# nanoporetech/isONclust2

Hardware: AMD Instinct MI355X
Metric: reads/s clustered (sahlin mode, k=11 w=15) (higher is better)
Workload: dtype u32

## Files before the change

include/isonclust2_hip.h:

```cpp
#ifndef ISONCLUST2_HIP_H
#define ISONCLUST2_HIP_H

#include <stddef.h>
#include <stdint.h>

#ifdef __cplusplus
extern "C" {
#endif

typedef struct ioc_ctx ioc_ctx;

typedef enum {
    IOC_OK = 0,
    IOC_ERR_ARG = -1,
    IOC_ERR_HIP = -2,
    IOC_ERR_STATE = -3,
    IOC_ERR_CAPACITY = -4,
    IOC_ERR_TABLE = -5,
    IOC_ERR_NO_DEVICE = -6,
    IOC_ERR_INPUT = -7
} ioc_status;

enum { IOC_MODE_SAHLIN = 0, IOC_MODE_FAST = 1, IOC_MODE_FURIOUS = 2, IOC_MODE_NONE = 3 };

typedef struct {
    int32_t k;
    int32_t w;
    int32_t min_shared;
    int32_t mode;
    double min_fraction;
    double mapped_threshold;
    double min_prob_no_hits;
    double aligned_threshold;
} ioc_params;

int ioc_ctx_create(int device, ioc_ctx** out);
void ioc_ctx_destroy(ioc_ctx* ctx);
int ioc_ctx_trim(ioc_ctx* ctx);
int ioc_ctx_prewarm(ioc_ctx* ctx, int32_t alignment_mode);
const char* ioc_last_error(const ioc_ctx* ctx);
int ioc_set_stream(ioc_ctx* ctx, void* hip_stream);
int ioc_synchronize(ioc_ctx* ctx);

int ioc_set_params(ioc_ctx* ctx, const ioc_params* p, const int32_t gap_limit[225]);

int ioc_queries_upload(ioc_ctx* ctx, int32_t n, const int64_t* off_fwd, const int64_t* off_rev,
                       const uint32_t* min_val, const uint32_t* min_pos, int64_t total,
                       const uint32_t* hpc_len, const uint8_t* err_cell, const uint32_t* min_total);
int ioc_queries_bind_device(ioc_ctx* ctx, int32_t n, const int64_t* d_off_fwd, const int64_t* d_off_rev,
                            const uint32_t* d_min_val, const uint32_t* d_min_pos, int64_t total,
                            const uint32_t* d_hpc_len, const uint8_t* d_err_cell,
                            const uint32_t* d_min_total, const int64_t* h_off_fwd,
                            const int64_t* h_off_rev);

int ioc_left_load(ioc_ctx* ctx, int32_t n_clusters, const uint8_t* cls_err_cell, int64_t n_keys,
                  const uint32_t* keys, const int64_t* offs, const uint32_t* postings);

int ioc_index_update(ioc_ctx* ctx, int32_t cls, const uint32_t* old_min, int64_t n_old, const uint32_t* new_min,
                     int64_t n_new, uint8_t new_err_cell);
int ioc_left_export(ioc_ctx* ctx, int64_t* n_keys, int64_t* n_postings, uint32_t* keys, int64_t* offs,
                    uint32_t* postings);

int ioc_index_build(ioc_ctx* ctx);
int ioc_score(ioc_ctx* ctx);
int ioc_resolve(ioc_ctx* ctx, int32_t* n_iter);
int ioc_get_decisions(ioc_ctx* ctx, int32_t* target, int8_t* strand, uint8_t* flags);
int ioc_get_cuts(ioc_ctx* ctx, int32_t* cut);
int ioc_force_decision(ioc_ctx* ctx, int32_t query, int32_t target, int32_t strand);
int ioc_clear_forced(ioc_ctx* ctx);
int ioc_set_aln_verdicts(ioc_ctx* ctx, const int32_t* target, const int8_t* strand);
#define IOC_TIE_SLOTS 16
int ioc_get_ties(ioc_ctx* ctx, uint32_t* count, uint32_t* keys);

int ioc_scored_candidates(ioc_ctx* ctx, int32_t q, int32_t cap, uint32_t* key, uint32_t* size);
int ioc_query_candidates(ioc_ctx* ctx, int32_t query, int32_t cap, int32_t* target, int8_t* strand,
                         uint32_t* size, uint32_t* first_index, uint32_t* total_mapped);

int ioc_index_export(ioc_ctx* ctx, int64_t* n_keys, int64_t* n_postings, uint32_t* keys,
                     int64_t* offs, uint32_t* postings);

int ioc_qual_scores(ioc_ctx* ctx, int32_t n, const int64_t* offs, const uint8_t* qual, int32_t k,
                    double* score, double* err_rate);
int ioc_extract_minimizers(ioc_ctx* ctx, int32_t n, const int64_t* offs, const uint8_t* seq,
                           const uint8_t* qual, int32_t k, int32_t w, uint32_t* hpc_len,
                           double* hpc_err, int64_t* off_fwd, int64_t* off_rev, int32_t* status);
int ioc_extracted_hpc_download(ioc_ctx* ctx, char* hpc_seq, char* hpc_qual, int64_t cap);
int ioc_extracted_download(ioc_ctx* ctx, uint32_t* min_val, uint32_t* min_pos, int64_t cap);
int ioc_queries_from_extracted(ioc_ctx* ctx, const uint8_t* keep, const uint8_t* err_cell,
                               const uint32_t* min_total);

typedef struct {
    float ms_build;
    float ms_score;
    float ms_resolve;
    int32_t resolve_iters;
    int32_t n_queries;
    int64_t n_minimizers;
    int64_t n_index_postings;
    int64_t n_candidates;
    int64_t n_mapped_evals;
    int64_t postings_traversed;
    float ms_align_fwd;
    float ms_align_trace;
    int64_t n_align_pairs;
    int64_t n_align_cells;
    int64_t n_align_refused;
    int32_t score_oob;
    int32_t score_oob_probe;
    int64_t align_arena_bytes;
    int32_t align_slices;
    int32_t align_version;
    int64_t n_align_cells_computed;
} ioc_timings;
int ioc_get_timings(ioc_ctx* ctx, ioc_timings* out);
int ioc_count_reference_postings(ioc_ctx* ctx, int64_t* n_postings);

int ioc_host_gap_limits(const char* table_path, int32_t k, int32_t w, double min_prob_no_hits,
                        int32_t* gap_limit, double* p_shared);
uint8_t ioc_host_err_cell(double err_rate);
uint32_t ioc_host_min_total(uint32_t hpc_len, double mapped_threshold);

int ioc_host_align(const char* query, int32_t qlen, const char* ref, int32_t rlen, int32_t match,
                   int32_t mismatch, int32_t gap_open, int32_t gap_extend, char* comp, int32_t comp_cap,
                   int32_t* score_out);
int32_t ioc_host_gap_open(double e1_plus_e2);
double ioc_host_aln_ratio(const char* comp, int32_t comp_len, double e, uint32_t slen, uint32_t k);

typedef struct {
    int32_t query;
    int32_t ref;
    int32_t ref_revcomp;
    int32_t reserved;
    double e;
} ioc_aln_pair;
int ioc_align_set_pool(ioc_ctx* ctx, int32_t n_seqs, const char* seqs, const int64_t* offs);
int ioc_align_pairs(ioc_ctx* ctx, int32_t n_pairs, const ioc_aln_pair* pairs, int32_t k, int32_t match,
                    int32_t mismatch, int32_t gap_extend, int32_t* out_score, int64_t* out_windows,
                    double* out_ratio);
int ioc_align_set_verdict_threshold(ioc_ctx* ctx, double aligned_threshold);

int64_t ioc_queries_generation(const ioc_ctx* ctx);
int64_t ioc_gather_records_device(ioc_ctx* ctx, int32_t n_idx, const int32_t* entries, uint32_t* d_out_min,
                                  uint32_t* d_out_pos, int64_t cap, int64_t* off_fwd, int64_t* off_rev);

typedef struct {
    int32_t n;
    const int64_t* off_fwd;
    const int64_t* off_rev;
    const uint32_t* min_val;
    const uint32_t* min_pos;
    int64_t total;
    const uint32_t* raw_len;
    const uint32_t* hpc_len;
    const double* score;
    const double* raw_err;
    const double* hpc_err;
    const uint8_t* state;
    double min_qual;
    const char* raw_seq;
    const int64_t* raw_off;
    const int32_t* n_members;
    int32_t depth;
    int32_t min_cls_size;
    const uint8_t* is_cluster;
    int32_t minimizers_on_device;
} ioc_batch_view;

typedef struct {
    int32_t n_clusters;
    const double* cls_hpc_err;
    int64_t n_keys;
    const uint32_t* keys;
    const int64_t* offs;
    const uint32_t* postings;
    const char* rep_seq;
    const int64_t* rep_off;
    const double* cls_raw_err;
} ioc_left_view;

typedef struct {
    int64_t n_clusters;
    int64_t n_joined;
    int64_t n_gated;
    int64_t n_tie_replays;
    int64_t n_aln_invoked;
    int32_t resolve_iters;
    int32_t aln_rounds;
    int64_t n_aln_pairs;
    int64_t n_aln_order_dep;
    int64_t n_cons_invoked;
    int64_t n_cons_restarts;
} ioc_cluster_stats;

int ioc_cluster_batch(ioc_ctx* ctx, const ioc_params* p, const char* table_path,
                      const ioc_batch_view* right, int32_t* out_cls, int8_t* out_strand,
                      ioc_cluster_stats* stats);
int ioc_cluster_merge(ioc_ctx* ctx, const ioc_params* p, const char* table_path, const ioc_left_view* left,
                      const ioc_batch_view* right, int32_t* out_cls, int8_t* out_strand,
                      ioc_cluster_stats* stats);
typedef struct {
    const char* raw_seq;
    int32_t raw_len;
    char raw_qual;
    double raw_err;
    double raw_score;
    const char* hpc_seq;
    int32_t hpc_len;
    double hpc_err;
    const uint32_t* fwd_min;
    const uint32_t* fwd_pos;
    int32_t n_fwd;
    const uint32_t* rev_min;
    const uint32_t* rev_pos;
    int32_t n_rev;
    int32_t entry;
} ioc_rep_record;
typedef struct {
    void* user;
    int (*create)(void* user, int side, int idx, const char* seq, int len);
    int (*size)(void* user, int side, int idx);
    int (*add)(void* user, int side, int idx, const char* seq, int len, unsigned weight);
    int (*consensus)(void* user, int side, int idx, char* out, int cap);
    int (*purge)(void* user, int side, int idx, const char* seq, int len, unsigned weight);
    void (*rep_changed)(void* user, int32_t cls, const ioc_rep_record* rec);
    const struct ioc_consensus_spec_ops* spec;
} ioc_consensus_ops;
typedef struct ioc_consensus_spec_ops {
    int (*create_tagged)(void* user, int side, int idx, const char* seq, int len, int tag);
    int (*add_tagged)(void* user, int side, int idx, const char* seq, int len, unsigned weight, int tag);
    int (*consensus_deferred)(void* user, int side, int idx, int tag);
    int (*flush)(void* user, int safe_tag);
    int (*collect)(void* user, int side, int idx, int tag, char* out, int cap);
    int (*rollback)(void* user, int first_tag);
    int (*commit)(void* user);
} ioc_consensus_spec_ops;
typedef struct {
    int32_t cons_min_size;
    int32_t cons_max_size;
    int32_t cons_period;
    int32_t left_depth;
    const int32_t* left_sizes;
} ioc_consensus_args;
int ioc_cluster_consensus(ioc_ctx* ctx, const ioc_params* p, const char* table_path, const ioc_left_view* left,
                          const ioc_batch_view* right, const ioc_consensus_args* args, const ioc_consensus_ops* ops,
                          int32_t* out_cls, int8_t* out_strand, ioc_cluster_stats* stats);

#define IOC_POA_LOCAL 0
#define IOC_POA_GLOBAL 1
#define IOC_POA_SEMI_GLOBAL 2
typedef struct ioc_poa ioc_poa;
int ioc_poa_create(ioc_ctx* ctx, int32_t m, int32_t n, int32_t g, int32_t e, int32_t q, int32_t c, ioc_poa** out);
int ioc_poa_create_mode(ioc_ctx* ctx, int32_t mode, int32_t m, int32_t n, int32_t g, int32_t e, int32_t q, int32_t c, ioc_poa** out);
void ioc_poa_destroy(ioc_poa* poa);
void ioc_poa_bind(ioc_poa* poa, ioc_consensus_ops* ops);
int ioc_poa_graph_export(ioc_poa* poa, int side, int idx, int32_t* n_nodes, int32_t* n_edges, char* bases, int32_t* rank,
                         int32_t* edge_from, int32_t* edge_to, int64_t* edge_w);
int ioc_poa_last_alignment(ioc_poa* poa, int32_t cap, int32_t* nodes, int32_t* pos, int32_t* score);
int64_t ioc_poa_graph_save(ioc_poa* poa, int side, int idx, uint8_t* out, int64_t cap);
int ioc_poa_graph_load(ioc_poa* poa, int side, int idx, const uint8_t* in, int64_t len);
int ioc_poa_graph_load_many(ioc_poa* poa, int side, int32_t count, const int32_t* idx, const uint8_t* const* in, const int64_t* len);

int ioc_cluster_resident(ioc_ctx* ctx, int32_t* out_cls, int8_t* out_strand, ioc_cluster_stats* stats);
int ioc_resident_set_sequences(ioc_ctx* ctx, const char* raw_seq, const int64_t* raw_off, const double* raw_err);

#define IOC_DIST_ID_BYTES 128
int ioc_dist_unique_id(uint8_t* id );
int ioc_dist_init(ioc_ctx* ctx, const uint8_t* id, int32_t rank, int32_t world);
int ioc_dist_shutdown(ioc_ctx* ctx);
int ioc_dist_info(const ioc_ctx* ctx, int32_t* rank, int32_t* world);
int ioc_dist_allgather_device(ioc_ctx* ctx, const void* d_send, void* d_recv, int64_t bytes_per_rank);
int ioc_dist_allgatherv_device(ioc_ctx* ctx, const void* d_send, void* d_recv, const int64_t* counts, const int64_t* displs,
                               int32_t esize);
int ioc_dist_allgather_i64(ioc_ctx* ctx, int64_t mine, int64_t* all );
int ioc_dist_allgatherv_host(ioc_ctx* ctx, const void* send, int64_t bytes, void* recv, int64_t* sizes);
int ioc_dist_allreduce_max(ioc_ctx* ctx, double* x);
int ioc_dist_barrier(ioc_ctx* ctx);
typedef struct {
    float ms_exchange_lists;
    double ms_merge;
    int64_t bytes_lists;
    int64_t bytes_records;
    int32_t sharded;
    int32_t exchanges;
} ioc_dist_merge_times;
#define IOC_XCHG_MAX_U8 0
#define IOC_XCHG_MIN_U32 1
#define IOC_XCHG_SUM_I32 2
typedef int (*ioc_exchange_fn)(void* user, void* d_buf, int64_t count, int32_t kind, void* hip_stream);
int ioc_set_shard(ioc_ctx* ctx, int32_t world, int32_t rank, ioc_exchange_fn fn, void* user);
int32_t ioc_shard_exchanges(const ioc_ctx* ctx);
int64_t ioc_shard_aligned_pairs(const ioc_ctx* ctx);
int ioc_dist_exchange(ioc_ctx* ctx, void* d_buf, int64_t count, int32_t kind);
int ioc_dist_set_shard(ioc_ctx* ctx, int32_t on);

int ioc_dist_merge(ioc_ctx* ctx, const ioc_params* p, const char* table_path, const ioc_batch_view* reps, int32_t min_cls_size,
                   int64_t out_cap, int32_t* out_cls, int8_t* out_strand, int64_t* out_counts, ioc_cluster_stats* stats,
                   ioc_dist_merge_times* times);

#ifdef __cplusplus
}
#endif
#endif
```

isonclust2_amd/_lib.py:

```python
import ctypes as C
import os

HERE = os.path.dirname(os.path.abspath(__file__))
LIB_PATH = os.environ.get("IOC_LIB", os.path.join(HERE, "libisonclust2_hip.so"))
TABLE_PATH = os.path.join(HERE, "data", "pmin_shared.bin")


class IocError(RuntimeError):
    def __init__(self, code, msg):
        super().__init__(f"isonclust2_hip error {code}: {msg}")
        self.code = code


class Params(C.Structure):
    _fields_ = [("k", C.c_int32), ("w", C.c_int32), ("min_shared", C.c_int32), ("mode", C.c_int32),
                ("min_fraction", C.c_double), ("mapped_threshold", C.c_double),
                ("min_prob_no_hits", C.c_double), ("aligned_threshold", C.c_double)]


class BatchView(C.Structure):
    _fields_ = [("n", C.c_int32), ("off_fwd", C.POINTER(C.c_int64)), ("off_rev", C.POINTER(C.c_int64)),
                ("min_val", C.POINTER(C.c_uint32)), ("min_pos", C.POINTER(C.c_uint32)),
                ("total", C.c_int64), ("raw_len", C.POINTER(C.c_uint32)),
                ("hpc_len", C.POINTER(C.c_uint32)), ("score", C.POINTER(C.c_double)),
                ("raw_err", C.POINTER(C.c_double)), ("hpc_err", C.POINTER(C.c_double)),
                ("state", C.POINTER(C.c_uint8)), ("min_qual", C.c_double),
                ("raw_seq", C.c_char_p), ("raw_off", C.POINTER(C.c_int64)),
                ("n_members", C.POINTER(C.c_int32)), ("depth", C.c_int32), ("min_cls_size", C.c_int32),
                ("is_cluster", C.POINTER(C.c_uint8)), ("minimizers_on_device", C.c_int32)]


class LeftView(C.Structure):
    _fields_ = [("n_clusters", C.c_int32), ("cls_hpc_err", C.POINTER(C.c_double)), ("n_keys", C.c_int64),
                ("keys", C.POINTER(C.c_uint32)), ("offs", C.POINTER(C.c_int64)),
                ("postings", C.POINTER(C.c_uint32)), ("rep_seq", C.c_char_p),
                ("rep_off", C.POINTER(C.c_int64)), ("cls_raw_err", C.POINTER(C.c_double))]


class ClusterStats(C.Structure):
    _fields_ = [("n_clusters", C.c_int64), ("n_joined", C.c_int64), ("n_gated", C.c_int64),
                ("n_tie_replays", C.c_int64), ("n_aln_invoked", C.c_int64),
                ("resolve_iters", C.c_int32), ("aln_rounds", C.c_int32), ("n_aln_pairs", C.c_int64),
                ("n_aln_order_dep", C.c_int64), ("n_cons_invoked", C.c_int64), ("n_cons_restarts", C.c_int64)]

    def as_dict(self):
        return {n: int(getattr(self, n)) for n, _ in self._fields_}


class RepRecord(C.Structure):
    _fields_ = [("raw_seq", C.POINTER(C.c_char)), ("raw_len", C.c_int32), ("raw_qual", C.c_char), ("raw_err", C.c_double),
                ("raw_score", C.c_double), ("hpc_seq", C.POINTER(C.c_char)), ("hpc_len", C.c_int32), ("hpc_err", C.c_double),
                ("fwd_min", C.POINTER(C.c_uint32)), ("fwd_pos", C.POINTER(C.c_uint32)), ("n_fwd", C.c_int32),
                ("rev_min", C.POINTER(C.c_uint32)), ("rev_pos", C.POINTER(C.c_uint32)), ("n_rev", C.c_int32),
                ("entry", C.c_int32)]


CONS_CREATE = C.CFUNCTYPE(C.c_int, C.c_void_p, C.c_int, C.c_int, C.POINTER(C.c_char), C.c_int)
CONS_SIZE = C.CFUNCTYPE(C.c_int, C.c_void_p, C.c_int, C.c_int)
CONS_ADD = C.CFUNCTYPE(C.c_int, C.c_void_p, C.c_int, C.c_int, C.POINTER(C.c_char), C.c_int, C.c_uint)
CONS_CONSENSUS = C.CFUNCTYPE(C.c_int, C.c_void_p, C.c_int, C.c_int, C.POINTER(C.c_char), C.c_int)
CONS_PURGE = C.CFUNCTYPE(C.c_int, C.c_void_p, C.c_int, C.c_int, C.POINTER(C.c_char), C.c_int, C.c_uint)
CONS_REP_CHANGED = C.CFUNCTYPE(None, C.c_void_p, C.c_int32, C.POINTER(RepRecord))


class ConsensusOps(C.Structure):
    _fields_ = [("user", C.c_void_p), ("create", CONS_CREATE), ("size", CONS_SIZE), ("add", CONS_ADD),
                ("consensus", CONS_CONSENSUS), ("purge", CONS_PURGE), ("rep_changed", CONS_REP_CHANGED),
                ("spec", C.c_void_p)]


class ConsensusArgs(C.Structure):
    _fields_ = [("cons_min_size", C.c_int32), ("cons_max_size", C.c_int32), ("cons_period", C.c_int32),
                ("left_depth", C.c_int32), ("left_sizes", C.POINTER(C.c_int32))]


class AlnPair(C.Structure):
    _fields_ = [("query", C.c_int32), ("ref", C.c_int32), ("ref_revcomp", C.c_int32), ("reserved", C.c_int32),
                ("e", C.c_double)]


class DistMergeTimes(C.Structure):
    _fields_ = [("ms_exchange_lists", C.c_float), ("ms_merge", C.c_double), ("bytes_lists", C.c_int64), ("bytes_records", C.c_int64),
                ("sharded", C.c_int32), ("exchanges", C.c_int32)]


EXCHANGE_FN = C.CFUNCTYPE(C.c_int, C.c_void_p, C.c_void_p, C.c_int64, C.c_int32, C.c_void_p)
XCHG_MAX_U8, XCHG_MIN_U32, XCHG_SUM_I32 = 0, 1, 2


class Timings(C.Structure):
    _fields_ = [("ms_build", C.c_float), ("ms_score", C.c_float), ("ms_resolve", C.c_float),
                ("resolve_iters", C.c_int32), ("n_queries", C.c_int32), ("n_minimizers", C.c_int64),
                ("n_index_postings", C.c_int64), ("n_candidates", C.c_int64),
                ("n_mapped_evals", C.c_int64), ("postings_traversed", C.c_int64),
                ("ms_align_fwd", C.c_float), ("ms_align_trace", C.c_float), ("n_align_pairs", C.c_int64),
                ("n_align_cells", C.c_int64),
                ("n_align_refused", C.c_int64), ("score_oob", C.c_int32), ("score_oob_probe", C.c_int32),
                ("align_arena_bytes", C.c_int64), ("align_slices", C.c_int32), ("align_version", C.c_int32),
                ("n_align_cells_computed", C.c_int64)]

    def as_dict(self):
        return {n: getattr(self, n) for n, _ in self._fields_}


SYMBOLS = [
    "ioc_ctx_create", "ioc_ctx_destroy", "ioc_ctx_trim", "ioc_ctx_prewarm", "ioc_last_error", "ioc_set_stream", "ioc_synchronize",
    "ioc_set_params", "ioc_queries_upload", "ioc_queries_bind_device", "ioc_left_load",
    "ioc_index_build", "ioc_score", "ioc_resolve", "ioc_get_decisions", "ioc_get_cuts", "ioc_force_decision",
    "ioc_clear_forced", "ioc_query_candidates", "ioc_index_export", "ioc_qual_scores",
    "ioc_extract_minimizers", "ioc_extracted_download", "ioc_extracted_hpc_download", "ioc_queries_from_extracted",
    "ioc_get_timings", "ioc_count_reference_postings", "ioc_host_gap_limits", "ioc_host_err_cell", "ioc_host_min_total",
    "ioc_cluster_batch", "ioc_cluster_merge", "ioc_cluster_resident", "ioc_host_align", "ioc_host_gap_open",
    "ioc_host_aln_ratio", "ioc_align_set_pool", "ioc_align_pairs", "ioc_set_aln_verdicts", "ioc_get_ties", "ioc_resident_set_sequences",
    "ioc_index_update", "ioc_left_export", "ioc_cluster_consensus",
    "ioc_poa_create", "ioc_poa_create_mode", "ioc_poa_destroy", "ioc_poa_bind", "ioc_poa_graph_export", "ioc_poa_last_alignment",
    "ioc_poa_graph_save", "ioc_poa_graph_load", "ioc_poa_graph_load_many", "ioc_gather_records_device", "ioc_queries_generation", "ioc_scored_candidates",
    "ioc_dist_unique_id", "ioc_dist_init", "ioc_dist_shutdown", "ioc_dist_info", "ioc_dist_allgather_device",
    "ioc_dist_allgatherv_device", "ioc_dist_allgather_i64", "ioc_dist_allgatherv_host", "ioc_dist_allreduce_max",
    "ioc_dist_barrier", "ioc_dist_merge", "ioc_set_shard", "ioc_shard_exchanges", "ioc_shard_aligned_pairs", "ioc_dist_exchange", "ioc_dist_set_shard", "ioc_align_set_verdict_threshold",
]

_lib = None


def load():
    global _lib
    if _lib is not None:
        return _lib
    if not os.path.exists(LIB_PATH):
        raise IocError(-100, f"{LIB_PATH} is missing: run `python -c 'import __graft_entry__ as g; g.build()'` "
                             "(hipcc --offload-arch=gfx950); there is no CPU fallback")
    try:
        import torch
    except Exception:
        pass
    L = C.CDLL(LIB_PATH)
    vp, i32, i64 = C.c_void_p, C.c_int32, C.c_int64
    pi64, pu32, pu8 = C.POINTER(C.c_int64), C.POINTER(C.c_uint32), C.POINTER(C.c_uint8)
    pi32, pi8, pd = C.POINTER(C.c_int32), C.POINTER(C.c_int8), C.POINTER(C.c_double)
    L.ioc_ctx_create.argtypes = [i32, C.POINTER(vp)]
    L.ioc_ctx_destroy.argtypes = [vp]
    L.ioc_ctx_destroy.restype = None
    L.ioc_last_error.argtypes = [vp]
    L.ioc_last_error.restype = C.c_char_p
    L.ioc_set_stream.argtypes = [vp, vp]
    L.ioc_synchronize.argtypes = [vp]
    L.ioc_set_params.argtypes = [vp, C.POINTER(Params), pi32]
    L.ioc_queries_upload.argtypes = [vp, i32, pi64, pi64, pu32, pu32, i64, pu32, pu8, pu32]
    L.ioc_queries_bind_device.argtypes = [vp, i32, vp, vp, vp, vp, i64, vp, vp, vp, pi64, pi64]
    L.ioc_gather_records_device.argtypes = [vp, i32, pi32, vp, vp, i64, pi64, pi64]
    L.ioc_gather_records_device.restype = i64
    L.ioc_scored_candidates.argtypes = [vp, i32, i32, pu32, pu32]
    L.ioc_queries_generation.argtypes = [vp]
    L.ioc_queries_generation.restype = i64
    L.ioc_left_load.argtypes = [vp, i32, pu8, i64, pu32, pi64, pu32]
    L.ioc_index_update.argtypes = [vp, i32, pu32, i64, pu32, i64, C.c_uint8]
    L.ioc_left_export.argtypes = [vp, pi64, pi64, pu32, pi64, pu32]
    L.ioc_index_build.argtypes = [vp]
    L.ioc_score.argtypes = [vp]
    L.ioc_resolve.argtypes = [vp, pi32]
    L.ioc_get_decisions.argtypes = [vp, pi32, pi8, pu8]
    L.ioc_get_cuts.argtypes = [vp, pi32]
    L.ioc_force_decision.argtypes = [vp, i32, i32, i32]
    L.ioc_clear_forced.argtypes = [vp]
    L.ioc_query_candidates.argtypes = [vp, i32, i32, pi32, pi8, pu32, pu32, pu32]
    L.ioc_index_export.argtypes = [vp, pi64, pi64, pu32, pi64, pu32]
    L.ioc_qual_scores.argtypes = [vp, i32, pi64, pu8, i32, pd, pd]
    L.ioc_extract_minimizers.argtypes = [vp, i32, pi64, pu8, pu8, i32, i32, pu32, pd, pi64, pi64, pi32]
    L.ioc_extracted_download.argtypes = [vp, pu32, pu32, i64]
    L.ioc_extracted_hpc_download.argtypes = [vp, C.c_char_p, C.c_char_p, i64]
    L.ioc_queries_from_extracted.argtypes = [vp, pu8, pu8, pu32]
    L.ioc_get_timings.argtypes = [vp, C.POINTER(Timings)]
    L.ioc_count_reference_postings.argtypes = [vp, pi64]
    L.ioc_host_gap_limits.argtypes = [C.c_char_p, i32, i32, C.c_double, pi32, pd]
    L.ioc_host_err_cell.argtypes = [C.c_double]
    L.ioc_host_err_cell.restype = C.c_uint8
    L.ioc_host_min_total.argtypes = [C.c_uint32, C.c_double]
    L.ioc_host_min_total.restype = C.c_uint32
    L.ioc_cluster_batch.argtypes = [vp, C.POINTER(Params), C.c_char_p, C.POINTER(BatchView), pi32, pi8,
                                    C.POINTER(ClusterStats)]
    L.ioc_cluster_merge.argtypes = [vp, C.POINTER(Params), C.c_char_p, C.POINTER(LeftView), C.POINTER(BatchView),
                                    pi32, pi8, C.POINTER(ClusterStats)]
    L.ioc_cluster_consensus.argtypes = [vp, C.POINTER(Params), C.c_char_p, C.POINTER(LeftView), C.POINTER(BatchView),
                                        C.POINTER(ConsensusArgs), C.POINTER(ConsensusOps), pi32, pi8, C.POINTER(ClusterStats)]
    L.ioc_poa_create.argtypes = [vp, i32, i32, i32, i32, i32, i32, C.POINTER(vp)]
    L.ioc_poa_create_mode.argtypes = [vp, i32, i32, i32, i32, i32, i32, i32, C.POINTER(vp)]
    L.ioc_poa_destroy.argtypes = [vp]
    L.ioc_poa_destroy.restype = None
    L.ioc_poa_bind.argtypes = [vp, C.POINTER(ConsensusOps)]
    L.ioc_poa_bind.restype = None
    L.ioc_poa_graph_export.argtypes = [vp, C.c_int, C.c_int, pi32, pi32, C.c_char_p, pi32, pi32, pi32, pi64]
    L.ioc_poa_last_alignment.argtypes = [vp, i32, pi32, pi32, pi32]
    L.ioc_poa_graph_save.argtypes = [vp, C.c_int, C.c_int, pu8, i64]
    L.ioc_poa_graph_save.restype = C.c_int64
    L.ioc_poa_graph_load.argtypes = [vp, C.c_int, C.c_int, pu8, i64]
    L.ioc_poa_graph_load_many.argtypes = [vp, C.c_int, C.c_int32, C.POINTER(C.c_int32), C.POINTER(pu8), C.POINTER(i64)]
    L.ioc_host_align.argtypes = [C.c_char_p, i32, C.c_char_p, i32, i32, i32, i32, i32, C.c_char_p, i32, pi32]
    L.ioc_host_gap_open.argtypes = [C.c_double]
    L.ioc_host_aln_ratio.argtypes = [C.c_char_p, i32, C.c_double, C.c_uint32, C.c_uint32]
    L.ioc_host_aln_ratio.restype = C.c_double
    L.ioc_cluster_resident.argtypes = [vp, pi32, pi8, C.POINTER(ClusterStats)]
    L.ioc_resident_set_sequences.argtypes = [vp, C.c_char_p, pi64, pd]
    L.ioc_set_aln_verdicts.argtypes = [vp, pi32, pi8]
    L.ioc_get_ties.argtypes = [vp, C.POINTER(C.c_uint32), C.POINTER(C.c_uint32)]
    L.ioc_align_set_pool.argtypes = [vp, i32, C.c_char_p, C.POINTER(C.c_int64)]
    L.ioc_align_pairs.argtypes = [vp, i32, C.POINTER(AlnPair), i32, i32, i32, i32, pi32, C.POINTER(C.c_int64),
                                  C.POINTER(C.c_double)]
    L.ioc_dist_unique_id.argtypes = [pu8]
    L.ioc_dist_init.argtypes = [vp, pu8, i32, i32]
    L.ioc_dist_shutdown.argtypes = [vp]
    L.ioc_dist_info.argtypes = [vp, pi32, pi32]
    L.ioc_dist_allgather_device.argtypes = [vp, vp, vp, i64]
    L.ioc_dist_allgatherv_device.argtypes = [vp, vp, vp, pi64, pi64, i32]
    L.ioc_dist_allgather_i64.argtypes = [vp, i64, pi64]
    L.ioc_dist_allgatherv_host.argtypes = [vp, vp, i64, vp, pi64]
    L.ioc_dist_allreduce_max.argtypes = [vp, pd]
    L.ioc_dist_barrier.argtypes = [vp]
    L.ioc_dist_merge.argtypes = [vp, C.POINTER(Params), C.c_char_p, C.POINTER(BatchView), i32, i64, pi32, pi8, pi64,
                                 C.POINTER(ClusterStats), C.POINTER(DistMergeTimes)]
    L.ioc_set_shard.argtypes = [vp, i32, i32, EXCHANGE_FN, vp]
    L.ioc_shard_exchanges.argtypes = [vp]
    L.ioc_shard_aligned_pairs.argtypes = [vp]
    L.ioc_shard_aligned_pairs.restype = C.c_int64
    L.ioc_dist_exchange.argtypes = [vp, vp, i64, i32]
    L.ioc_dist_set_shard.argtypes = [vp, i32]
    L.ioc_align_set_verdict_threshold.argtypes = [vp, C.c_double]
    _lib = L
    return L
```

isonclust2_amd/csrc/ioc_align_gpu.hip:

```cpp
#include <hip/hip_runtime.h>

#include <algorithm>
#include <chrono>
#include <cmath>
#include <cstdint>
#include <cstring>
#include <numeric>
#include <string>
#include <type_traits>
#include <vector>

#include "ioc_internal.h"

namespace {

constexpr int ALN_C = 8;
constexpr int ALN_MAXW = 8;
constexpr int ALN_NEG = INT32_MIN / 4;
constexpr uint32_t ALN_LEN_SHIFT = 26;

struct AlnPairDev {
    uint32_t q_off, n;
    uint32_t r_off, m;
    int32_t gap_open, ilimit;
// ... 867 lines not shown
    const AlnPairDev pr = pairs[pid];
    const uint32_t n = pr.n, m = pr.m;
    const int go = pr.gap_open, il = pr.ilimit;
    const uint8_t* __restrict__ q = pool + pr.q_off;
    const uint8_t* __restrict__ r = pool + pr.r_off;
    const int2* __restrict__ rowck = ck + cko[pid].row_off;
    const int2* __restrict__ colck = ck + cko[pid].col_off;
    const uint32_t lane = threadIdx.x & 63u;
    const uint32_t k = P.k, kmask = k >= 32 ? 0xFFFFFFFFu : ((1u << k) - 1u);
    const int4 en = ends[pid];
    uint32_t i = uint32_t(en.y), j = uint32_t(en.z);
    int state = 0;
    WinStat ws;
    ws.blanks((m - j) + (n - i), kmask, k, il);

    while (i > 0 && j > 0) {
        const uint32_t r0 = ((i - 1) / TILE) * TILE, c0 = ((j - 1) / TILE) * TILE;
        const uint32_t rows = i - r0, cols = j - c0;
        const int gd = go - P.gap_extend, ge = P.gap_extend;
        int cm = P.match + 2 * ge + gd, cx = P.mismatch + 2 * ge + gd;
        asm volatile("" : "+v"(cm), "+v"(cx));
        for (uint32_t x = lane; x < rows; x += 64) {
            s_q[x] = q[r0 + x];
            int2 le{ge * int(r0 + x + 1) - gd, ALN_NEG};
            if (c0) le = colck[uint64_t(c0 / TILE - 1) * col_pitch(n) + r0 + x];
            s_left[x] = le;
        }
        const uint32_t jb = c0 + lane * TR_C;
        uint32_t rpk[1];
        {
            uint32_t w = 0;
#pragma unroll
            for (int e = 0; e < TR_C; ++e) w |= ref_byte(r, m, pr.rc, jb + e) << (8 * e);
            rpk[0] = w;
        }
        int Hp[TR_C], F[TR_C];
        int dg = ge * int(r0 + jb) - gd;
        if (r0 == 0) {
#pragma unroll
            for (int c = 0; c < TR_C; ++c) {
                Hp[c] = ge * int(jb + c + 1) - gd;
                F[c] = ALN_NEG;
            }
        } else {
            const int* roh = reinterpret_cast<const int*>(rowck + uint64_t(r0 / TILE - 1) * row_pitch(m));
            const int* rof = roh + row_pitch(m);
#pragma unroll
            for (int c = 0; c < TR_C; ++c) {
                int2 v{0, ALN_NEG};
                if (jb + c < m) v = int2{roh[jb + c], rof[jb + c]};
                Hp[c] = v.x;
                F[c] = v.y;
            }
            if (jb > 0 && jb <= m) dg = roh[jb - 1];
        }
        tr_wave_sync();
        const uint32_t nact = (cols + TR_C - 1) / TR_C;
        const uint32_t nsteps = rows + nact - 1;
        int out_h = 0, out_e = ALN_NEG;
        uint32_t out_q = 0;
        int2 nle = s_left[0];
        uint32_t nq = s_q[0];
        auto tstep = [&](const uint32_t s) __attribute__((always_inline)) {
            int hl = int(from_left_or(uint32_t(out_h), uint32_t(nle.x)));
            int el = int(from_left_or(uint32_t(out_e), uint32_t(nle.y)));
            uint32_t qc = from_left_or(out_q, nq);
            {
                const uint32_t sn = s + 1u < rows ? s + 1u : rows - 1u;
                nle = s_left[sn];
                nq = s_q[sn];
            }
            const int ri = int(s) - int(lane);
            if (ri >= 0 && uint32_t(ri) < rows && lane < nact) {
                const int hl_in = hl;
                uint32_t bits = 0;
#pragma unroll
                for (int c = 0; c < TR_C; ++c) {
                    const bool ex = el > hl;
                    const int E = max(el, hl);
                    const bool fx = F[c] > Hp[c];
                    const int Fn = max(F[c], Hp[c]);
                    const bool mt = qc == ((rpk[0] >> (8 * c)) & 0xFFu);
                    const int hd = dg + (mt ? cm : cx);
                    const int h = max(max(hd, E), Fn);
                    const uint32_t from = h == hd ? (mt ? 0u : 3u << (4 * c)) : (h == E ? 1u << (4 * c) : 2u << (4 * c));
                    bits |= from | (ex ? 4u << (4 * c) : 0u) | (fx ? 8u << (4 * c) : 0u);
                    dg = Hp[c];
                    Hp[c] = h - gd;
                    F[c] = Fn;
                    hl = h - gd;
                    el = E;
                }
                dg = hl_in;
                if (TR_C == 4)
                    dirs[ri][lane] = uint16_t(bits);
                else
                    reinterpret_cast<uint8_t*>(&dirs[0][0])[uint32_t(ri) * 64u + lane] = uint8_t(bits);
            }
            out_h = hl;
            out_e = el;
            out_q = qc;
        };
        {
            uint32_t s = 0;
#if IOC_TR_STEP_UNROLL == 4
            for (; s + 3u < nsteps; s += 4) {
                tstep(s);
                tstep(s + 1u);
                tstep(s + 2u);
                tstep(s + 3u);
            }
#endif
            for (; s + 1u < nsteps; s += 2) {
                tstep(s);
                tstep(s + 1u);
            }
            if (s < nsteps) tstep(s);
        }
        tr_wave_sync();
        while (i > r0 && j > c0) {
            const uint32_t cj = j - c0 - 1;
            const uint32_t ri = i - r0 - 1;
            const uint32_t t = TR_C == 4 ? (uint32_t(dirs[ri][cj / TR_C]) >> (4 * (cj % TR_C))) & 0xFu
                                         : (uint32_t(reinterpret_cast<const uint8_t*>(&dirs[0][0])[ri * 64u + cj / TR_C]) >> (4 * (cj % TR_C))) & 0xFu;
            if (state == 0) {
                const bool inr = i - r0 > lane && j - c0 > lane;
                uint32_t tl = 1u;
                if (inr) {
                    const uint32_t rl = ri - lane, cl = cj - lane;
                    tl = (TR_C == 4 ? (uint32_t(dirs[rl][cl / TR_C]) >> (4 * (cl % TR_C)))
                                    : (uint32_t(reinterpret_cast<const uint8_t*>(&dirs[0][0])[rl * 64u + cl / TR_C]) >> (4 * (cl % TR_C)))) & 3u;
                }
                const bool dgl = inr && (tl == 0u || tl == 3u);
                const unsigned long long dm = __ballot(dgl);
                const uint32_t run = ~dm ? uint32_t(__builtin_ctzll(~dm)) : 64u;
                if (run > 0) {
                    const unsigned long long mb = __ballot(dgl && tl == 0u) & (run == 64u ? ~0ull : ((1ull << run) - 1ull));
                    ws.push_run(mb, run, kmask, k, il, lane);
                    i -= run;
                    j -= run;
                } else {
                    state = (t & 3u) == 1u ? 1 : 2;
                }
            } else if (state == 1) {
                ws.push(0u, kmask, k, il);
                if (!(t & 4u)) state = 0;
                --j;
            } else {
                ws.push(0u, kmask, k, il);
                if (!(t & 8u)) state = 0;
                --i;
            }
        }
        tr_wave_sync();
    }
    ws.blanks(i + j, kmask, k, il);
    if (lane == 0) {
        out_score[pid] = en.x;
        out_count[pid] = ws.cnt;
    }
}

__global__ void __launch_bounds__(256)
k_seq_flags(const uint8_t* __restrict__ pool, const int64_t* __restrict__ offs, uint8_t* __restrict__ flags)
{
    __shared__ uint32_t s_any;
    if (threadIdx.x == 0) s_any = 0;
    __syncthreads();
    const int64_t a = offs[blockIdx.x], b = offs[blockIdx.x + 1];
    uint32_t any = 0;
    for (int64_t i = a + threadIdx.x; i < b; i += 256) {
        const uint8_t ch = pool[i];
        any |= (ch != 'A' && ch != 'C' && ch != 'G' && ch != 'T') ? 1u : 0u;
    }
    if (any) s_any = 1;
    __syncthreads();
    if (threadIdx.x == 0) flags[blockIdx.x] = uint8_t(s_any);
}

int reserve(ioc_ctx* c, DevBuf& b, size_t bytes)
{
    if (bytes == 0) bytes = 16;
    if (b.cap >= bytes) return IOC_OK;
    if (b.p) {
        if (hipStreamSynchronize(c->stream) != hipSuccess) return ioc_fail(c, IOC_ERR_HIP, "stream synchronize failed");
        (void)hipFree(b.p);
        b.p = nullptr;
        b.cap = 0;
    }
    const size_t want = bytes + bytes / 8 + 256;
    const hipError_t e = hipMalloc(&b.p, want);
    if (e != hipSuccess) {
        b.p = nullptr;
        return ioc_fail(c, IOC_ERR_CAPACITY, "hipMalloc(" + std::to_string(want) + " B) failed: " + hipGetErrorString(e));
    }
    b.cap = want;
    ioc_poison(b.p, want);
    return IOC_OK;
}

#define ACHK(c, call)                                                                             \
    do {                                                                                          \
        hipError_t e__ = (call);                                                                  \
        if (e__ != hipSuccess)                                                                    \
            return ioc_fail((c), IOC_ERR_HIP, std::string(#call) + ": " + hipGetErrorString(e__)); \
    } while (0)

#include "ioc_align_v2.inc"


struct EventSet {
    std::vector<hipEvent_t> v;
    ~EventSet()
    {
        for (auto& e : v)
            if (e) (void)hipEventDestroy(e);
    }
};

void add_elapsed(ioc_ctx* c, const std::vector<hipEvent_t>& evs, size_t used)
{
    for (size_t x = 0; x + 2 < used && x + 2 < evs.size(); x += 3) {
        float a = 0, b = 0;
        if (hipEventElapsedTime(&a, evs[x], evs[x + 1]) == hipSuccess) c->tm.ms_align_fwd += a;
        if (hipEventElapsedTime(&b, evs[x + 1], evs[x + 2]) == hipSuccess) c->tm.ms_align_trace += b;
    }
}

int compute_units(const ioc_ctx* c)
{
    int n_cu = 256;
    (void)hipDeviceGetAttribute(&n_cu, hipDeviceAttributeMultiprocessorCount, c->device);
    return n_cu < 1 ? 256 : n_cu;
}

int ck_budget(ioc_ctx* c, uint64_t* budget)
{
    size_t free_b = 0, total_b = 0;
    ACHK(c, hipMemGetInfo(&free_b, &total_b));
    *budget = uint64_t(free_b + c->a_ck.cap) / 2;
    if (const char* e = getenv("IOC_ALIGN_CK_BUDGET_MB")) *budget = uint64_t(atoll(e)) << 20;
    return IOC_OK;
}


constexpr int P16_GUARD = 28000;

struct CorridorModel {
    const ioc_ctx* c;
    AlnParams P;
    double frac;
    bool fixed;
    bool fit_ok;
    double pair_frac(const AlnPairDev& d) const
    {
        if (fixed || !(P.match > 0)) return frac;
        const double e = double(d.e_sum);
        if (!(e > 0.0) || !(e < 1.0)) return frac;
        const int go = std::max(2, std::min(5, d.gap_open));
        double rho = double(P.match) - e * (double(P.match - P.mismatch) / 3.0 + 2.0 / 3.0 * double(go + P.match)), margin = 0.02;
        const ioc_ctx::CorridorFit& f = c->aln_fit[go - 2];
        if (fit_ok && f.n >= 64.0 && e >= f.e_lo - 0.02 && e <= f.e_hi + 0.02) {
            const double me = f.se / f.n, mr = f.sr / f.n, vee = f.see / f.n - me * me, ver = f.ser / f.n - me * mr, vrr = f.srr / f.n - mr * mr;
            const double slope = vee > 1e-9 ? ver / vee : 0.0;
            const double sd = std::sqrt(std::max(0.0, vrr - slope * ver));
            rho = mr + slope * (e - me) - 4.5 * std::max(sd, 0.004);
            margin = 0.003;
        }
        return std::max(0.03, std::min(0.45, 1.0 - rho / double(P.match) + margin));
    }
};

CorridorModel corridor_model(const ioc_ctx* c, const AlnParams& P, bool corridor)
{
    CorridorModel m{c, P, corridor ? 0.2 : 0.0, false, false};
    if (const char* e = getenv("IOC_ALIGN_CORRIDOR")) {
        m.frac = corridor ? std::max(0.0, std::min(1.0, atof(e))) : 0.0;
        m.fixed = true;
    }
    m.fit_ok = c->aln_fit_sig[0] == P.match && c->aln_fit_sig[1] == P.mismatch && c->aln_fit_sig[2] == P.gap_extend && !getenv("IOC_ALIGN_CORRIDOR_NO_FIT");
    return m;
}

uint32_t band_target(uint32_t ncouples, uint32_t few_limit, int occ, int n_cu)
{
    const uint32_t waves = uint32_t(occ) * uint32_t(n_cu) * uint32_t(V2_WAVES);
    uint32_t want = std::max(12u, std::min(uint32_t(V2_MAX_BANDS), (waves + ncouples - 1u) / std::max(1u, ncouples)));
    if (few_limit && ncouples <= few_limit) want = std::min(want, 17u);
    return want;
}

struct V2Plan {
    uint32_t cnt = 0, np = 0, ncouples = 0;
    std::vector<V2Couple> cps;
    std::vector<V2PairCk> pck;
    std::vector<V2PairEnd> pend;
    std::vector<uint64_t> cwords;
    uint32_t lrow_total = 0, best_total = 0, max_strips = 1;
    uint64_t tiles_skipped = 0, tiles_all = 0;
    std::vector<std::pair<uint32_t, uint32_t>> slices;
    uint64_t arena_words = 0, prof_total = 0;
    std::vector<std::vector<V2Item>> items;
    std::vector<uint32_t> n_probe;
    uint32_t max_items = 0, max_flags = 0, max_pairs = 0;
};

void plan_bands(V2Couple& cp, uint32_t ncoarse, uint32_t want_bands, bool corridor)
{
    const uint32_t wb = (corridor && ncoarse >= 16u) ? std::max(want_bands, 17u) : want_bands;
    const uint32_t reg = std::max<uint32_t>(want_bands > 16u ? 1u : 2u, (ncoarse + wb - 1) / wb);
    std::vector<uint32_t> hts;
    for (uint32_t left = ncoarse; left;) {
        const uint32_t hgt = std::min(reg, left);
        hts.push_back(hgt);
        left -= hgt;
    }
    while (hts.size() > size_t(V2_MAX_BANDS)) {
        const size_t mid = hts.size() / 2;
        hts[mid - 1] += hts[mid];
        hts.erase(hts.begin() + long(mid));
    }
    cp.nbands = uint32_t(hts.size());
    cp.tpb = reg;
    uint32_t acc = 0;
    for (uint32_t b = 0; b <= uint32_t(V2_MAX_BANDS); ++b) {
        cp.bstart[b] = uint16_t(std::min<uint32_t>(acc, 0xFFFFu));
        if (b < cp.nbands) acc += hts[b];
    }
}

uint32_t plan_corridor(V2Couple& cp, const std::vector<AlnPairDev>& dp, const CorridorModel& cm, uint32_t nmax, uint32_t mmax, int32_t cert[2])
{
    const AlnParams& P = cm.P;
    constexpr uint32_t probe_rows = 1024;
    cp.corridor = 0;
    for (uint32_t b = 0; b < uint32_t(V2_MAX_BANDS); ++b) {
        cp.plo[b] = 0;
        cp.phi[b] = uint16_t(std::min<uint32_t>(65535u, cp.nstrips - 1u));
    }
    const uint32_t strip_cols = 64u * FW_C;
    double frac = 0.0;
    for (int h = 0; h < 2; ++h)
        if (cp.pid[h] != 0xFFFFFFFFu) frac = std::max(frac, cm.pair_frac(dp[cp.pid[h]]));
    if (cm.frac <= 0.0) frac = 0.0;
    const uint32_t B = uint32_t(frac * double(std::max(nmax, mmax)));
    cp.b0 = B;
    int64_t beff = INT64_MAX;
    uint32_t skipped = 0;
    uint16_t lo[V2_MAX_BANDS], hi[V2_MAX_BANDS];
    bool fits = cm.frac > 0.0 && B >= strip_cols && cp.nstrips <= 65535u && cp.nbands <= uint32_t(V2_MAX_BANDS) && P.match > 0 && P.mismatch <= P.match &&
                P.gap_extend >= 0;
    for (int h = 0; fits && h < 2; ++h)
        if (cp.pid[h] != 0xFFFFFFFFu) fits = dp[cp.pid[h]].gap_open >= 0;
    for (uint32_t b = 0; fits && b < cp.nbands; ++b) {
        const uint32_t r0 = uint32_t(cp.bstart[b]) * uint32_t(CK2), r1 = std::min(nmax, uint32_t(cp.bstart[b + 1u]) * uint32_t(CK2));
        const uint32_t c_lo = r0 > B ? r0 - B : 0u, c_hi = std::min<uint64_t>(mmax, uint64_t(r1) + B);
        if (c_hi <= c_lo) {
            fits = false;
            break;
        }
        lo[b] = uint16_t(c_lo / strip_cols);
        hi[b] = uint16_t((c_hi - 1u) / strip_cols);
        skipped += lo[b] + (cp.nstrips - 1u - hi[b]);
        if (lo[b] > 0) beff = std::min<int64_t>(beff, int64_t(r0) - int64_t(lo[b]) * strip_cols);
        if ((uint64_t(hi[b]) + 1u) * strip_cols < mmax) beff = std::min<int64_t>(beff, int64_t(hi[b] + 1u) * strip_cols - int64_t(r1));
    }
    uint32_t pb = 0, ps = 0;
    if (fits) {
        while (pb + 1u < cp.nbands && uint32_t(cp.bstart[pb + 1u]) * uint32_t(CK2) < probe_rows) ++pb;
        const uint32_t R = uint32_t(cp.bstart[pb + 1u]) * uint32_t(CK2);
        ps = (R - 1u) / strip_cols;
        fits = pb + 1u < cp.nbands && R >= probe_rows;
        for (uint32_t b = 0; fits && b <= pb; ++b) fits = lo[b] == 0 && hi[b] >= ps;
        for (int h = 0; fits && h < 2; ++h)
            if (cp.pid[h] != 0xFFFFFFFFu) fits = dp[cp.pid[h]].n >= R && dp[cp.pid[h]].m > ps * strip_cols;
    }
    cp.probe_band = uint16_t(pb);
    cp.probe_strip = uint16_t(ps);
    if (fits && skipped * 5u >= cp.nbands * cp.nstrips && beff > 0 && beff < INT64_MAX) {
        cp.corridor = 1;
        for (uint32_t b = 0; b < cp.nbands; ++b) {
            cp.plo[b] = lo[b];
            cp.phi[b] = hi[b];
        }
    }
    for (int h = 0; h < 2; ++h) {
        cert[h] = INT32_MIN;
        if (cp.pid[h] == 0xFFFFFFFFu || !cp.corridor) continue;
        const AlnPairDev& d = dp[cp.pid[h]];
        cert[h] = int32_t(std::min<int64_t>(INT32_MAX, int64_t(P.match) * std::max<int64_t>(0, int64_t(std::max(d.n, d.m)) - beff - 1)));
    }
    return cp.corridor ? skipped : 0u;
}

uint64_t couple_words(V2Couple& cp, uint32_t nmax, uint32_t mmax)
{
    auto up4 = [](uint64_t x) { return (x + 3u) & ~uint64_t(3); };
    cp.mpad = uint32_t((uint64_t(mmax) + 15u) & ~uint64_t(15));
    cp.nq = (nmax + 3u) / 4u;
    const uint64_t ncr = (nmax - 1u) / CK2, ncc = (mmax - 1u) / CK2;
    uint64_t w = 0;
    cp.rdat = w;
    w += up4(ncr * 2u * cp.mpad);
    cp.rbase = w;
    w += up4(ncr * (cp.mpad / 16u) * 2u);
    cp.cdat = w;
    w += up4(ncc * uint64_t(cp.nq) * 8u);
    cp.cbase = w;
    w += up4(ncc * uint64_t(cp.nq) * 2u);
    return w;
}

void plan_couples(V2Plan& pl, const std::vector<AlnPairDev>& dp, const uint32_t* order, const CorridorModel& cm, uint32_t want_bands)
{
    pl.cps.resize(pl.ncouples);
    pl.pck.resize(pl.np);
    pl.pend.resize(pl.np);
    pl.cwords.resize(pl.ncouples);
    for (uint32_t k2 = 0; k2 < pl.ncouples; ++k2) {
        V2Couple& cp = pl.cps[k2];
        cp.pid[0] = order[2u * k2];
        cp.pid[1] = 2u * k2 + 1u < pl.cnt ? order[2u * k2 + 1u] : 0xFFFFFFFFu;
        uint32_t nmax = 0, mmax = 0;
        for (int h = 0; h < 2; ++h)
            if (cp.pid[h] != 0xFFFFFFFFu) {
                nmax = std::max(nmax, dp[cp.pid[h]].n);
                mmax = std::max(mmax, dp[cp.pid[h]].m);
            }
        cp.nstrips = (mmax + 64u * FW_C - 1) / (64u * FW_C);
        plan_bands(cp, (nmax + CK2 - 1) / CK2, want_bands, cm.frac > 0.0);
        int32_t cert[2];
        pl.tiles_skipped += plan_corridor(cp, dp, cm, nmax, mmax, cert);
        pl.tiles_all += uint64_t(cp.nbands) * cp.nstrips;
        pl.cwords[k2] = couple_words(cp, nmax, mmax);
        cp.prof = 0;
        pl.max_strips = std::max(pl.max_strips, cp.nstrips);
        for (int h = 0; h < 2; ++h) {
            cp.lrow0[h] = pl.lrow_total;
            cp.best0[h] = pl.best_total;
            if (cp.pid[h] == 0xFFFFFFFFu) continue;
            const AlnPairDev& d = dp[cp.pid[h]];
            const uint32_t nstr = (d.m + 64u * FW_C - 1) / (64u * FW_C);
            pl.pend[cp.pid[h]] = V2PairEnd{pl.lrow_total, pl.best_total, cp.nbands, k2, cert[h]};
            pl.lrow_total += nstr * 64u;
            pl.best_total += cp.nbands;
        }
    }
}

void slice_couples(V2Plan& pl, uint64_t budget)
{
    for (uint32_t first = 0; first < pl.ncouples;) {
        uint64_t used = 0;
        uint32_t k2 = first;
        uint64_t prof_used = 0;
        while (k2 < pl.ncouples) {
            const uint64_t prof_k = uint64_t(pl.cps[k2].nstrips) * 2u * 5u * 64u;
            if (k2 != first && (used + pl.cwords[k2]) * 4ull + (prof_used + prof_k) * sizeof(uint4) > budget) break;
            V2Couple& cp = pl.cps[k2];
            cp.prof = prof_used;
            prof_used += prof_k;
            cp.rdat += used;
            cp.rbase += used;
            cp.cdat += used;
            cp.cbase += used;
            for (int h = 0; h < 2; ++h)
                if (cp.pid[h] != 0xFFFFFFFFu) pl.pck[cp.pid[h]] = V2PairCk{cp.rdat, cp.rbase, cp.cdat, cp.cbase, cp.mpad, cp.nq, uint32_t(h), k2};
            used += pl.cwords[k2];
            ++k2;
        }
        pl.arena_words = std::max(pl.arena_words, used);
        pl.prof_total = std::max(pl.prof_total, prof_used);
        pl.slices.emplace_back(first, k2 - first);
        first = k2;
    }
}

void tile_lists(V2Plan& pl)
{
    pl.items.resize(pl.slices.size());
    pl.n_probe.assign(pl.slices.size(), 0);
    for (size_t si = 0; si < pl.slices.size(); ++si) {
        const uint32_t k_lo = pl.slices[si].first, k_hi = pl.slices[si].first + pl.slices[si].second;
        uint32_t nf = 0;
        auto& it = pl.items[si];
        uint32_t maxdiag = 0;
        size_t total_items = 0;
        for (uint32_t k2 = k_lo; k2 < k_hi; ++k2) {
            V2Couple& cp = pl.cps[k2];
            cp.flag0 = nf;
            nf += cp.nbands * cp.nstrips;
            total_items += size_t(cp.nbands) * cp.nstrips;
            maxdiag = std::max(maxdiag, cp.nbands + cp.nstrips - 2u);
        }
        it.reserve(total_items + 64u * pl.slices[si].second);
        for (uint32_t dg = 0; dg <= maxdiag; ++dg) {
            bool any = false;
            for (uint32_t k2 = k_lo; k2 < k_hi; ++k2) {
                const V2Couple& cp = pl.cps[k2];
                if (!cp.corridor || dg > uint32_t(cp.probe_band) + cp.probe_strip) continue;
                any = true;
                const uint32_t b_lo = dg >= uint32_t(cp.probe_strip) + 1u ? dg - cp.probe_strip : 0u, b_hi = std::min<uint32_t>(dg, cp.probe_band);
                for (uint32_t b = b_lo; b <= b_hi; ++b) it.push_back(V2Item{k2, uint16_t(b), uint16_t(dg - b)});
            }
            if (!any && dg > 64u) break;
        }
        pl.n_probe[si] = uint32_t(it.size());
        for (uint32_t dg = 0; dg <= maxdiag; ++dg)
            for (uint32_t k2 = k_lo; k2 < k_hi; ++k2) {
                const V2Couple& cp = pl.cps[k2];
                if (dg > cp.nbands + cp.nstrips - 2u) continue;
                const uint32_t b_lo = dg >= cp.nstrips ? dg - cp.nstrips + 1u : 0u, b_hi = std::min(dg, cp.nbands - 1u);
                for (uint32_t b = b_lo; b <= b_hi; ++b) it.push_back(V2Item{k2, uint16_t(b), uint16_t(dg - b)});
            }
        pl.max_items = std::max<uint32_t>(pl.max_items, uint32_t(it.size()));
        pl.max_flags = std::max(pl.max_flags, nf);
        pl.max_pairs = std::max(pl.max_pairs, std::min(pl.cnt, 2u * k_hi) - 2u * k_lo);
    }
}

struct V2Opts {
    int n_cu, occ, guard;
    uint32_t few_limit;
    uint32_t deadline;
    unsigned long long deadline_cycles;
    uint32_t help_wgs;
    bool side_help;
};

struct V2Dev {
    V2Couple* cps;
    V2PairCk* pck;
    V2PairEnd* pend;
    V2Item* items;
    int2 *lrow, *best;
    uint32_t* ctl;
    size_t ctl_words;
    V2Scratch *scratch, *hscratch;
    uint32_t* resume;
    uint32_t* park;
    uint32_t* early;
    uint32_t* gate;
    size_t resume_words;
};

int v2_tables(ioc_ctx* c, const V2Plan& pl, uint32_t help_wgs, V2Dev& t)
{
    hipStream_t s = c->stream;
    int r;
    const uint32_t ncouples = pl.ncouples, np = pl.np;
    const size_t tab_bytes = size_t(ncouples) * sizeof(V2Couple) + size_t(np) * (sizeof(V2PairCk) + sizeof(V2PairEnd)) + size_t(pl.max_items) * sizeof(V2Item) + 256;
    if ((r = reserve(c, c->a_cko, tab_bytes)) != IOC_OK) return r;
    uint8_t* tb = static_cast<uint8_t*>(c->a_cko.p);
    t.cps = reinterpret_cast<V2Couple*>(tb);
    t.pck = reinterpret_cast<V2PairCk*>(tb + size_t(ncouples) * sizeof(V2Couple));
    t.pend = reinterpret_cast<V2PairEnd*>(reinterpret_cast<uint8_t*>(t.pck) + size_t(np) * sizeof(V2PairCk));
    t.items = reinterpret_cast<V2Item*>(reinterpret_cast<uint8_t*>(t.pend) + size_t(np) * sizeof(V2PairEnd));
    ACHK(c, hipMemcpyAsync(t.cps, pl.cps.data(), size_t(ncouples) * sizeof(V2Couple), hipMemcpyHostToDevice, s));
    ACHK(c, hipMemcpyAsync(t.pck, pl.pck.data(), size_t(np) * sizeof(V2PairCk), hipMemcpyHostToDevice, s));
    ACHK(c, hipMemcpyAsync(t.pend, pl.pend.data(), size_t(np) * sizeof(V2PairEnd), hipMemcpyHostToDevice, s));
    if ((r = reserve(c, c->a_prof, size_t(pl.prof_total) * sizeof(uint4) + 256)) != IOC_OK) return r;
    if ((r = reserve(c, c->a_ends2, size_t(np) * sizeof(int4))) != IOC_OK) return r;
    if ((r = reserve(c, c->a_lrow, (size_t(pl.lrow_total) + pl.best_total + 16) * sizeof(int2))) != IOC_OK) return r;
    t.lrow = static_cast<int2*>(c->a_lrow.p);
    t.best = t.lrow + pl.lrow_total;
    t.ctl_words = ((16 + 2 * size_t(pl.max_flags) + np + 1) & ~size_t(1)) + 2;
    if ((r = reserve(c, c->a_xflags, t.ctl_words * 4)) != IOC_OK) return r;
    t.ctl = static_cast<uint32_t*>(c->a_xflags.p);
    const size_t n_scratch = size_t(pl.max_pairs) + size_t(help_wgs) * V2_NHELP * V2_HBUF;
    t.resume_words = size_t(np) * V2_RESUME_WORDS + 2u * (size_t(pl.max_pairs) + 1u) + 4u;
    if ((r = reserve(c, c->a_bnd, n_scratch * sizeof(V2Scratch) + t.resume_words * 4)) != IOC_OK) return r;
    t.scratch = static_cast<V2Scratch*>(c->a_bnd.p);
    t.hscratch = t.scratch + pl.max_pairs;
    t.resume = reinterpret_cast<uint32_t*>(t.scratch + n_scratch);
    t.park = t.resume + size_t(np) * V2_RESUME_WORDS;
    t.early = t.park + size_t(pl.max_pairs) + 1u;
    t.gate = t.early + size_t(pl.max_pairs) + 1u;
    return IOC_OK;
}

uint32_t v2_per_cu(const V2Plan& pl, size_t si, const V2Opts& o, bool few_couples)
{
    if (few_couples) return uint32_t(o.occ);
    uint64_t tiles = 0;
    uint32_t diags = 1;
    for (uint32_t k2 = pl.slices[si].first; k2 < pl.slices[si].first + pl.slices[si].second; ++k2) {
        const V2Couple& cp = pl.cps[k2];
        for (uint32_t b = 0; b < cp.nbands; ++b) tiles += uint32_t(cp.phi[b]) - uint32_t(cp.plo[b]) + 1u;
        diags = std::max(diags, cp.nbands + cp.nstrips - 1u);
    }
    const double x = double(tiles) / double(diags) / double(uint32_t(o.n_cu) * uint32_t(V2_WAVES));
    return x < 1.0 ? 1u : x < 2.75 ? std::min(2u, uint32_t(o.occ)) : uint32_t(o.occ);
}

int v2_slice(ioc_ctx* c, const V2Plan& pl, const V2Dev& t, size_t si, const V2Opts& o, const AlnParams& P, const uint32_t* d_order,
             int32_t* d_score, uint32_t* d_count, const hipEvent_t* ev, uint32_t* xe)
{
    hipStream_t s = c->stream;
    const uint32_t k_first = pl.slices[si].first, n_couples = pl.slices[si].second;
    const uint32_t first_pair = 2u * k_first, n_pairs = std::min(pl.cnt, 2u * (k_first + n_couples)) - first_pair;
    const uint32_t n_items = uint32_t(pl.items[si].size()), n_probe = pl.n_probe[si];
    const AlnPairDev* d_pairs = static_cast<const AlnPairDev*>(c->a_pairs.p);
    const uint8_t* d_pool = static_cast<const uint8_t*>(c->a_pool.p);
    uint32_t* d_ctl = t.ctl;
    const bool few_couples = n_couples <= o.few_limit;
    const uint32_t prog_every = few_couples ? 1u : 0u;
    ACHK(c, hipMemcpyAsync(t.items, pl.items[si].data(), size_t(n_items) * sizeof(V2Item), hipMemcpyHostToDevice, s));
    ACHK(c, hipMemcpyAsync(t.cps + k_first, pl.cps.data() + k_first, size_t(n_couples) * sizeof(V2Couple), hipMemcpyHostToDevice, s));
    hipLaunchKernelGGL(k_fwd2_prof, dim3(n_couples, pl.max_strips), dim3(128), 0, s, d_pairs, t.cps + k_first, d_pool, P, static_cast<uint4*>(c->a_prof.p));
    ACHK(c, hipGetLastError());
    ACHK(c, hipMemsetAsync(d_ctl, 0, t.ctl_words * 4, s));
    ACHK(c, hipMemsetAsync(t.resume, 0, t.resume_words * 4, s));
    if (pl.tiles_skipped)
        ACHK(c, hipMemsetAsync(t.lrow, 0x80, (size_t(pl.lrow_total) + pl.best_total) * sizeof(int2), s));
    if (getenv("IOC_ALIGN_V2_FAKE_TIMEOUT")) {
        const uint32_t one = 1;
        ACHK(c, hipMemcpyAsync(d_ctl + 1, &one, 4, hipMemcpyHostToDevice, s));
    }
    ACHK(c, hipEventRecord(ev[0], s));
    auto fwd = [&](decltype(&k_fwd2) kernel, uint32_t n_wg, const V2Item* items, uint32_t n) {
        hipLaunchKernelGGL(kernel, dim3(n_wg), dim3(64 * V2_WAVES), 0, s, d_pairs, t.cps, items, n, d_ctl, d_ctl + 16, d_ctl + 1, d_pool, P,
                           static_cast<uint32_t*>(c->a_ck.p), t.lrow, t.best, d_ctl + 16 + 2 * pl.max_flags, o.guard, static_cast<const uint4*>(c->a_prof.p),
                           reinterpret_cast<unsigned long long*>(d_ctl + t.ctl_words - 2), few_couples ? d_ctl + 16 + pl.max_flags : static_cast<uint32_t*>(nullptr),
                           prog_every);
    };
    if (n_probe) {
        fwd(k_fwd2, std::max(1u, std::min(uint32_t(o.occ) * uint32_t(o.n_cu), (n_probe + V2_WAVES - 1) / V2_WAVES)), t.items, n_probe);
        ACHK(c, hipGetLastError());
        hipLaunchKernelGGL(k_fwd2_probe, dim3(n_couples), dim3(64), 0, s, d_pairs, t.cps + k_first, t.pend, static_cast<const uint32_t*>(c->a_ck.p), P);
        ACHK(c, hipGetLastError());
        ACHK(c, hipMemsetAsync(d_ctl, 0, 4, s));
    }
    const uint32_t n_main = n_items - n_probe, per_cu = v2_per_cu(pl, si, o, few_couples);
    const uint32_t n_wg = std::max(1u, std::min(per_cu * uint32_t(o.n_cu), (n_main + V2_WAVES - 1) / V2_WAVES));
    fwd((per_cu <= 2 && !getenv("IOC_ALIGN_V2_NO_W2")) ? k_fwd2_w2 : k_fwd2, n_wg, t.items + n_probe, n_main);
    ACHK(c, hipGetLastError());
    const uint32_t n_help = std::min<uint32_t>(n_pairs, o.help_wgs);
    hipLaunchKernelGGL(k_fwd2_ends, dim3(n_pairs), dim3(64), 0, s, d_pairs, t.cps, d_order + first_pair, n_pairs, t.pend, t.lrow, t.best,
                       d_ctl + 16 + 2 * pl.max_flags, static_cast<int4*>(c->a_ends2.p), t.resume, t.early, o.side_help ? int(P.match) : 0, n_help);
    ACHK(c, hipGetLastError());
    ACHK(c, hipEventRecord(ev[1], s));
    auto help = [&](hipStream_t hs, uint32_t* list, uint32_t which, uint32_t* gate) {
        hipLaunchKernelGGL(k_trace2_help, dim3(n_help), dim3(64 * V2_HWAVES), 0, hs, d_pairs, d_order + first_pair, d_pool, P,
                           static_cast<const uint32_t*>(c->a_ck.p), t.cps, t.pck, static_cast<const int4*>(c->a_ends2.p), t.scratch, t.hscratch, t.resume,
                           list, d_score, d_count, n_pairs, which, gate);
    };
    if (o.side_help) {
        ACHK(c, hipEventRecord(c->ev_side[0], s));
        ACHK(c, hipStreamWaitEvent(c->side_stream, c->ev_side[0], 0));
        help(c->side_stream, t.early, 2u, t.gate);
        ACHK(c, hipGetLastError());
        ACHK(c, hipEventRecord(c->ev_side[1], c->side_stream));
        hipLaunchKernelGGL(k_trace2_gate, dim3(1), dim3(1), 0, s, t.early, t.gate, n_help);
        ACHK(c, hipGetLastError());
    }
    hipLaunchKernelGGL(k_trace2, dim3((n_pairs + TR_WAVES - 1) / TR_WAVES), dim3(64 * TR_WAVES), 0, s, d_pairs, d_order + first_pair, d_pool, P,
                       static_cast<const uint32_t*>(c->a_ck.p), t.cps, t.pck, static_cast<const int4*>(c->a_ends2.p), t.scratch, t.resume, t.park, d_score,
                       d_count, n_pairs, o.deadline, o.deadline_cycles);
    ACHK(c, hipGetLastError());
    if (o.side_help) ACHK(c, hipStreamWaitEvent(s, c->ev_side[1], 0));
    if (o.deadline) {
        help(s, t.park, 1u, nullptr);
        ACHK(c, hipGetLastError());
    }
    ACHK(c, hipEventRecord(ev[2], s));
    unsigned long long cells_done = 0;
    ACHK(c, hipMemcpyAsync(xe, d_ctl + 1, 4, hipMemcpyDeviceToHost, s));
    ACHK(c, hipMemcpyAsync(&cells_done, d_ctl + t.ctl_words - 2, 8, hipMemcpyDeviceToHost, s));
    ACHK(c, hipStreamSynchronize(s));
    c->tm.n_align_cells_computed += int64_t(cells_done);
    return IOC_OK;
}

int v2_report(ioc_ctx* c, const std::vector<AlnPairDev>& dp, const uint32_t* order, const V2Plan& pl, const V2Dev& t, size_t si, uint32_t deadline)
{
    const bool rates = getenv("IOC_V2_TRACE_RATES") != nullptr, times = getenv("IOC_V2_TRACE_TIMES") != nullptr;
    if (!rates && !times) return IOC_OK;
    const uint32_t np = pl.np, first_pair = 2u * pl.slices[si].first;
    const uint32_t n_pairs = std::min(pl.cnt, 2u * (pl.slices[si].first + pl.slices[si].second)) - first_pair;
    std::vector<int4> he(np);
    ACHK(c, hipMemcpy(he.data(), c->a_ends2.p, size_t(np) * sizeof(int4), hipMemcpyDeviceToHost));
    if (rates)
        for (uint32_t x = 0; x < n_pairs; ++x) {
            const uint32_t pid = order[first_pair + x];
            const AlnPairDev& d = dp[pid];
            fprintf(stderr, "[rate] e %.5f n %u m %u score %d per_base %.5f go %d flags %d corridor %u\n", double(d.e_sum), d.n, d.m, he[pid].x,
                    double(he[pid].x) / double(std::max(d.n, d.m)), d.gap_open, he[pid].w, pl.cps[pl.pend[pid].couple].corridor);
        }
    if (!times) return IOC_OK;
    std::vector<uint32_t> rw(size_t(np) * V2_RESUME_WORDS);
    ACHK(c, hipMemcpy(rw.data(), t.resume, rw.size() * 4, hipMemcpyDeviceToHost));
    std::vector<uint32_t> ids(n_pairs);
    for (uint32_t x = 0; x < n_pairs; ++x) ids[x] = order[first_pair + x];
    auto rec = [&](uint32_t pid, uint32_t w) { return rw[size_t(pid) * V2_RESUME_WORDS + w]; };
    auto cost = [&](uint32_t pid) { return (double(rec(pid, 8)) + double(rec(pid, 12))) * 256.0; };
    std::sort(ids.begin(), ids.end(), [&](uint32_t a, uint32_t b) { return cost(a) > cost(b); });
    double sum = 0;
    uint32_t parked = 0;
    for (uint32_t pid : ids) {
        sum += cost(pid);
        parked += rec(pid, 6) ? 1u : 0u;
    }
    fprintf(stderr, "[ioc] k_trace2: %u pairs, %u walks went on in the second launch (deadline %u blocks); mean %.3e cycles (s_memtime), slowest first:\n", n_pairs, parked,
            deadline, sum / n_pairs);
    auto line = [&](const char* tag, uint32_t pid) {
        const AlnPairDev& d = dp[pid];
        fprintf(stderr, "[ioc]   %s pair %u: %.3e + %.3e cycles, n %u m %u, blocks %u (%u on the diagonal) + %u (%u by helpers), tiles %u + %u, gap steps %u, windows %u\n", tag, pid,
                double(rec(pid, 8)) * 256.0, double(rec(pid, 12)) * 256.0, d.n, d.m, rec(pid, 9) & 0xFFFFu, rec(pid, 9) >> 16, rec(pid, 13) & 0xFFFFu, rec(pid, 13) >> 16,
                rec(pid, 10), rec(pid, 14), rec(pid, 11), rec(pid, 15));
    };
    {
        double pk_max = -1e9, un_min = 1e9, pk_sum = 0, un_sum = 0;
        uint32_t npk = 0, nun = 0;
        std::vector<double> pks, uns;
        for (uint32_t pid : ids) {
            const AlnPairDev& d = dp[pid];
            const double q = double(he[pid].x) / double(std::max(1u, std::min(d.n, d.m)));
            if (rec(pid, 6)) {
                pk_max = std::max(pk_max, q), pk_sum += q, ++npk;
                pks.push_back(q);
            } else {
                un_min = std::min(un_min, q), un_sum += q, ++nun;
                uns.push_back(q);
            }
        }
        std::sort(pks.begin(), pks.end());
        std::sort(uns.begin(), uns.end());
        auto qt = [](const std::vector<double>& v, double f) { return v.empty() ? 0.0 : v[std::min(v.size() - 1, size_t(f * double(v.size())))]; };
        fprintf(stderr, "[ioc]   forward score / shorter length: parked walks (%u) mean %.3f, 50 %% %.3f, 90 %% %.3f, 99 %% %.3f, max %.3f | others (%u) min %.3f, 1 %% %.3f, 10 %% %.3f, mean %.3f\n", npk,
                npk ? pk_sum / npk : 0.0, qt(pks, 0.5), qt(pks, 0.9), qt(pks, 0.99), pk_max, nun, un_min, qt(uns, 0.01), qt(uns, 0.1), nun ? un_sum / nun : 0.0);
    }
    for (uint32_t x = 0; x < std::min(n_pairs, 10u); ++x) line("", ids[x]);
    for (uint32_t qx : {n_pairs / 4u, n_pairs / 2u, 3u * n_pairs / 4u}) line("rank", ids[qx]);
    return IOC_OK;
}

int align_v2_run(ioc_ctx* c, const std::vector<AlnPairDev>& dp, const uint32_t* order, uint32_t cnt, const uint32_t* d_order,
                 const AlnParams& P, int32_t* d_score, uint32_t* d_count, bool corridor, bool* fell_back)
{
    *fell_back = false;
    if (cnt == 0) return IOC_OK;
    int r;
    const auto t_plan0 = std::chrono::steady_clock::now();
    V2Opts o{};
    o.n_cu = compute_units(c);
    uint64_t budget = 0;
    if ((r = ck_budget(c, &budget)) != IOC_OK) return r;
    o.guard = P16_GUARD;
    if (const char* e = getenv("IOC_ALIGN_V2_GUARD")) o.guard = std::max(1, std::min(P16_GUARD, atoi(e)));
    o.few_limit = 128;
    if (const char* e = getenv("IOC_ALIGN_V2_FEW")) o.few_limit = uint32_t(std::max(0, atoi(e)));
    if (hipOccupancyMaxActiveBlocksPerMultiprocessor(&o.occ, reinterpret_cast<const void*>(k_fwd2), 64 * V2_WAVES, 0) != hipSuccess) o.occ = 0;
    (void)hipGetLastError();
    if (o.occ < 1) o.occ = 3;

    V2Plan pl;
    pl.cnt = cnt;
    pl.np = uint32_t(dp.size());
    pl.ncouples = (cnt + 1u) / 2u;
    plan_couples(pl, dp, order, corridor_model(c, P, corridor), band_target(pl.ncouples, o.few_limit, o.occ, o.n_cu));
    slice_couples(pl, budget);
    const auto t_res0 = std::chrono::steady_clock::now();
    if ((r = reserve(c, c->a_ck, size_t(pl.arena_words) * 4)) != IOC_OK) return r;
    c->tm.align_arena_bytes = int64_t(pl.arena_words) * 4;
    c->tm.align_slices = int32_t(pl.slices.size());
    c->tm.align_version = 2;
    if (getenv("IOC_TRACE"))
        fprintf(stderr, "[ioc]   aligner v2: %u couples, checkpoint arena %.1f MB (%zu slice(s)) reserved in %.3f ms; corridor: %llu of %llu tiles skipped\n", pl.ncouples,
                double(pl.arena_words) * 4e-6, pl.slices.size(), std::chrono::duration<double, std::milli>(std::chrono::steady_clock::now() - t_res0).count(),
                (unsigned long long)pl.tiles_skipped, (unsigned long long)pl.tiles_all);
    tile_lists(pl);

    o.deadline = 4;
    if (const char* e = getenv("IOC_TRACE2_DEADLINE")) o.deadline = uint32_t(std::max(0, atoi(e)));
    if (const char* e = getenv("IOC_TRACE2_CYCLES")) o.deadline_cycles = (unsigned long long)std::max(0.0, atof(e));
    o.help_wgs = o.deadline ? std::min<uint32_t>(pl.max_pairs, uint32_t(o.n_cu)) : 0u;
    V2Dev t{};
    if ((r = v2_tables(c, pl, o.help_wgs, t)) != IOC_OK) return r;
    o.side_help = o.deadline && !(getenv("IOC_TRACE2_EARLY") && atoi(getenv("IOC_TRACE2_EARLY")) == 0);
    if (o.side_help && !c->side_stream) {
        ACHK(c, hipStreamCreateWithFlags(&c->side_stream, hipStreamNonBlocking));
        for (auto& e : c->ev_side) ACHK(c, hipEventCreateWithFlags(&e, hipEventDisableTiming));
    }
    EventSet evs;
    evs.v.assign(pl.slices.size() * 3, nullptr);
    for (auto& e : evs.v) ACHK(c, hipEventCreate(&e));
    if (getenv("IOC_TRACE"))
        fprintf(stderr, "[ioc]   aligner v2: planning (couples, corridors, tile lists, tables) took the host %.3f ms\n",
                std::chrono::duration<double, std::milli>(std::chrono::steady_clock::now() - t_plan0).count());
    size_t evi = 0;
    bool bad = false;
    for (size_t si = 0; si < pl.slices.size() && !bad; ++si, evi += 3) {
        uint32_t xe = 0;
        if ((r = v2_slice(c, pl, t, si, o, P, d_order, d_score, d_count, &evs.v[evi], &xe)) != IOC_OK) return r;
        if ((r = v2_report(c, dp, order, pl, t, si, o.deadline)) != IOC_OK) return r;
        bad = xe != 0;
    }
    add_elapsed(c, evs.v, evi);
    if (getenv("IOC_TRACE"))
        fprintf(stderr, "[ioc]   aligner v2: forward %.3f ms, traceback %.3f ms (device, all slices so far)%s\n", c->tm.ms_align_fwd,
                c->tm.ms_align_trace, bad ? " — a wait ran out: falling back to version 1" : "");
    *fell_back = bad;
    return IOC_OK;
}


enum class AlnRoute { normal, every_tile, v1_only };

struct AlnOut {
    int32_t* score;
    int64_t* windows;
    double* ratio;
    void set(size_t i, int32_t s, int64_t w, double r) const
    {
        if (score) score[i] = s;
        if (windows) windows[i] = w;
        if (ratio) ratio[i] = r;
    }
};

struct AlnBatch {
    std::vector<AlnPairDev> dp;
    std::vector<uint32_t> back;
    std::vector<uint32_t> order;
    uint32_t max_n = 1, max_m = 1;
};

int prepare_pairs(ioc_ctx* c, int32_t n_pairs, const ioc_aln_pair* pairs, const AlnParams& P, const AlnOut& out, AlnBatch& b)
{
    const int32_t n_seqs = c->aln_offs.empty() ? 0 : int32_t(c->aln_offs.size() - 1);
    const int32_t k = int32_t(P.k);
    b.dp.reserve(size_t(n_pairs));
    for (int32_t i = 0; i < n_pairs; ++i) {
        const ioc_aln_pair& a = pairs[i];
        if (a.query < 0 || a.query >= n_seqs || a.ref < 0 || a.ref >= n_seqs)
            return ioc_fail(c, IOC_ERR_ARG, "alignment pair refers to a sequence outside the pool");
        const int64_t n = c->aln_offs[size_t(a.query) + 1] - c->aln_offs[size_t(a.query)];
        const int64_t m = c->aln_offs[size_t(a.ref) + 1] - c->aln_offs[size_t(a.ref)];
        if (n + m >= (int64_t(1) << ALN_LEN_SHIFT))
            return ioc_fail(c, IOC_ERR_CAPACITY, "GPU aligner: sequences above 2^26 bases");
        const double limit = std::floor((1.0 - a.e) * double(k));
        const int32_t il = limit < -1.0 ? -1 : limit > 64.0 ? 64 : int32_t(limit);
        if (n == 0 || m == 0) {
            const int64_t len = n + m;
            const int64_t cnt = (il <= 0 && len > k) ? len - k : 0;
            out.set(size_t(i), 0, cnt, n == 0 ? 0.0 : double(cnt) / double(n));
            continue;
        }
        AlnPairDev d{};
        d.q_off = uint32_t(c->aln_offs[size_t(a.query)]);
        d.n = uint32_t(n);
        d.r_off = uint32_t(c->aln_offs[size_t(a.ref)]);
        d.m = uint32_t(m);
        d.gap_open = ioc_host_gap_open(a.e);
        d.e_sum = float(a.e);
        d.ilimit = il;
        d.rc = a.ref_revcomp ? 1u : 0u;
        d.stop_at = 0;
        if (c->aln_verdict_thr > 0.0 && n > 0) {
            double a0 = std::ceil(c->aln_verdict_thr * double(n));
            while (a0 > 0 && (a0 - 1.0) / double(n) >= c->aln_verdict_thr) a0 -= 1.0;
            while (a0 / double(n) < c->aln_verdict_thr) a0 += 1.0;
            d.stop_at = a0 >= 1.0 && a0 < 4.0e9 ? uint32_t(a0) : 0u;
        }
        {
            const int gd = d.gap_open - P.gap_extend, cm = P.match + 2 * P.gap_extend + gd, cx = P.mismatch + 2 * P.gap_extend + gd;
            const bool ok = !c->aln_other[size_t(a.query)] && !c->aln_other[size_t(a.ref)] && cm >= 0 && cm <= 255 &&
                            cx >= 0 && cx <= 255 && !getenv("IOC_ALIGN_NO_PROFILE");
            d.pad = ok ? 1u : 0u;
        }
        b.dp.push_back(d);
        b.back.push_back(uint32_t(i));
        b.max_n = std::max(b.max_n, d.n);
        b.max_m = std::max(b.max_m, d.m);
    }
    return IOC_OK;
}

void order_pairs(AlnBatch& b, const ioc_aln_pair* pairs)
{
    const std::vector<AlnPairDev>& dp = b.dp;
    const uint32_t np = uint32_t(dp.size());
    std::vector<uint32_t>& order = b.order;
    order.resize(np);
    std::iota(order.begin(), order.end(), 0u);
    std::stable_sort(order.begin(), order.end(), [&](uint32_t x, uint32_t y) {
        return uint64_t(dp[x].n) * dp[x].m > uint64_t(dp[y].n) * dp[y].m;
    });
    {
        auto rows = [&](uint32_t x) { return uint64_t((dp[x].n + 511u) / 512u); };
        auto cols = [&](uint32_t x) { return uint64_t((dp[x].m + 511u) / 512u); };
        std::stable_sort(order.begin(), order.end(), [&](uint32_t x, uint32_t y) {
            const uint64_t tx = rows(x) * cols(x), ty = rows(y) * cols(y);
            if (tx != ty) return tx > ty;
            if (rows(x) != rows(y)) return rows(x) > rows(y);
            return dp[x].e_sum > dp[y].e_sum;
        });
    }
    {
        std::vector<int32_t> hp;
        for (uint32_t x = 0; x < np; ++x)
            if (pairs[b.back[x]].reserved > 0) hp.push_back(pairs[b.back[x]].reserved);
        if (hp.size() >= 8 && !getenv("IOC_ALIGN_NO_HINTS")) {
            std::nth_element(hp.begin(), hp.begin() + long(hp.size() / 2), hp.end());
            const int64_t med = hp[hp.size() / 2];
            std::stable_partition(order.begin(), order.end(), [&](uint32_t x) {
                const int64_t h = pairs[b.back[x]].reserved;
                return !(h > 0 && h * 4 < med);
            });
        }
    }
    std::stable_partition(order.begin(), order.end(), [&](uint32_t x) { return dp[x].pad != 0; });
}

struct WavePlan {
    uint32_t waves;
    bool few_pairs;
};
WavePlan plan_waves(const AlnBatch& b, bool carry)
{
    const uint32_t np = uint32_t(b.dp.size());
    uint32_t waves = ALN_MAXW;
    if (const char* e = getenv("IOC_ALIGN_WAVES")) {
        const int v = atoi(e);
        if (v >= 1 && v <= ALN_MAXW) waves = uint32_t(v);
    } else {
        while (waves > 1 && uint64_t(np) * waves > 4096) waves >>= 1;
        if (carry) {
            while (waves > 1 && uint64_t(waves / 2) * 64 * ALN_C >= b.max_m) waves >>= 1;
        } else {
            const uint32_t strips = (b.max_m + 64 * FW_C - 1) / (64 * FW_C), tiles = (b.max_n + TILE - 1) / TILE;
            while (waves > 1 && (strips < 2 * waves || tiles < 2 * waves)) waves >>= 1;
        }
    }
    const bool few_pairs = !carry && !getenv("IOC_ALIGN_WAVES") && np <= 64 && waves >= 4 && !getenv("IOC_ALIGN_NO_CROSS_TAIL");
    return WavePlan{few_pairs ? 4u : waves, few_pairs};
}

int run_v2(ioc_ctx* c, const AlnBatch& b, const AlnParams& P, int32_t* d_score, uint32_t* d_count, AlnRoute route, uint32_t* n_v2)
{
    const uint32_t np = uint32_t(b.dp.size());
    uint32_t n = 0;
    while (n < np && b.dp[b.order[n]].pad != 0) ++n;
    bool fell_back = false;
    const int r = align_v2_run(c, b.dp, b.order.data(), n, static_cast<const uint32_t*>(c->a_order.p), P, d_score, d_count, route != AlnRoute::every_tile,
                               &fell_back);
    if (r != IOC_OK) return r;
    if (fell_back) {
        c->tm.n_align_refused += n;
        n = 0;
    }
    *n_v2 = n;
    return IOC_OK;
}

int run_carry(ioc_ctx* c, const AlnBatch& b, uint32_t waves, const AlnParams& P, int32_t* d_score, uint32_t* d_count)
{
    const uint32_t np = uint32_t(b.dp.size()), NT = waves * 64;
    const uint64_t bnd_stride = 2ull * 6ull * b.max_n;
    const uint64_t lrow_entries = uint64_t((b.max_m + NT * ALN_C - 1) / (NT * ALN_C)) * NT;
    const uint64_t lrow_stride = lrow_entries * 4ull;
    const uint64_t budget = 8ull << 30;
    const uint64_t per_pair = (bnd_stride + lrow_stride) * 4ull;
    const uint32_t slice = uint32_t(std::min<uint64_t>(np, std::max<uint64_t>(1, budget / per_pair)));
    int r;
    if ((r = reserve(c, c->a_bnd, size_t(slice) * bnd_stride * 4)) != IOC_OK) return r;
    if ((r = reserve(c, c->a_lrow, size_t(slice) * lrow_stride * 4)) != IOC_OK) return r;
    for (uint32_t first = 0; first < np; first += slice) {
        const uint32_t cnt = std::min(slice, np - first);
        hipLaunchKernelGGL(k_align_carry, dim3(cnt), dim3(NT), 0, c->stream, static_cast<const AlnPairDev*>(c->a_pairs.p),
                           static_cast<const uint32_t*>(c->a_order.p) + first, static_cast<const uint8_t*>(c->a_pool.p), P,
                           static_cast<uint32_t*>(c->a_bnd.p), bnd_stride, static_cast<uint32_t*>(c->a_lrow.p), lrow_stride, d_score, d_count);
        ACHK(c, hipGetLastError());
    }
    return IOC_OK;
}


size_t fwd_lds_limit(ioc_ctx* c, bool prof, const void* kfn, size_t fallback, size_t* stat)
{
    hipFuncAttributes fa{};
    *stat = fallback;
    if (hipFuncGetAttributes(&fa, kfn) == hipSuccess) *stat = fa.sharedSizeBytes;
    size_t& lim = prof ? c->aln_lds_max : c->aln_lds_max2;
    if (lim == 0) {
        int mx = 0;
        (void)hipDeviceGetAttribute(&mx, hipDeviceAttributeMaxSharedMemoryPerBlock, c->device);
        lim = 64 * 1024 > *stat ? 64 * 1024 - *stat : 1;
        if (mx > 72 * 1024 && hipFuncSetAttribute(kfn, hipFuncAttributeMaxDynamicSharedMemorySize, mx - int(*stat)) == hipSuccess)
            lim = size_t(mx) - *stat;
        (void)hipGetLastError();
    }
    return lim;
}

struct V1Plan {
    std::vector<AlnCk> cko;
    std::vector<std::pair<uint32_t, uint32_t>> slices;
    uint64_t arena = 0;
    uint32_t max_cnt = 0;
};
uint64_t v1_row_units(const AlnPairDev& d) { return uint64_t((d.n - 1) / TILE) * row_pitch(d.m); }

V1Plan plan_v1(const AlnBatch& b, uint32_t n_v2, uint64_t budget)
{
    const std::vector<AlnPairDev>& dp = b.dp;
    const uint32_t np = uint32_t(dp.size());
    V1Plan pl;
    pl.cko.resize(np);
    for (uint32_t first = n_v2; first < np;) {
        uint64_t used = 0;
        uint32_t cnt = 0;
        while (first + cnt < np) {
            const AlnPairDev& d = dp[b.order[first + cnt]];
            const uint64_t u = v1_row_units(d) + uint64_t((d.m - 1) / TILE) * col_pitch(d.n);
            if (cnt > 0 && (used + u) * 8ull > budget) break;
            if (cnt > 0 && d.pad != dp[b.order[first]].pad) break;
            pl.cko[b.order[first + cnt]] = AlnCk{used, used + v1_row_units(d)};
            used += u;
            ++cnt;
        }
        pl.arena = std::max(pl.arena, used);
        pl.slices.emplace_back(first, cnt);
        pl.max_cnt = std::max(pl.max_cnt, cnt);
        first += cnt;
    }
    return pl;
}

struct V1Fwd {
    ioc_ctx* c;
    bool prof;
    AlnParams P;
    uint64_t lrow_stride;
    int operator()(const uint32_t* o, uint32_t cnt, uint32_t wv, uint32_t wgw, uint32_t nwg, uint32_t nmain, uint32_t wtail, size_t lds,
                   uint32_t lrow_first, const AlnCross& X) const
    {
        const AlnPairDev* dpairs = static_cast<const AlnPairDev*>(c->a_pairs.p);
        const uint8_t* dpool = static_cast<const uint8_t*>(c->a_pool.p);
        int2* dck = static_cast<int2*>(c->a_ck.p);
        const AlnCk* dcko = static_cast<const AlnCk*>(c->a_cko.p);
        int2* lr = static_cast<int2*>(c->a_lrow.p) + uint64_t(lrow_first) * lrow_stride;
        int4* dends = static_cast<int4*>(c->a_ends2.p);
        if (prof)
            hipLaunchKernelGGL(k_align_fwd<true>, dim3(nwg), dim3(wgw * 64), lds, c->stream, dpairs, o, cnt, wv, nmain, wtail, dpool, P, dck, dcko, lr,
                               lrow_stride, dends, X);
        else
            hipLaunchKernelGGL(k_align_fwd<false>, dim3(nwg), dim3(wgw * 64), lds, c->stream, dpairs, o, cnt, wv, nmain, wtail, dpool, P, dck, dcko, lr,
                               lrow_stride, dends, X);
        ACHK(c, hipGetLastError());
        return IOC_OK;
    }
};

int v1_cross_tail(ioc_ctx* c, const AlnBatch& b, const V1Fwd& fwd, const std::pair<uint32_t, uint32_t>& sl, uint32_t waves, uint32_t wg_waves,
                  uint32_t n_main, uint32_t ppw, uint32_t groups, bool inl, size_t lds_pad, const void* kfn)
{
    hipStream_t s = c->stream;
    const uint32_t* ord = static_cast<const uint32_t*>(c->a_order.p) + sl.first;
    const uint32_t first_cnt = n_main * ppw, rest = sl.second - first_cnt, nb = 4 * groups;
    uint32_t strips = 1;
    for (uint32_t x = first_cnt; x < sl.second; ++x) strips = std::max(strips, (b.dp[b.order[sl.first + x]].m + 64 * FW_C - 1) / (64 * FW_C));
    AlnCross X;
    X.groups = groups;
    X.flag_stride = nb * strips;
    const size_t fbytes = size_t(rest) * X.flag_stride * 4, bbytes = size_t(rest) * nb * sizeof(int2);
    int r;
    if ((r = reserve(c, c->a_xflags, fbytes + bbytes + 64)) != IOC_OK) return r;
    X.err = static_cast<uint32_t*>(c->a_xflags.p);
    X.flags = X.err + 16;
    X.best = reinterpret_cast<int2*>(reinterpret_cast<uint8_t*>(c->a_xflags.p) + 64 + fbytes);
    ACHK(c, hipMemsetAsync(c->a_xflags.p, 0, 64 + fbytes, s));
    if (inl && first_cnt) {
        X.first_wg = n_main;
        X.first_pair = first_cnt;
        if ((r = fwd(ord, sl.second, waves, wg_waves, n_main + rest * groups, n_main + rest * groups, waves, lds_pad, 0, X)) != IOC_OK) return r;
    } else {
        if (first_cnt && (r = fwd(ord, first_cnt, waves, wg_waves, n_main, n_main, waves, lds_pad, 0, AlnCross{})) != IOC_OK) return r;
        size_t stat = 0, xlds = 0;
        const size_t lim = fwd_lds_limit(c, fwd.prof, kfn, 52 * 1024, &stat), want = 84 * 1024;
        if (want > stat && want - stat <= lim) xlds = (want - stat) & ~size_t(255);
        if ((r = fwd(ord + first_cnt, rest, 4, 4, rest * groups, rest * groups, 4, xlds, first_cnt, X)) != IOC_OK) return r;
    }
    uint32_t xe = 0;
    ACHK(c, hipMemcpyAsync(&xe, X.err, 4, hipMemcpyDeviceToHost, s));
    ACHK(c, hipStreamSynchronize(s));
    if (xe) {
        if ((r = fwd(ord + first_cnt, rest, 4, 4, rest, rest, 4, 0, first_cnt, AlnCross{})) != IOC_OK) return r;
        c->tm.n_align_refused += rest;
    }
    return IOC_OK;
}

int v1_slice(ioc_ctx* c, const AlnBatch& b, const std::pair<uint32_t, uint32_t>& sl, const WavePlan& wp, const AlnParams& P, int n_cu,
             uint64_t lrow_stride, int32_t* d_score, uint32_t* d_count, const hipEvent_t* ev)
{
    hipStream_t s = c->stream;
    const uint32_t waves = wp.waves;
    const uint32_t* ord = static_cast<const uint32_t*>(c->a_order.p) + sl.first;
    const bool prof = b.dp[b.order[sl.first]].pad != 0;
    const void* kfn = prof ? reinterpret_cast<const void*>(k_align_fwd<true>) : reinterpret_cast<const void*>(k_align_fwd<false>);
    const V1Fwd fwd{c, prof, P, lrow_stride};
    size_t lds_pad = 0;
    const uint32_t wg_waves = waves > 4 ? waves : 4, ppw = wg_waves / waves;
    uint32_t n_wg = (sl.second + ppw - 1) / ppw, n_main = n_wg, wpp_tail = waves;
    {
        int occ = 0;
        if (hipOccupancyMaxActiveBlocksPerMultiprocessor(&occ, kfn, int(wg_waves * 64), 0) != hipSuccess) occ = 0;
        (void)hipGetLastError();
        const uint32_t gen = uint32_t(occ > 0 ? occ : 3) * uint32_t(n_cu);
        if (n_wg > gen && n_wg < gen + gen / 2 && 2 * waves <= wg_waves) {
            n_main = gen;
            wpp_tail = 2 * waves;
            const uint32_t rest = sl.second - n_main * ppw, ppw_tail = wg_waves / wpp_tail;
            n_wg = n_main + (rest + ppw_tail - 1) / ppw_tail;
        }
    }
    const uint32_t per_cu = (n_main + uint32_t(n_cu) - 1) / uint32_t(n_cu);
    if (per_cu * wg_waves < 32) {
        size_t stat = 0;
        const size_t lim = fwd_lds_limit(c, prof, kfn, 48 * 1024, &stat);
        const size_t want = size_t(160u * 1024u) * (2 * per_cu + 1) / (2 * per_cu * (per_cu + 1));
        lds_pad = want > stat + 1024 ? (want - stat - 512) & ~size_t(255) : 0;
        lds_pad = std::min(lds_pad, lim > 1 ? lim : 0);
    }
    ACHK(c, hipEventRecord(ev[0], s));
    uint32_t groups = 1;
    const bool force_cross = getenv("IOC_ALIGN_FORCE_CROSS") != nullptr || (wp.few_pairs && waves == 4);
    if (force_cross && wg_waves == 4) {
        n_main = 0;
        n_wg = 1;
    }
    const bool inl = !force_cross;
    if (n_main < n_wg && wg_waves == 4 && !getenv("IOC_ALIGN_NO_CROSS_TAIL")) {
        const AlnPairDev& big = b.dp[b.order[sl.first]];
        const uint32_t strips = (big.m + 64 * FW_C - 1) / (64 * FW_C), tiles = (big.n + TILE - 1) / TILE;
        groups = force_cross ? 4 : 2;
        if (const char* eg = getenv("IOC_ALIGN_CROSS_GROUPS")) groups = uint32_t(std::max(1, std::min(4, atoi(eg))));
        while (groups > 1 && (strips < 4 * groups || tiles < 8 * groups)) groups >>= 1;
        const uint32_t rest = sl.second - n_main * ppw;
        while (groups > 1 && uint64_t(rest) * groups > uint64_t(inl ? 2 : 1) * uint64_t(n_cu)) groups >>= 1;
    }
    int r;
    if (groups > 1) {
        if ((r = v1_cross_tail(c, b, fwd, sl, waves, wg_waves, n_main, ppw, groups, inl, lds_pad, kfn)) != IOC_OK) return r;
    } else {
        if (force_cross && n_main == 0) {
            n_wg = (sl.second + ppw - 1) / ppw;
            n_main = n_wg;
        }
        if ((r = fwd(ord, sl.second, waves, wg_waves, n_wg, n_main, wpp_tail, lds_pad, 0, AlnCross{})) != IOC_OK) return r;
    }
    ACHK(c, hipEventRecord(ev[1], s));
    const uint32_t tr_wg = (sl.second + TR_WAVES - 1) / TR_WAVES;
    hipLaunchKernelGGL(k_align_trace, dim3(tr_wg), dim3(64 * TR_WAVES), 0, s, static_cast<const AlnPairDev*>(c->a_pairs.p), ord,
                       static_cast<const uint8_t*>(c->a_pool.p), P, static_cast<const int2*>(c->a_ck.p), static_cast<const AlnCk*>(c->a_cko.p),
                       static_cast<const int4*>(c->a_ends2.p), d_score, d_count, sl.second);
    ACHK(c, hipGetLastError());
    ACHK(c, hipEventRecord(ev[2], s));
    return IOC_OK;
}

int run_v1(ioc_ctx* c, const AlnBatch& b, uint32_t n_v2, const WavePlan& wp, const AlnParams& P, int32_t* d_score, uint32_t* d_count)
{
    hipStream_t s = c->stream;
    const uint32_t np = uint32_t(b.dp.size());
    int r;
    uint64_t budget = 0;
    if ((r = ck_budget(c, &budget)) != IOC_OK) return r;
    const uint64_t lrow_stride = uint64_t((b.max_m + 64 * FW_C - 1) / (64 * FW_C)) * 64;
    for (const AlnPairDev& d : b.dp)
        if (v1_row_units(d) >= (uint64_t(1) << 29))
            return ioc_fail(c, IOC_ERR_CAPACITY, "alignment of " + std::to_string(d.n) + " x " + std::to_string(d.m) + " bases: row checkpoints above 4 GB per pair");
    const V1Plan pl = plan_v1(b, n_v2, budget);
    const auto t_res0 = std::chrono::steady_clock::now();
    if ((r = reserve(c, c->a_ck, size_t(pl.arena) * 8)) != IOC_OK) return r;
    c->tm.align_arena_bytes = int64_t(pl.arena) * 8;
    c->tm.align_slices = int32_t(pl.slices.size());
    c->tm.align_version = 1;
    if (getenv("IOC_TRACE"))
        fprintf(stderr, "[ioc]   aligner: checkpoint arena %.1f MB (%zu slice(s)) reserved in %.3f ms\n", double(pl.arena) * 8e-6, pl.slices.size(),
                std::chrono::duration<double, std::milli>(std::chrono::steady_clock::now() - t_res0).count());
    if ((r = reserve(c, c->a_cko, size_t(np) * sizeof(AlnCk))) != IOC_OK) return r;
    if ((r = reserve(c, c->a_ends2, size_t(np) * sizeof(int4))) != IOC_OK) return r;
    if ((r = reserve(c, c->a_lrow, size_t(pl.max_cnt) * lrow_stride * 8)) != IOC_OK) return r;
    ACHK(c, hipMemcpyAsync(c->a_cko.p, pl.cko.data(), size_t(np) * sizeof(AlnCk), hipMemcpyHostToDevice, s));
    const int n_cu = compute_units(c);
    EventSet evs;
    evs.v.assign(pl.slices.size() * 3, nullptr);
    for (auto& e : evs.v) ACHK(c, hipEventCreate(&e));
    for (size_t si = 0; si < pl.slices.size(); ++si)
        if ((r = v1_slice(c, b, pl.slices[si], wp, P, n_cu, lrow_stride, d_score, d_count, &evs.v[3 * si])) != IOC_OK) return r;
    ACHK(c, hipStreamSynchronize(s));
    add_elapsed(c, evs.v, evs.v.size());
    if (getenv("IOC_TRACE"))
        fprintf(stderr, "[ioc]   aligner: forward %.3f ms, traceback %.3f ms (device, all slices so far)\n", c->tm.ms_align_fwd, c->tm.ms_align_trace);
    return IOC_OK;
}


void learn_corridor(ioc_ctx* c, const AlnBatch& b, const AlnParams& P, const std::vector<int32_t>& hs, const std::vector<uint32_t>& hc)
{
    if (c->aln_fit_sig[0] != P.match || c->aln_fit_sig[1] != P.mismatch || c->aln_fit_sig[2] != P.gap_extend) {
        for (auto& f : c->aln_fit) f = ioc_ctx::CorridorFit();
        c->aln_fit_sig[0] = P.match, c->aln_fit_sig[1] = P.mismatch, c->aln_fit_sig[2] = P.gap_extend;
    }
    for (size_t x = 0; x < b.dp.size(); ++x) {
        const AlnPairDev& d = b.dp[x];
        const uint32_t len = std::max(d.n, d.m);
        if (hc[x] == 0xFFFFFFFFu || len < 4096u || !(d.e_sum > 0.0f) || std::min(d.n, d.m) * 10u < len * 9u) continue;
        const double rho = double(hs[x]) / double(len), e = double(d.e_sum);
        if (rho * 2.0 < double(P.match)) continue;
        ioc_ctx::CorridorFit& f = c->aln_fit[std::max(2, std::min(5, d.gap_open)) - 2];
        if (f.n >= 1e6) continue;
        f.n += 1.0, f.se += e, f.sr += rho, f.see += e * e, f.ser += e * rho, f.srr += rho * rho;
        f.e_lo = std::min(f.e_lo, e), f.e_hi = std::max(f.e_hi, e);
    }
}

int read_results(ioc_ctx* c, const AlnBatch& b, uint32_t n_v2, const int32_t* d_score, const uint32_t* d_count, std::vector<int32_t>& hs,
                 std::vector<uint32_t>& hc)
{
    const uint32_t np = uint32_t(b.dp.size());
    c->tm.n_align_pairs += np;
    for (auto& d : b.dp) c->tm.n_align_cells += int64_t(d.n) * int64_t(d.m);
    for (uint32_t x = n_v2; x < np; ++x)
        c->tm.n_align_cells_computed += int64_t(b.dp[b.order[x]].n) * int64_t(b.dp[b.order[x]].m);
    hs.resize(np);
    hc.resize(np);
    ACHK(c, hipMemcpyAsync(hs.data(), d_score, size_t(np) * 4, hipMemcpyDeviceToHost, c->stream));
    ACHK(c, hipMemcpyAsync(hc.data(), d_count, size_t(np) * 4, hipMemcpyDeviceToHost, c->stream));
    ACHK(c, hipStreamSynchronize(c->stream));
    return IOC_OK;
}


int align_pairs(ioc_ctx* c, int32_t n_pairs, const ioc_aln_pair* pairs, int32_t k, int32_t match, int32_t mismatch, int32_t gap_extend,
                const AlnOut& out, AlnRoute route);

int align_again(ioc_ctx* c, const ioc_aln_pair* pairs, const std::vector<int32_t>& idx, const AlnParams& P, AlnRoute route, const AlnOut& out)
{
    std::vector<ioc_aln_pair> sub(idx.size());
    std::vector<int32_t> sc(idx.size());
    std::vector<int64_t> sw(idx.size());
    std::vector<double> sr(idx.size());
    for (size_t x = 0; x < idx.size(); ++x) sub[x] = pairs[idx[x]];
    const int r = align_pairs(c, int32_t(sub.size()), sub.data(), int32_t(P.k), P.match, P.mismatch, P.gap_extend, AlnOut{sc.data(), sw.data(), sr.data()}, route);
    if (r != IOC_OK) return r;
    for (size_t x = 0; x < idx.size(); ++x) out.set(size_t(idx[x]), sc[x], sw[x], sr[x]);
    return IOC_OK;
}

int scatter_results(ioc_ctx* c, const AlnBatch& b, const ioc_aln_pair* pairs, bool v2, const AlnParams& P, const std::vector<int32_t>& hs,
                    const std::vector<uint32_t>& hc, const AlnOut& out)
{
    std::vector<int32_t> again;
    std::vector<int32_t> again_full;
    for (size_t x = 0; x < b.dp.size(); ++x) {
        const uint32_t i = b.back[x];
        if (v2 && hc[x] == 0xFFFFFFFFu && hs[x] == INT32_MIN) {
            again.push_back(int32_t(i));
            continue;
        }
        if (v2 && hc[x] == 0xFFFFFFFFu && hs[x] == INT32_MIN + 1) {
            again_full.push_back(int32_t(i));
            continue;
        }
        out.set(i, hs[x], int64_t(hc[x]), double(hc[x]) / double(b.dp[x].n));
    }
    int r;
    if (!again_full.empty()) {
        const int64_t pairs_so_far = c->tm.n_align_pairs, cells_so_far = c->tm.n_align_cells;
        if ((r = align_again(c, pairs, again_full, P, AlnRoute::every_tile, out)) != IOC_OK) return r;
        c->tm.n_align_pairs = pairs_so_far;
        c->tm.n_align_cells = cells_so_far;
        if (getenv("IOC_TRACE")) fprintf(stderr, "[ioc]   aligner v2: %zu of %zu pairs run again without a corridor\n", again_full.size(), b.dp.size());
    }
    if (!again.empty()) {
        if ((r = align_again(c, pairs, again, P, AlnRoute::v1_only, out)) != IOC_OK) return r;
        c->tm.n_align_refused += int64_t(again.size());
    }
    return IOC_OK;
}

int align_pairs(ioc_ctx* c, int32_t n_pairs, const ioc_aln_pair* pairs, int32_t k, int32_t match, int32_t mismatch, int32_t gap_extend,
                const AlnOut& out, AlnRoute route)
{
    if (!c || n_pairs < 0 || (n_pairs > 0 && !pairs)) return IOC_ERR_ARG;
    if (k < 1 || k > 32) return ioc_fail(c, IOC_ERR_CAPACITY, "GPU aligner: window length k must be in 1..32");
    ACHK(c, hipSetDevice(c->device));
    if (n_pairs == 0) return IOC_OK;
    const AlnParams P{match, mismatch, gap_extend, uint32_t(k), 1u << (32 - k)};
    AlnBatch b;
    int r;
    if ((r = prepare_pairs(c, n_pairs, pairs, P, out, b)) != IOC_OK) return r;
    const uint32_t np = uint32_t(b.dp.size());
    if (np == 0) return IOC_OK;
    order_pairs(b, pairs);
    const char* ev = getenv("IOC_ALIGN_VARIANT");
    const bool carry = ev && strcmp(ev, "carry") == 0;
    const WavePlan wp = plan_waves(b, carry);
    if ((r = reserve(c, c->a_pairs, size_t(np) * sizeof(AlnPairDev))) != IOC_OK) return r;
    if ((r = reserve(c, c->a_order, size_t(np) * 4)) != IOC_OK) return r;
    if ((r = reserve(c, c->a_out, size_t(np) * 8)) != IOC_OK) return r;
    ACHK(c, hipMemcpyAsync(c->a_pairs.p, b.dp.data(), size_t(np) * sizeof(AlnPairDev), hipMemcpyHostToDevice, c->stream));
    ACHK(c, hipMemcpyAsync(c->a_order.p, b.order.data(), size_t(np) * 4, hipMemcpyHostToDevice, c->stream));
    int32_t* d_score = static_cast<int32_t*>(c->a_out.p);
    uint32_t* d_count = reinterpret_cast<uint32_t*>(d_score + np);
    const char* arena_mode = getenv("IOC_ALIGN_ARENA");
    const bool v2 = route != AlnRoute::v1_only && !carry && !getenv("IOC_ALIGN_V1") && !(arena_mode && strcmp(arena_mode, "fat") == 0);
    uint32_t n_v2 = 0;
    if (v2 && (r = run_v2(c, b, P, d_score, d_count, route, &n_v2)) != IOC_OK) return r;
    if (carry)
        r = run_carry(c, b, wp.waves, P, d_score, d_count);
    else if (n_v2 < np)
        r = run_v1(c, b, n_v2, wp, P, d_score, d_count);
    if (r != IOC_OK) return r;
    std::vector<int32_t> hs;
    std::vector<uint32_t> hc;
    if ((r = read_results(c, b, n_v2, d_score, d_count, hs, hc)) != IOC_OK) return r;
    if (v2 && route == AlnRoute::normal) learn_corridor(c, b, P, hs, hc);
    return scatter_results(c, b, pairs, v2, P, hs, hc, out);
}

}

extern "C" {

int ioc_align_set_pool(ioc_ctx* c, int32_t n_seqs, const char* seqs, const int64_t* offs)
{
    if (!c || n_seqs < 0 || (n_seqs > 0 && (!seqs || !offs))) return IOC_ERR_ARG;
    ACHK(c, hipSetDevice(c->device));
    c->res_pool_ready = false;
    c->aln_offs.assign(offs, offs + (n_seqs > 0 ? n_seqs + 1 : 0));
    if (n_seqs == 0) return IOC_OK;
    if (offs[0] != 0) return ioc_fail(c, IOC_ERR_ARG, "sequence pool offsets must start at 0");
    for (int32_t i = 0; i < n_seqs; ++i)
        if (offs[i + 1] < offs[i]) return ioc_fail(c, IOC_ERR_ARG, "sequence pool offsets must be ascending");
    const int64_t total = offs[n_seqs];
    if (total >= (int64_t(1) << 32)) return ioc_fail(c, IOC_ERR_CAPACITY, "sequence pool above 4 GiB");
    int r = reserve(c, c->a_pool, size_t(total));
    if (r != IOC_OK) return r;
    ACHK(c, hipMemcpyAsync(c->a_pool.p, seqs, size_t(total), hipMemcpyHostToDevice, c->stream));
    if ((r = reserve(c, c->a_ends, size_t(n_seqs + 1) * 8 + size_t(n_seqs))) != IOC_OK) return r;
    int64_t* d_offs = static_cast<int64_t*>(c->a_ends.p);
    uint8_t* d_flags = reinterpret_cast<uint8_t*>(d_offs + n_seqs + 1);
    ACHK(c, hipMemcpyAsync(d_offs, offs, size_t(n_seqs + 1) * 8, hipMemcpyHostToDevice, c->stream));
    hipLaunchKernelGGL(k_seq_flags, dim3(uint32_t(n_seqs)), dim3(256), 0, c->stream,
                       static_cast<const uint8_t*>(c->a_pool.p), d_offs, d_flags);
    ACHK(c, hipGetLastError());
    c->aln_other.assign(size_t(n_seqs), 0);
    ACHK(c, hipMemcpyAsync(c->aln_other.data(), d_flags, size_t(n_seqs), hipMemcpyDeviceToHost, c->stream));
    ACHK(c, hipStreamSynchronize(c->stream));
    return IOC_OK;
}

int ioc_align_set_verdict_threshold(ioc_ctx* c, double aligned_threshold)
{
    if (!c) return IOC_ERR_ARG;
    c->aln_verdict_thr = aligned_threshold > 0.0 ? aligned_threshold : -1.0;
    return IOC_OK;
}

int ioc_align_pairs(ioc_ctx* c, int32_t n_pairs, const ioc_aln_pair* pairs, int32_t k, int32_t match, int32_t mismatch,
                    int32_t gap_extend, int32_t* out_score, int64_t* out_windows, double* out_ratio)
{
    return align_pairs(c, n_pairs, pairs, k, match, mismatch, gap_extend, AlnOut{out_score, out_windows, out_ratio}, AlnRoute::normal);
}

hipError_t iock_warm_align()
{
    hipFuncAttributes a;
    return hipFuncGetAttributes(&a, reinterpret_cast<const void*>(k_fwd2_ends));
}

}
```

isonclust2_amd/csrc/ioc_align_v2.inc:

```

constexpr int CK2 = 512;
constexpr int V2_WAVES = 4;
constexpr int V2_BLK_C = 8;
constexpr int V2_MAX_BANDS = 40;
static_assert(CK2 % TILE == 0 && CK2 == 64 * V2_BLK_C, "block geometry");

struct V2Couple {
    uint32_t pid[2];
    uint32_t nbands, nstrips;
    uint32_t tpb;
    uint32_t flag0;
    uint32_t mpad;
    uint32_t nq;
    uint64_t rdat;
    uint64_t rbase;
    uint64_t cdat;
    uint64_t cbase;
    uint64_t prof;
    uint32_t lrow0[2];
    uint32_t best0[2];
    uint16_t bstart[V2_MAX_BANDS + 1];
    uint16_t plo[V2_MAX_BANDS], phi[V2_MAX_BANDS];
    uint32_t corridor;
    uint16_t probe_band, probe_strip;
    uint32_t b0;
};

struct V2Item {
    uint32_t couple;
    uint16_t band, strip;
};

struct V2PairCk {
    uint64_t rdat, rbase, cdat, cbase;
    uint32_t mpad, nq, half, couple;
};


__device__ __forceinline__ bool v2_wait(const uint32_t* flag, uint32_t* err)
{
    uint32_t seen = 0;
    for (uint32_t it = 0; it < (1u << 22); ++it) {
        seen = uint32_t(__builtin_amdgcn_readfirstlane(int(__hip_atomic_load(flag, __ATOMIC_RELAXED, __HIP_MEMORY_SCOPE_AGENT))));
        if (seen) break;
        if ((it & 255u) == 255u && __builtin_amdgcn_readfirstlane(int(__hip_atomic_load(err, __ATOMIC_RELAXED, __HIP_MEMORY_SCOPE_AGENT)))) break;
        __builtin_amdgcn_s_sleep(8);
    }
    if (!seen) __hip_atomic_store(err, 1u, __ATOMIC_RELAXED, __HIP_MEMORY_SCOPE_AGENT);
    return seen != 0;
}

__device__ __forceinline__ bool v2_wait_rows(const uint32_t* prog, const uint32_t* flag, uint32_t need, uint32_t* err, uint32_t& avail)
{
    bool ok = false;
    for (uint32_t it = 0; it < (1u << 22); ++it) {
        const uint32_t f = uint32_t(__builtin_amdgcn_readfirstlane(int(__hip_atomic_load(flag, __ATOMIC_RELAXED, __HIP_MEMORY_SCOPE_AGENT))));
        const uint32_t g = uint32_t(__builtin_amdgcn_readfirstlane(int(__hip_atomic_load(prog, __ATOMIC_RELAXED, __HIP_MEMORY_SCOPE_AGENT))));
        if (f || g >= need) {
            ok = true;
            avail = f ? 0xFFFFFFFFu : g;
            break;
        }
        if ((it & 255u) == 255u && __builtin_amdgcn_readfirstlane(int(__hip_atomic_load(err, __ATOMIC_RELAXED, __HIP_MEMORY_SCOPE_AGENT)))) break;
        __builtin_amdgcn_s_sleep(4);
    }
    if (!ok) __hip_atomic_store(err, 1u, __ATOMIC_RELAXED, __HIP_MEMORY_SCOPE_AGENT);
    return ok;
}

__device__ __forceinline__ uint32_t v2_dequeue(uint32_t* queue)
{
    uint32_t x = 0, one = 1;
    unsigned long long save;
    asm volatile(
        "s_mov_b64 %1, exec\n\t"
        "s_mov_b64 exec, 1\n\t"
        "global_atomic_add %0, %2, %3, off sc0\n\t"
        "s_waitcnt vmcnt(0)\n\t"
        "s_mov_b64 exec, %1"
        : "+v"(x), "=&s"(save)
        : "v"(queue), "v"(one)
        : "memory");
    return uint32_t(__builtin_amdgcn_readfirstlane(int(x)));
}

typedef unsigned short v2u __attribute__((ext_vector_type(2)));
__device__ __forceinline__ v2u as_v2u(uint32_t x) { return __builtin_bit_cast(v2u, x); }
__device__ __forceinline__ uint32_t u32_of(v2u x) { return __builtin_bit_cast(uint32_t, x); }
__device__ __forceinline__ uint32_t umax2(uint32_t a, uint32_t b) { return u32_of(__builtin_elementwise_max(as_v2u(a), as_v2u(b))); }
__device__ __forceinline__ uint32_t umin2(uint32_t a, uint32_t b) { return u32_of(__builtin_elementwise_min(as_v2u(a), as_v2u(b))); }
__device__ __forceinline__ uint32_t usubs2(uint32_t a, uint32_t b) { return u32_of(__builtin_elementwise_sub_sat(as_v2u(a), as_v2u(b))); }
__device__ __forceinline__ uint32_t clampu16(int v) { return uint32_t(min(max(v, 0), 65535)); }
__device__ __forceinline__ uint32_t packu(uint32_t lo, uint32_t hi) { return lo | (hi << 16); }
__device__ __forceinline__ int v2_half(uint32_t w, int h) { return h ? int(w >> 16) : int(w & 0xFFFFu); }
constexpr int U16_BIAS = 32768;

__device__ __forceinline__ void cells_u16(uint32_t (&Hq)[FW_C], uint32_t (&F)[FW_C], const uint4& xa, const uint4& xb, uint32_t& hql, uint32_t& el,
                                          uint32_t dgq, uint32_t gd2)
{
    const uint32_t xl[FW_C / 4] = {xa.x, xa.y, xa.z, xa.w}, xh[FW_C / 4] = {xb.x, xb.y, xb.z, xb.w};
    uint32_t T[FW_C];
#pragma unroll
    for (int c = 0; c < FW_C; ++c) {
        const uint32_t Fn = umax2(F[c], Hq[c]);
        const uint32_t sel = 0x0c000c00u | uint32_t(4 + (c & 3)) << 16 | uint32_t(c & 3);
        const uint32_t inc = __builtin_amdgcn_perm(xh[c >> 2], xl[c >> 2], sel);
        T[c] = umax2((c ? Hq[c - 1] : dgq) + inc, Fn);
        F[c] = Fn;
    }
    uint32_t e = el, h = hql;
#pragma unroll
    for (int c = 0; c < FW_C; ++c) {
        e = umax2(e, h);
        h = umax2(T[c], e) - gd2;
        Hq[c] = h;
    }
    hql = h;
    el = e;
}

__device__ __forceinline__ uint32_t v2_par(uint32_t lds_byte_addr)
{
    uint32_t x;
    asm volatile("ds_read_b32 %0, %1\n\ts_waitcnt lgkmcnt(0)" : "=v"(x) : "v"(lds_byte_addr) : "memory");
    return x;
}

__device__ __forceinline__ void v2_lds_store(uint32_t lds_byte_addr, uint32_t v)
{
    asm volatile("ds_write_b32 %0, %1\n\ts_waitcnt lgkmcnt(0)" : : "v"(lds_byte_addr), "v"(v) : "memory");
}

enum V2Par : uint32_t {
    VP_N0 = 0, VP_N1, VP_M0, VP_M1, VP_GD0, VP_GD1, VP_LROW0, VP_LROW1, VP_BEST0, VP_BEST1, VP_PID0, VP_PID1,
    VP_RDAT_LO, VP_RDAT_HI, VP_RBASE_LO, VP_RBASE_HI, VP_CDAT_LO, VP_CDAT_HI, VP_CBASE_LO, VP_CBASE_HI,
    VP_MPAD, VP_NQ, VP_FLAG, VP_BAND, VP_STRIP, VP_COLIN_LO, VP_COLIN_HI, VP_RHI0, VP_RHI1, VP_COUNT = 32
};

__global__ void __launch_bounds__(128)
k_fwd2_prof(const AlnPairDev* __restrict__ pairs, const V2Couple* __restrict__ couples, const uint8_t* __restrict__ pool, AlnParams P, uint4* __restrict__ prof)
{
    const V2Couple& cp = couples[blockIdx.x];
    const uint32_t p = blockIdx.y;
    if (p >= cp.nstrips) return;
    const uint32_t h = threadIdx.x >> 6, lane = threadIdx.x & 63u;
    const bool have = cp.pid[h] != 0xFFFFFFFFu;
    const AlnPairDev pr = pairs[have ? cp.pid[h] : cp.pid[0]];
    const uint32_t m = have ? pr.m : 0u;
    const uint8_t* r = pool + pr.r_off;
    const int ge = P.gap_extend, gd = pr.gap_open - ge;
    const int cm = P.match + 2 * ge + gd, cx = P.mismatch + 2 * ge + gd;
    const uint32_t jb = p * (64u * FW_C) + lane * FW_C;
    uint32_t rpk[FW_C / 4];
#pragma unroll
    for (int c4 = 0; c4 < FW_C / 4; ++c4) {
        uint32_t w = 0;
#pragma unroll
        for (int e = 0; e < 4; ++e) w |= (have ? ref_byte(r, m, pr.rc, jb + c4 * 4 + e) : 0u) << (8 * e);
        rpk[c4] = w;
    }
    const uint32_t bases = 'A' | ('C' << 8) | ('G' << 16) | ('T' << 24);
    uint4* out = prof + cp.prof + (uint64_t(p) * 2u + h) * 5u * 64u + lane;
#pragma unroll
    for (int code = 0; code < 5; ++code) {
        const uint32_t b = code < 4 ? (bases >> (8 * code)) & 0xFFu : 0x100u;
        uint32_t w4[FW_C / 4];
#pragma unroll
        for (int c4 = 0; c4 < FW_C / 4; ++c4) {
            uint32_t w = 0;
#pragma unroll
            for (int e = 0; e < 4; ++e) w |= uint32_t(((rpk[c4] >> (8 * e)) & 0xFFu) == b ? cm : cx) << (8 * e);
            w4[c4] = w;
        }
        out[uint32_t(code) * 64u] = uint4{w4[0], w4[1], w4[2], w4[3]};
    }
}

static __device__ __forceinline__ void
v2_fwd_body(const AlnPairDev* __restrict__ pairs, const V2Couple* __restrict__ couples, const V2Item* __restrict__ items, uint32_t n_items,
       uint32_t* __restrict__ queue, uint32_t* __restrict__ flags, uint32_t* __restrict__ err, const uint8_t* __restrict__ pool, AlnParams P,
       uint32_t* __restrict__ arena, int2* __restrict__ lrow, int2* __restrict__ bandbest, uint32_t* __restrict__ ovf_out, int guard,
       const uint4* __restrict__ prof, unsigned long long* __restrict__ cells_done, uint32_t* __restrict__ prog, uint32_t prog_every)
{
    __shared__ __attribute__((aligned(16))) uint32_t s_look_all[V2_WAVES][3][128];
    __shared__ __attribute__((aligned(16))) uint32_t s_prof_all[V2_WAVES][2][5][64][4];
    __shared__ uint32_t s_par_all[V2_WAVES][VP_COUNT];
    const uint32_t lane = threadIdx.x & 63u;
    const uint32_t wv = uint32_t(__builtin_amdgcn_readfirstlane(int(threadIdx.x >> 6)));
    uint32_t(*s_look)[128] = s_look_all[wv];
    uint32_t* s_par = s_par_all[wv];
    const uint32_t par_addr = uint32_t(reinterpret_cast<uintptr_t>(s_par));
    auto par = [&](uint32_t k) -> uint32_t { return v2_par(par_addr + 4u * k); };
    auto par64 = [&](uint32_t k) -> uint64_t { return uint64_t(par(k)) | (uint64_t(par(k + 1u)) << 32); };
    constexpr uint32_t strip_cols = 64u * FW_C;
    const int ge = P.gap_extend;
    auto qcode = [](uint32_t ch) -> uint32_t {
        const uint32_t code = ch == 'A' ? 0u : ch == 'C' ? 1u : ch == 'G' ? 2u : ch == 'T' ? 3u : 4u;
        return code * 1024u;
    };
    uint32_t it = v2_dequeue(queue);
    while (it < n_items) {
        uint32_t band, p, r_lo, nblk[2];
        bool vh[2], last_band[2];
        bool left_ok = true;
        bool top_none = false;
        bool left_rows = false;
        uint32_t left_idx = 0, nblk_band = 0, left_avail = 0;
        const uint8_t* q[2];
        int base[2];
        uint32_t gd2;
        uint32_t Hp[FW_C], F[FW_C];
        uint32_t dg;
        uint64_t cb_off = 0;
        uint64_t co_off = 0;
        uint64_t rd_off = 0;
        uint64_t rb_off = 0;
        uint32_t mpad = 0, ncr = 0;
        {
            const V2Item item = items[it];
            const V2Couple cp = couples[item.couple];
            band = item.band;
            p = item.strip;
            if (p < cp.plo[band] || p > cp.phi[band] ||
                __builtin_amdgcn_readfirstlane(int(__hip_atomic_load(&flags[cp.flag0 + band * cp.nstrips + p], __ATOMIC_RELAXED, __HIP_MEMORY_SCOPE_AGENT))) != 0) {
                it = v2_dequeue(queue);
                continue;
            }
            const bool top_in = band > 0 && p >= cp.plo[band - 1u] && p <= cp.phi[band - 1u];
            const bool left_in = p > cp.plo[band];
            left_ok = p == 0 || left_in;
            top_none = band > 0 && !top_in;
            const bool corner_in = band > 0 && p > 0 && p - 1u >= cp.plo[band - 1u] && p - 1u <= cp.phi[band - 1u];
            if (top_in) (void)v2_wait(&flags[cp.flag0 + (band - 1u) * cp.nstrips + p], err);
            left_rows = prog != nullptr && left_in;
            left_idx = cp.flag0 + band * cp.nstrips + (p - 1u);
            {
                const uint32_t rows_b = min(max(cp.pid[0] != 0xFFFFFFFFu ? pairs[cp.pid[0]].n : 0u, cp.pid[1] != 0xFFFFFFFFu ? pairs[cp.pid[1]].n : 0u),
                                            uint32_t(cp.bstart[band + 1u]) * uint32_t(CK2));
                const uint32_t r0_b = uint32_t(cp.bstart[band]) * uint32_t(CK2);
                nblk_band = rows_b > r0_b ? (rows_b - r0_b + FW_R - 1) / FW_R : 0u;
            }
            if (left_in && !left_rows) (void)v2_wait(&flags[left_idx], err);
            if (left_rows) (void)v2_wait_rows(&prog[left_idx], &flags[left_idx], min(32u, nblk_band), err, left_avail);
            __builtin_amdgcn_fence(__ATOMIC_ACQUIRE, "agent");
            r_lo = uint32_t(cp.bstart[band]) * uint32_t(CK2);
            const uint32_t jb = p * strip_cols + lane * FW_C;
            uint32_t n[2], m[2], r_hi[2];
            int gd[2];
#pragma unroll
            for (int h = 0; h < 2; ++h) {
                const bool have = cp.pid[h] != 0xFFFFFFFFu;
                const AlnPairDev pr = pairs[have ? cp.pid[h] : cp.pid[0]];
                n[h] = have ? pr.n : 0u;
                m[h] = have ? pr.m : 0u;
                q[h] = pool + pr.q_off;
                gd[h] = pr.gap_open - ge;
                r_hi[h] = min(n[h], uint32_t(cp.bstart[band + 1u]) * uint32_t(CK2));
                nblk[h] = r_hi[h] > r_lo ? (r_hi[h] - r_lo + FW_R - 1) / FW_R : 0u;
                const uint32_t nstr = (m[h] + strip_cols - 1) / strip_cols;
                vh[h] = have && p < nstr && nblk[h] > 0;
                last_band[h] = vh[h] && r_hi[h] == n[h];
            }
            gd2 = packu(uint32_t(gd[0]), uint32_t(gd[1]));
            mpad = cp.mpad;
            rd_off = cp.rdat + jb;
            rb_off = cp.rbase + uint64_t(jb / 16u) * 2u;
            {
                uint32_t nmx = max(n[0], n[1]);
                ncr = nmx ? (nmx - 1u) / uint32_t(CK2) : 0u;
            }
            {
                const uint64_t e0 = uint64_t((jb + FW_C) / CK2 - ((jb + FW_C) >= uint32_t(CK2) ? 1u : 0u)) * cp.nq + r_lo / 4u;
                co_off = cp.cdat + e0 * 8u;
                cb_off = cp.cbase + e0 * 2u;
            }
            const uint64_t colin = p ? uint64_t(p * (strip_cols / CK2) - 1u) * cp.nq : 0;
            __builtin_amdgcn_fence(__ATOMIC_RELEASE, "workgroup");
            __builtin_amdgcn_wave_barrier();
            if (lane == 0) {
                s_par[VP_N0] = n[0];
                s_par[VP_N1] = n[1];
                s_par[VP_M0] = m[0];
                s_par[VP_M1] = m[1];
                s_par[VP_GD0] = uint32_t(gd[0]);
                s_par[VP_GD1] = uint32_t(gd[1]);
                s_par[VP_LROW0] = cp.lrow0[0];
                s_par[VP_LROW1] = cp.lrow0[1];
                s_par[VP_BEST0] = cp.best0[0];
                s_par[VP_BEST1] = cp.best0[1];
                s_par[VP_PID0] = cp.pid[0];
                s_par[VP_PID1] = cp.pid[1];
                s_par[VP_RDAT_LO] = uint32_t(cp.rdat);
                s_par[VP_RDAT_HI] = uint32_t(cp.rdat >> 32);
                s_par[VP_RBASE_LO] = uint32_t(cp.rbase);
                s_par[VP_RBASE_HI] = uint32_t(cp.rbase >> 32);
                s_par[VP_CDAT_LO] = uint32_t(cp.cdat);
                s_par[VP_CDAT_HI] = uint32_t(cp.cdat >> 32);
                s_par[VP_CBASE_LO] = uint32_t(cp.cbase);
                s_par[VP_CBASE_HI] = uint32_t(cp.cbase >> 32);
                s_par[VP_MPAD] = cp.mpad;
                s_par[VP_NQ] = cp.nq;
                s_par[VP_FLAG] = cp.flag0 + band * cp.nstrips + p;
                s_par[VP_BAND] = band;
                s_par[VP_STRIP] = p;
                s_par[VP_COLIN_LO] = uint32_t(colin);
                s_par[VP_COLIN_HI] = uint32_t(colin >> 32);
                s_par[VP_RHI0] = r_hi[0];
                s_par[VP_RHI1] = r_hi[1];
            }
            int Ha[2][FW_C], Fa[2][FW_C], dga[2];
#pragma unroll
            for (int h = 0; h < 2; ++h) {
                if (!vh[h]) {
#pragma unroll
                    for (int c = 0; c < FW_C; ++c) Ha[h][c] = Fa[h][c] = 0;
                    dga[h] = 0;
                } else if (r_lo > 0 && !top_in) {
#pragma unroll
                    for (int c = 0; c < FW_C; ++c) Ha[h][c] = Fa[h][c] = ALN_NEG;
                    dga[h] = ALN_NEG;
                } else if (r_lo == 0) {
                    const int b0 = ge * int(jb) - gd[h];
#pragma unroll
                    for (int c = 0; c < FW_C; ++c) {
                        Ha[h][c] = b0 + ge * (c + 1);
                        Fa[h][c] = ALN_NEG;
                    }
                    dga[h] = b0;
                } else {
                    const uint32_t ckr = r_lo / CK2 - 1u;
                    const uint32_t* rh = arena + cp.rdat + uint64_t(2u * ckr) * cp.mpad;
                    const uint32_t* rf = rh + cp.mpad;
                    const int2* rb = reinterpret_cast<const int2*>(arena + cp.rbase) + uint64_t(ckr) * (cp.mpad / 16u);
                    const int2 bb = jb < cp.mpad ? rb[jb / 16u] : int2{0, 0};
                    const int bs = h ? bb.y : bb.x;
#pragma unroll
                    for (int c = 0; c < FW_C; ++c) {
                        int2 v{0, 0};
                        if (jb + c < m[h]) v = int2{v2_half(rh[jb + c], h) + bs, v2_half(rf[jb + c], h) + bs};
                        Ha[h][c] = v.x;
                        Fa[h][c] = v.y;
                    }
                    if (lane == 0 && p > 0 && !corner_in) {
                        dga[h] = ALN_NEG;
                    } else if (jb > 0 && jb <= m[h]) {
                        const int2 bl = rb[(jb - 1u) / 16u];
                        dga[h] = v2_half(rh[jb - 1u], h) + (h ? bl.y : bl.x);
                    } else {
                        dga[h] = ge * int(r_lo) - gd[h];
                    }
                }
                if (vh[h] && r_lo > 0 && !top_in) {
                    const uint64_t e = colin + r_lo / 4u;
                    const uint32_t* d = arena + cp.cdat + e * 8u;
                    const int2 bb = reinterpret_cast<const int2*>(arena + cp.cbase)[e];
                    base[h] = v2_half(d[0], h) + (h ? bb.y : bb.x) - U16_BIAS;
                } else
                base[h] = __builtin_amdgcn_readfirstlane(Ha[h][0]) - U16_BIAS;
            }
#pragma unroll
            for (int c = 0; c < FW_C; ++c) {
                const bool in0 = vh[0] && jb + c < m[0], in1 = vh[1] && jb + c < m[1];
                Hp[c] = packu(in0 ? clampu16(Ha[0][c] - base[0]) : uint32_t(U16_BIAS), in1 ? clampu16(Ha[1][c] - base[1]) : uint32_t(U16_BIAS));
                F[c] = packu(in0 ? clampu16(Fa[0][c] - base[0]) : uint32_t(U16_BIAS), in1 ? clampu16(Fa[1][c] - base[1]) : uint32_t(U16_BIAS));
            }
            dg = packu(clampu16(dga[0] - base[0]), clampu16(dga[1] - base[1]));
            {
                const uint4* pp = prof + cp.prof + uint64_t(p) * (2u * 5u * 64u) + lane;
#pragma unroll
                for (int h = 0; h < 2; ++h)
#pragma unroll
                    for (int code = 0; code < 5; ++code) {
                        const uint4 w = pp[(uint32_t(h) * 5u + uint32_t(code)) * 64u];
                        *reinterpret_cast<uint4*>(&s_prof_all[wv][h][code][lane][0]) = w;
                    }
            }
        }
        const uint32_t jb = p * strip_cols + lane * FW_C;
        const uint32_t nsteps = max(nblk[0], nblk[1]) + 63u;
        uint32_t lanef = 0;
        int lastc[2];
        uint32_t ncl[2];
        bool strip_has_lastc = false;
        __builtin_amdgcn_fence(__ATOMIC_RELEASE, "workgroup");
        __builtin_amdgcn_wave_barrier();
        __builtin_amdgcn_fence(__ATOMIC_ACQUIRE, "workgroup");
        {
            const uint32_t jr = jb + FW_C;
            bool any_right = false;
#pragma unroll
            for (int h = 0; h < 2; ++h) {
                const uint32_t mh = par(VP_M0 + h);
                const bool hc = vh[h] && jb < mh;
                ncl[h] = vh[h] ? min(64u, (mh - p * strip_cols + FW_C - 1) / FW_C) : 0u;
                lastc[h] = (vh[h] && mh - 1 >= jb && mh - 1 < jb + FW_C) ? int(mh - 1 - jb) : -1;
                strip_has_lastc = strip_has_lastc || (vh[h] && uint64_t(p + 1u) * strip_cols >= mh);
                any_right = any_right || (vh[h] && jr < mh);
                lanef |= (hc ? 1u : 0u) << h;
                lanef |= (lastc[h] >= 0 ? 4u : 0u) << h;
            }
            if ((jr % CK2) == 0 && any_right) lanef |= 16u;
        }
        const uint8_t* profA = reinterpret_cast<const uint8_t*>(&s_prof_all[wv][0][0][lane][0]);
        const uint8_t* profB = reinterpret_cast<const uint8_t*>(&s_prof_all[wv][1][0][lane][0]);
        auto left_edge = [&](int h, uint32_t row) {
            int2 v{ge * int(row + 1) - int(par(VP_GD0 + h)), ALN_NEG};
            if (!left_ok) v = int2{ALN_NEG, ALN_NEG};
            else if (vh[h] && p > 0 && row < par(VP_RHI0 + h)) {
                const uint64_t e = par64(VP_COLIN_LO) + row / 4u;
                const uint32_t* d = arena + par64(VP_CDAT_LO) + e * 8u;
                const int2 bb = reinterpret_cast<const int2*>(arena + par64(VP_CBASE_LO))[e];
                const int bs = h ? bb.y : bb.x;
                v = int2{v2_half(d[row & 3u], h) + bs, v2_half(d[4u + (row & 3u)], h) + bs};
            }
            return v;
        };
        uint32_t qn = 0;
        int2 en[2] = {{0, 0}, {0, 0}};
        uint32_t hl[FW_R], el[FW_R];
        uint32_t qc[FW_R];
#pragma unroll
        for (int rr = 0; rr < FW_R; ++rr) {
            hl[rr] = packu(U16_BIAS, U16_BIAS);
            el[rr] = 0;
            qc[rr] = 0;
        }
        auto publish = [&](uint32_t blk) {
            s_look[0][(blk & 1u) * 64u + lane] = packu(clampu16(en[0].x - base[0]), clampu16(en[1].x - base[1]));
            s_look[1][(blk & 1u) * 64u + lane] = packu(clampu16(en[0].y - base[0]), clampu16(en[1].y - base[1]));
            s_look[2][(blk & 1u) * 64u + lane] = qn;
        };
        auto fetch = [&](uint32_t blk) {
            const uint32_t row = r_lo + blk * 64u + lane;
            uint32_t qq[2];
#pragma unroll
            for (int h = 0; h < 2; ++h) {
                qq[h] = qcode((vh[h] && row < par(VP_RHI0 + h)) ? q[h][row] : 0u);
                en[h] = left_edge(h, row);
            }
            qn = qq[0] | (qq[1] << 16);
        };
        fetch(0);
        publish(0);
        fetch(1);
        __builtin_amdgcn_fence(__ATOMIC_RELEASE, "workgroup");
        __builtin_amdgcn_wave_barrier();
        __builtin_amdgcn_fence(__ATOMIC_ACQUIRE, "workgroup");
        uint4 nxh, nxe, nxq;
        nxh = *reinterpret_cast<const uint4*>(&s_look[0][0]);
        nxe = *reinterpret_cast<const uint4*>(&s_look[1][0]);
        nxq = *reinterpret_cast<const uint4*>(&s_look[2][0]);
        {
            const uint32_t q4[FW_R] = {nxq.x, nxq.y, nxq.z, nxq.w};
#pragma unroll
            for (int rr = 0; rr < FW_R; ++rr) qc[rr] = from_left_or(qc[rr], q4[rr]);
        }
        int bc[2] = {ALN_NEG, ALN_NEG};
        uint32_t bc_i[2] = {0, 0};
        uint32_t ovf = 0;

        auto step = [&](const uint32_t s, auto first) __attribute__((always_inline)) {
            if (decltype(first)::value && (s & (64 / FW_R - 1)) == 0) {
                if (s) {
                    int dl[2];
#pragma unroll
                    for (int h = 0; h < 2; ++h) {
                        const uint32_t lr = s + 1u > nblk[h] ? min(63u, s + 1u - nblk[h]) : 0u;
                        const int ref = __builtin_amdgcn_readlane(int(Hp[0]), int(lr));
                        dl[h] = max(v2_half(uint32_t(ref), h) - U16_BIAS, 0);
                        if (!vh[h] || lr >= ncl[h]) dl[h] = 0;
                        base[h] += dl[h];
                    }
                    const uint32_t d2 = packu(uint32_t(dl[0]), uint32_t(dl[1]));
                    {
                        uint32_t mx = Hp[0], mn = Hp[0];
#pragma unroll
                        for (int c = 1; c < FW_C; ++c) {
                            mx = umax2(mx, Hp[c]);
                            mn = umin2(mn, Hp[c]);
                        }
                        const int bi = int(s) - int(lane);
#pragma unroll
                        for (int h = 0; h < 2; ++h) {
                            const int hi_v = v2_half(mx, h) - U16_BIAS, lo_v = v2_half(mn, h) - U16_BIAS;
                            if ((lanef >> h & 1u) && bi >= (top_none ? 1 : 0) && uint32_t(bi) < nblk[h] && (hi_v > guard || lo_v < -guard)) {
#ifdef IOC_V2_GUARD_DEBUG
                                if (!(ovf >> h & 1u)) printf("guard: item %u band %u strip %u half %d lane %u step %u hi %d lo %d left_ok %d base %d\n", it, band, p, h, lane, s, hi_v, lo_v, int(left_ok), base[h]);
#endif
                                ovf |= 1u << h;
                            }
                        }
                    }
#pragma unroll
                    for (int c = 0; c < FW_C; ++c) {
                        Hp[c] = usubs2(Hp[c], d2);
                        F[c] = usubs2(F[c], d2);
                    }
                    dg = usubs2(dg, d2);
#pragma unroll
                    for (int rr = 0; rr < FW_R; ++rr) {
                        hl[rr] = usubs2(hl[rr], d2);
                        el[rr] = usubs2(el[rr], d2);
                    }
                    nxh = uint4{usubs2(nxh.x, d2), usubs2(nxh.y, d2), usubs2(nxh.z, d2), usubs2(nxh.w, d2)};
                    nxe = uint4{usubs2(nxe.x, d2), usubs2(nxe.y, d2), usubs2(nxe.z, d2), usubs2(nxe.w, d2)};
                    const uint32_t cur = ((s / (64 / FW_R)) & 1u) * 64u + lane;
                    s_look[0][cur] = usubs2(s_look[0][cur], d2);
                    s_look[1][cur] = usubs2(s_look[1][cur], d2);
                }
                const uint32_t blk = s / (64 / FW_R) + 1u;
                if (prog != nullptr && s >= 64u && (prog_every <= 1u || (s / 16u) % prog_every == 0u)) {
                    asm volatile("s_waitcnt vmcnt(0)" ::: "memory");
                    __builtin_amdgcn_fence(__ATOMIC_RELEASE, "agent");
                    asm volatile("s_waitcnt vmcnt(0)" ::: "memory");
                    __hip_atomic_store(&prog[uint32_t(__builtin_amdgcn_readfirstlane(int(par(VP_FLAG))))], s - 63u, __ATOMIC_RELAXED, __HIP_MEMORY_SCOPE_AGENT);
                }
                publish(blk);
                if (left_rows) {
                    const uint32_t need_rows = min(16u * (blk + 2u), nblk_band);
                    if (need_rows > left_avail) {
                        (void)v2_wait_rows(&prog[left_idx], &flags[left_idx], need_rows, err, left_avail);
                        __builtin_amdgcn_fence(__ATOMIC_ACQUIRE, "agent");
                    }
                }
                fetch(blk + 1u);
            }
            {
                const uint32_t h4[FW_R] = {nxh.x, nxh.y, nxh.z, nxh.w}, e4[FW_R] = {nxe.x, nxe.y, nxe.z, nxe.w};
#pragma unroll
                for (int rr = 0; rr < FW_R; ++rr) {
                    hl[rr] = from_left_or(hl[rr], h4[rr]);
                    el[rr] = from_left_or(el[rr], e4[rr]);
                }
                const uint32_t nx = ((s + 1u) * FW_R) & 127u;
                nxh = *reinterpret_cast<const uint4*>(&s_look[0][nx]);
                nxe = *reinterpret_cast<const uint4*>(&s_look[1][nx]);
                nxq = *reinterpret_cast<const uint4*>(&s_look[2][nx]);
            }
            const int bi = int(s) - int(lane);
            bool act[2];
#pragma unroll
            for (int h = 0; h < 2; ++h) act[h] = (lanef >> h & 1u) && bi >= 0 && uint32_t(bi) < nblk[h];
            if (act[0] || act[1]) {
                const bool special = strip_has_lastc || (last_band[0] && s + 1u >= nblk[0] && s + 1u - nblk[0] < 64u) ||
                                     (last_band[1] && s + 1u >= nblk[1] && s + 1u - nblk[1] < 64u);
                auto row_cells = [&](int rr) __attribute__((always_inline)) {
                    const uint32_t hl_in = hl[rr];
                    const uint4 xa = *reinterpret_cast<const uint4*>(profA + (qc[rr] & 0xFFFFu));
                    const uint4 xb = *reinterpret_cast<const uint4*>(profB + (qc[rr] >> 16));
                    cells_u16(Hp, F, xa, xb, hl[rr], el[rr], dg, gd2);
                    dg = hl_in;
                };
#pragma unroll
                for (int rr = 0; rr < FW_R; ++rr) {
                    row_cells(rr);
                    if (special) {

#pragma unroll
                        for (int h = 0; h < 2; ++h) {
                            const uint32_t i = r_lo + uint32_t(bi) * FW_R + rr;
                            const uint32_t nh = par(VP_N0 + h), mh = par(VP_M0 + h);
                            const int gdh = int(par(VP_GD0 + h));
                            if (act[h] && i < nh) {
                                if (lastc[h] >= 0) {
                                    const uint32_t lc = uint32_t(lastc[h]);
                                    const bool b0 = lc & 1u, b1 = lc & 2u, b2 = lc & 4u, b3 = lc & 8u;
                                    const uint32_t s0 = b0 ? Hp[1] : Hp[0], s1 = b0 ? Hp[3] : Hp[2], s2 = b0 ? Hp[5] : Hp[4], s3 = b0 ? Hp[7] : Hp[6],
                                                   s4 = b0 ? Hp[9] : Hp[8], s5 = b0 ? Hp[11] : Hp[10], s6 = b0 ? Hp[13] : Hp[12], s7 = b0 ? Hp[15] : Hp[14];
                                    const uint32_t u0 = b1 ? s1 : s0, u1 = b1 ? s3 : s2, u2 = b1 ? s5 : s4, u3 = b1 ? s7 : s6;
                                    const uint32_t v0 = b2 ? u1 : u0, v1 = b2 ? u3 : u2;
                                    int hm = v2_half(b3 ? v1 : v0, h) + base[h];
                                    hm += gdh - ge * int(i + 1u + mh);
                                    if (hm > bc[h]) {
                                        bc[h] = hm;
                                        bc_i[h] = i + 1u;
                                    }
                                }
                                if (i + 1u == nh) {
                                    int br = ALN_NEG;
                                    uint32_t bj = 0;
                                    const int b0 = base[h] + gdh - ge * int(nh + jb);
#pragma unroll
                                    for (int c = 0; c < FW_C; ++c) {
                                        const int ht = v2_half(Hp[c], h) + b0 - ge * (c + 1);
                                        if (jb + c < mh && ht > br) {
                                            br = ht;
                                            bj = jb + c + 1;
                                        }
                                    }
                                    lrow[par(VP_LROW0 + h) + p * 64u + lane] = int2{br, int(bj)};
                                }
                            }
                        }
                    }
                }
                const uint32_t ib = uint32_t(bi);
                if (lanef & 16u) {
                    uint32_t* d = arena + co_off + uint64_t(ib) * 8u;
                    uint4* co = reinterpret_cast<uint4*>(d);
                    co[0] = uint4{hl[0], hl[1], hl[2], hl[3]};
                    co[1] = uint4{el[0], el[1], el[2], el[3]};
                    reinterpret_cast<int2*>(arena + cb_off)[ib] = int2{base[0], base[1]};
                }
                const uint32_t i1 = (ib + 1u) * FW_R;
                if ((i1 % CK2) == 0) {
                    const uint32_t ckr1 = (r_lo + i1) / CK2;
                    if (ckr1 <= ncr) {
                        uint32_t* rh = arena + rd_off + uint64_t(2u * (ckr1 - 1u)) * mpad;
                        uint4* oh = reinterpret_cast<uint4*>(rh);
                        uint4* of = reinterpret_cast<uint4*>(rh + mpad);
#pragma unroll
                        for (int c = 0; c < FW_C; c += 4) {
                            oh[c / 4] = uint4{Hp[c], Hp[c + 1], Hp[c + 2], Hp[c + 3]};
                            of[c / 4] = uint4{F[c], F[c + 1], F[c + 2], F[c + 3]};
                        }
                        reinterpret_cast<int2*>(arena + rb_off)[uint64_t(ckr1 - 1u) * (mpad / 16u)] = int2{base[0], base[1]};
                    }
                }
            }
            {
                const uint32_t q4[FW_R] = {nxq.x, nxq.y, nxq.z, nxq.w};
#pragma unroll
                for (int rr = 0; rr < FW_R; ++rr) qc[rr] = from_left_or(qc[rr], q4[rr]);
            }
        };
        {
            uint32_t s = 0;
            for (; s + 1u < nsteps; s += 2) {
                step(s, std::true_type{});
                step(s + 1u, std::false_type{});
            }
            for (; s < nsteps; ++s) step(s, std::true_type{});
        }
#pragma unroll
        for (int h = 0; h < 2; ++h) {
            if (lastc[h] >= 0) bandbest[par(VP_BEST0 + h) + band] = int2{bc[h], int(bc_i[h])};
            if ((ovf >> h) & 1u) {
                const uint32_t pidh = par(VP_PID0 + h);
                if (pidh != 0xFFFFFFFFu) atomicOr(&ovf_out[pidh], 1u);
            }
        }
        if (lane == 0) {
            unsigned long long cells = 0;
#pragma unroll
            for (int h = 0; h < 2; ++h)
                if (vh[h]) cells += (unsigned long long)(par(VP_RHI0 + h) - r_lo) * (unsigned long long)min(strip_cols, par(VP_M0 + h) - p * strip_cols);
            atomicAdd(cells_done, cells);
        }
        const uint32_t my_flag = uint32_t(__builtin_amdgcn_readfirstlane(int(par(VP_FLAG))));
        asm volatile("s_waitcnt vmcnt(0)" ::: "memory");
        __builtin_amdgcn_fence(__ATOMIC_RELEASE, "agent");
        asm volatile("s_waitcnt vmcnt(0)" ::: "memory");
        __hip_atomic_store(&flags[my_flag], 1u, __ATOMIC_RELAXED, __HIP_MEMORY_SCOPE_AGENT);
        it = v2_dequeue(queue);
    }
}

#define V2_FWD_ARGS                                                                                                                        \
    const AlnPairDev *__restrict__ pairs, const V2Couple *__restrict__ couples, const V2Item *__restrict__ items, uint32_t n_items,        \
        uint32_t *__restrict__ queue, uint32_t *__restrict__ flags, uint32_t *__restrict__ err, const uint8_t *__restrict__ pool, AlnParams P, \
        uint32_t *__restrict__ arena, int2 *__restrict__ lrow, int2 *__restrict__ bandbest, uint32_t *__restrict__ ovf_out, int guard,     \
        const uint4 *__restrict__ prof, unsigned long long *__restrict__ cells_done, uint32_t *__restrict__ prog, uint32_t prog_every
__global__ void __launch_bounds__(64 * V2_WAVES) __attribute__((amdgpu_waves_per_eu(3, 8))) k_fwd2(V2_FWD_ARGS)
{
    v2_fwd_body(pairs, couples, items, n_items, queue, flags, err, pool, P, arena, lrow, bandbest, ovf_out, guard, prof, cells_done, prog, prog_every);
}
__global__ void __launch_bounds__(64 * V2_WAVES) __attribute__((amdgpu_waves_per_eu(2, 2))) k_fwd2_w2(V2_FWD_ARGS)
{
    v2_fwd_body(pairs, couples, items, n_items, queue, flags, err, pool, P, arena, lrow, bandbest, ovf_out, guard, prof, cells_done, prog, prog_every);
}


struct V2PairEnd {
    uint32_t lrow0, best0, nbands, couple;
    int32_t cert;
};
constexpr uint32_t V2_RESUME_WORDS = 16;

__global__ void __launch_bounds__(64)
k_fwd2_probe(const AlnPairDev* __restrict__ pairs, V2Couple* __restrict__ couples, V2PairEnd* __restrict__ pe, const uint32_t* __restrict__ arena, AlnParams P)
{
    V2Couple& cp = couples[blockIdx.x];
    if (!cp.corridor) return;
    const uint32_t lane = threadIdx.x;
    const uint32_t strip_cols = 64u * FW_C;
    const uint32_t R = uint32_t(cp.bstart[cp.probe_band + 1u]) * uint32_t(CK2);
    const uint32_t ckr = R / uint32_t(CK2) - 1u;
    const uint32_t* rh = arena + cp.rdat + uint64_t(2u * ckr) * cp.mpad;
    const int2* rb = reinterpret_cast<const int2*>(arena + cp.rbase) + uint64_t(ckr) * (cp.mpad / 16u);
    bool wrong = false;
    uint32_t nmax = 0, mmax = 0, need = 0, need_raw = 0;
    for (int h = 0; h < 2; ++h) {
        if (cp.pid[h] == 0xFFFFFFFFu) continue;
        const AlnPairDev pr = pairs[cp.pid[h]];
        nmax = max(nmax, pr.n);
        mmax = max(mmax, pr.m);
        const int gd = pr.gap_open - P.gap_extend;
        int mx = INT32_MIN;
        const uint32_t x0 = uint32_t(cp.probe_strip) * strip_cols, x1 = min(pr.m, x0 + strip_cols);
        for (uint32_t x = x0 + lane; x < x1; x += 64) {
            const int2 bb = rb[x / 16u];
            mx = max(mx, v2_half(rh[x], h) + (h ? bb.y : bb.x) + gd - P.gap_extend * int(R + x + 1u));
        }
        for (int o = 32; o > 0; o >>= 1) mx = max(mx, __shfl_xor(mx, o));
        if (pr.n < R || x1 <= x0 || mx < P.match * int(R) / 4) {
            wrong = true;
        } else {
            const float len = float(max(pr.n, pr.m)), rate = float(mx) / float(R);
            const float b = len - 0.97f * rate * float(min(pr.n, pr.m)) / float(P.match) + 512.0f;
            need = max(need, uint32_t(max(b, 0.0f)));
            need_raw = max(need_raw, uint32_t(max(len - rate * float(min(pr.n, pr.m)) / float(P.match), 0.0f)));
        }
    }
    const uint32_t len_max = max(nmax, mmax);
    const uint32_t B0 = cp.b0;
    if (!wrong && need_raw > B0 && need > B0) {
        if (float(need) > 0.4f * float(len_max)) {
            wrong = true;
        } else if (lane == 0) {
            long long beff = 0x7FFFFFFFFFFFll;
            uint32_t skipped = 0;
            for (uint32_t b = 0; b < cp.nbands; ++b) {
                const uint32_t r0 = uint32_t(cp.bstart[b]) * uint32_t(CK2), r1 = min(nmax, uint32_t(cp.bstart[b + 1u]) * uint32_t(CK2));
                const uint32_t c_lo = r0 > need ? r0 - need : 0u;
                const unsigned long long c_hi = min((unsigned long long)mmax, (unsigned long long)r1 + need);
                const uint32_t lo = c_lo / strip_cols, hi = uint32_t((max(c_hi, 1ull) - 1ull) / strip_cols);
                cp.plo[b] = uint16_t(min(lo, uint32_t(cp.plo[b])));
                cp.phi[b] = uint16_t(max(hi, uint32_t(cp.phi[b])));
                skipped += uint32_t(cp.plo[b]) + (cp.nstrips - 1u - uint32_t(cp.phi[b]));
                if (cp.plo[b] > 0) beff = min(beff, (long long)r0 - (long long)cp.plo[b] * strip_cols);
                if ((unsigned long long)(uint32_t(cp.phi[b]) + 1u) * strip_cols < mmax) beff = min(beff, (long long)(uint32_t(cp.phi[b]) + 1u) * strip_cols - (long long)r1);
            }
            for (int h = 0; h < 2; ++h)
                if (cp.pid[h] != 0xFFFFFFFFu) {
                    const AlnPairDev pr = pairs[cp.pid[h]];
                    const long long ct = (long long)P.match * max(0ll, (long long)max(pr.n, pr.m) - beff - 1ll);
                    pe[cp.pid[h]].cert = beff == 0x7FFFFFFFFFFFll ? INT32_MIN : int32_t(min(ct, 0x7FFFFFFFll));
                }
            if (skipped * 5u < cp.nbands * cp.nstrips) cp.corridor = 2u;
        }
    }
    __builtin_amdgcn_fence(__ATOMIC_RELEASE, "workgroup");
    __builtin_amdgcn_wave_barrier();
    if ((wrong || __hip_atomic_load(&cp.corridor, __ATOMIC_RELAXED, __HIP_MEMORY_SCOPE_WORKGROUP) == 2u) && lane == 0) {
        for (uint32_t b = 0; b < uint32_t(V2_MAX_BANDS); ++b) {
            cp.plo[b] = 0;
            cp.phi[b] = uint16_t(min(65535u, cp.nstrips - 1u));
        }
        cp.corridor = 0;
        for (int h = 0; h < 2; ++h)
            if (cp.pid[h] != 0xFFFFFFFFu) pe[cp.pid[h]].cert = INT32_MIN;
    }
}

__global__ void __launch_bounds__(64)
k_fwd2_ends(const AlnPairDev* __restrict__ pairs, const V2Couple* __restrict__ couples, const uint32_t* __restrict__ order, uint32_t count, const V2PairEnd* __restrict__ pe,
            const int2* __restrict__ lrow, const int2* __restrict__ bandbest, const uint32_t* __restrict__ ovf, int4* __restrict__ ends,
            uint32_t* __restrict__ resume, uint32_t* __restrict__ early, const int route_below, const uint32_t route_cap)
{
    const uint32_t pslot = blockIdx.x;
    if (pslot >= count) return;
    const uint32_t pid = order[pslot], lane = threadIdx.x;
    const AlnPairDev pr = pairs[pid];
    const V2PairEnd e = pe[pid];
    const uint32_t n = pr.n, m = pr.m;
    const uint32_t nstrips = (m + 64u * FW_C - 1) / (64u * FW_C);
    int br = 0;
    uint32_t bj = 0;
    for (uint32_t x = lane; x < nstrips * 64u; x += 64) {
        if (uint64_t(x) * FW_C >= m) continue;
        const int2 v = lrow[e.lrow0 + x];
        if (v.x > br || (v.x == br && uint32_t(v.y) < bj)) {
            br = v.x;
            bj = uint32_t(v.y);
        }
    }
    for (int o = 32; o > 0; o >>= 1) {
        const int s = __shfl_xor(br, o);
        const uint32_t j = __shfl_xor(bj, o);
        if (s > br || (s == br && j < bj)) {
            br = s;
            bj = j;
        }
    }
    if (lane == 0) {
        int fin = ALN_NEG;
        uint32_t bi = 0, bjj = m;
        for (uint32_t b = 0; b < e.nbands; ++b) {
            if (uint64_t(couples[e.couple].bstart[b]) * CK2 >= n) break;
            const int2 bb = bandbest[e.best0 + b];
            if (bb.x > fin) {
                fin = bb.x;
                bi = uint32_t(bb.y);
            }
        }
        if (br > fin) {
            fin = br;
            bi = n;
            bjj = bj;
        }
        const bool refuted = e.cert != INT32_MIN && fin <= e.cert;
        ends[pid] = int4{fin, int(bi), int(bjj), int(ovf[pid] & 1u) | (refuted ? 2 : 0)};
        if (route_below > 0 && pr.stop_at && !(ovf[pid] & 1u) && !refuted && min(n, m) >= 8u * uint32_t(CK2) &&
            (fin < route_below * int(min(n, m)) / 4 || count <= route_cap)) {
            const uint32_t slot = atomicAdd(&early[0], 1u);
            if (slot < route_cap) {
                resume[size_t(pid) * V2_RESUME_WORDS + 6] = 2u;
                early[1u + slot] = pslot;
            }
        }
    }
}

struct V2Scratch {
    int2 frow[CK2 / TILE][CK2 + 8];
    int2 fcol[CK2 / TILE][CK2];
};

__device__ __forceinline__ int2 v2_ld(const int2* p)
{
    const int x = __hip_atomic_load(&p->x, __ATOMIC_RELAXED, __HIP_MEMORY_SCOPE_AGENT);
    const int y = __hip_atomic_load(&p->y, __ATOMIC_RELAXED, __HIP_MEMORY_SCOPE_AGENT);
    return int2{x, y};
}

constexpr uint32_t V2_NROLE = 5, V2_NHELP = 2 * V2_NROLE, V2_HBUF = 2, V2_HWAVES = 1 + V2_NHELP;
enum V2Help : uint32_t { VH_SEQ = 0, VH_RB, VH_CB, VH_I, VH_J, VH_QUIT, VH_WORK = 8 , VH_SLOT = VH_WORK + 3 * V2_NHELP ,
                         VH_COUNT = VH_SLOT + 3 * V2_NHELP * V2_HBUF };

template <bool HELP>
__device__ __forceinline__ void trace2_body(const AlnPairDev* __restrict__ pairs, const uint32_t* __restrict__ order, const uint8_t* __restrict__ pool,
                                            const AlnParams& P, const uint32_t* __restrict__ arena, const V2Couple* __restrict__ couples, const V2PairCk* __restrict__ pck,
                                            const int4* __restrict__ ends, V2Scratch* __restrict__ scratch, V2Scratch* __restrict__ hscratch,
                                            uint32_t* __restrict__ resume, uint32_t* __restrict__ park, int32_t* __restrict__ out_score,
                                            uint32_t* __restrict__ out_count, const uint32_t count, const uint32_t max_blocks,
                                            const unsigned long long max_cycles, const uint32_t pslot, const uint32_t wv, const uint32_t want)
{
    constexpr int NW = HELP ? int(V2_HWAVES) : TR_WAVES, NDIRS = HELP ? 1 : TR_WAVES;
    constexpr uint32_t B_LEFT = uint32_t(CK2) * 8u, B_Q = uint32_t(CK2) * 4u, B_PROF = 5u * 64u * uint32_t(V2_BLK_C / 4) * 4u;
    constexpr uint32_t D_BYTES = uint32_t(TILE) * uint32_t(TR_C) / 4u * 64u * 2u;
    constexpr uint32_t U_BYTES = (B_LEFT + B_Q + B_PROF) > D_BYTES ? (B_LEFT + B_Q + B_PROF) : D_BYTES;
    __shared__ __attribute__((aligned(16))) uint8_t s_union_all[NW][U_BYTES];
    __shared__ __attribute__((aligned(16))) uint8_t s_tile_all[NDIRS][uint32_t(TILE) * 12u];
    __shared__ uint32_t s_help[VH_COUNT];
    if (pslot >= count) return;
    uint16_t(*dirs)[64] = reinterpret_cast<uint16_t(*)[64]>(&s_union_all[wv][0]);
    int2* const b_left = reinterpret_cast<int2*>(&s_union_all[wv][0]);
    uint32_t* const b_q = reinterpret_cast<uint32_t*>(&s_union_all[wv][B_LEFT]);
    uint32_t* const b_prof = reinterpret_cast<uint32_t*>(&s_union_all[wv][B_LEFT + B_Q]);
    int2* const s_left = reinterpret_cast<int2*>(&s_tile_all[HELP ? 0u : wv][0]);
    uint32_t* const s_q = reinterpret_cast<uint32_t*>(&s_tile_all[HELP ? 0u : wv][uint32_t(TILE) * 8u]);
    const uint32_t pid = order[pslot];
    const AlnPairDev pr = pairs[pid];
    const V2PairCk ck = pck[pid];
    const int hf = int(ck.half);
    const bool corridor = __builtin_amdgcn_readfirstlane(int(couples[ck.couple].corridor)) != 0;
    uint32_t* const rs = resume + size_t(pid) * V2_RESUME_WORDS;
    {
        const uint32_t fl = uint32_t(__builtin_amdgcn_readfirstlane(int(rs[6])));
        if (HELP ? fl != want : fl == 2u) return;
    }
    V2Scratch* scp = &scratch[pslot];
    const unsigned long long t_begin = __builtin_amdgcn_s_memtime();
    uint32_t n_blocks = 0, n_diag = 0, n_tiles = 0, n_gapsteps = 0;
    const uint32_t n = pr.n, m = pr.m;
    const int go = pr.gap_open, il = pr.ilimit;
    const uint8_t* __restrict__ q = pool + pr.q_off;
    const uint8_t* __restrict__ r = pool + pr.r_off;
    const uint32_t lane = threadIdx.x & 63u;
    const uint32_t k = P.k, kmask = k >= 32 ? 0xFFFFFFFFu : ((1u << k) - 1u);
    const int4 en = ends[pid];
    if (en.w & 3) {
        if (lane == 0) {
            out_score[pid] = (en.w & 1) ? INT32_MIN : INT32_MIN + 1;
            out_count[pid] = 0xFFFFFFFFu;
        }
        return;
    }
    const int gd = go - P.gap_extend, ge = P.gap_extend;
    FwdConst K;
    K.ge = ge;
    K.gd = gd;
    K.cm = P.match + 2 * ge + gd;
    K.cx = P.mismatch + 2 * ge + gd;
    uint32_t i = uint32_t(en.y), j = uint32_t(en.z);
    int state = 0;
    WinStat ws;
    if (HELP && want == 1u) {
        i = rs[0];
        j = rs[1];
        state = int(rs[2]);
        ws.wb = rs[3];
        ws.pushed = rs[4];
        ws.cnt = rs[5];
    } else {
        ws.blanks((m - j) + (n - i), kmask, k, il);
    }
    uint32_t blk_r = 0xFFFFFFFFu, blk_c = 0xFFFFFFFFu;
    auto coarse_row = [&](uint32_t R, uint32_t x) {
        const uint32_t ckr = R / CK2 - 1u;
        const uint32_t* rh = arena + ck.rdat + uint64_t(2u * ckr) * ck.mpad;
        const int2 bb = reinterpret_cast<const int2*>(arena + ck.rbase)[uint64_t(ckr) * (ck.mpad / 16u) + x / 16u];
        const int bs = hf ? bb.y : bb.x;
        return int2{v2_half(rh[x], hf) + bs, v2_half(rh[ck.mpad + x], hf) + bs};
    };
    auto coarse_col = [&](uint32_t C, uint32_t y) {
        const uint64_t e = uint64_t(C / CK2 - 1u) * ck.nq + y / 4u;
        const uint32_t* d = arena + ck.cdat + e * 8u;
        const int2 bb = reinterpret_cast<const int2*>(arena + ck.cbase)[e];
        const int bs = hf ? bb.y : bb.x;
        return int2{v2_half(d[y & 3u], hf) + bs, v2_half(d[4u + (y & 3u)], hf) + bs};
    };

    auto recompute_block = [&](const uint32_t Rb, const uint32_t Cb, const uint32_t brows, const uint32_t bcols, V2Scratch& dst) __attribute__((always_inline)) {
        bool top_ok = true, left_ok = true, corner_ok = true;
        if (corridor) {
            const V2Couple& cq = couples[ck.couple];
            auto band_of = [&](uint32_t row) {
                const uint32_t cr = row / uint32_t(CK2);
                uint32_t b = 0;
                while (b + 1u < cq.nbands && uint32_t(cq.bstart[b + 1u]) <= cr) ++b;
                return b;
            };
            auto in = [&](uint32_t b, uint32_t p) { return p >= cq.plo[b] && p <= cq.phi[b]; };
            const uint32_t ps = Cb / (64u * FW_C), pl = Cb ? (Cb - 1u) / (64u * FW_C) : 0u;
            const uint32_t bb = band_of(Rb), bt = Rb ? band_of(Rb - 1u) : 0u;
            if (Rb) top_ok = in(bt, ps);
            if (Cb) left_ok = in(bb, pl);
            if (Rb && Cb) corner_ok = in(bt, pl);
        }
        for (uint32_t x = lane; x <= bcols; x += 64) {
            int2 v;
            if (Rb == 0)
                v = int2{ge * int(Cb + x) - gd, ALN_NEG};
            else if (Cb + x == 0)
                v = int2{ge * int(Rb) - gd, ALN_NEG};
            else if (x ? top_ok : corner_ok)
                v = coarse_row(Rb, Cb + x - 1u);
            else
                v = int2{ALN_NEG, ALN_NEG};
            dst.frow[0][x] = v;
        }
        for (uint32_t y = lane; y < brows; y += 64) {
            int2 v{ge * int(Rb + y + 1) - gd, ALN_NEG};
            if (Cb) v = left_ok ? coarse_col(Cb, Rb + y) : int2{ALN_NEG, ALN_NEG};
            dst.fcol[0][y] = v;
            b_left[y] = v;
            const uint32_t ch = q[Rb + y];
            b_q[y] = (ch == 'A' ? 0u : ch == 'C' ? 1u : ch == 'G' ? 2u : ch == 'T' ? 3u : 4u) * uint32_t(64 * (V2_BLK_C / 4) * 4);
        }
        for (uint32_t y = brows + lane; y < ((brows + 3u) & ~3u) + 4u && y < uint32_t(CK2); y += 64) {
            b_left[y] = int2{0, ALN_NEG};
            b_q[y] = 0;
        }
        const uint32_t jb8 = Cb + lane * V2_BLK_C;
        uint32_t rpk[V2_BLK_C / 4];
#pragma unroll
        for (int c4 = 0; c4 < V2_BLK_C / 4; ++c4) {
            uint32_t w = 0;
#pragma unroll
            for (int e = 0; e < 4; ++e) w |= ref_byte(r, m, pr.rc, jb8 + c4 * 4 + e) << (8 * e);
            rpk[c4] = w;
        }
        {
            const uint32_t bases = 'A' | ('C' << 8) | ('G' << 16) | ('T' << 24);
#pragma unroll
            for (int code = 0; code < 5; ++code) {
                const uint32_t bq = code < 4 ? (bases >> (8 * code)) & 0xFFu : 0x100u;
#pragma unroll
                for (int c4 = 0; c4 < V2_BLK_C / 4; ++c4) {
                    uint32_t w = 0;
#pragma unroll
// ... 383 lines not shown
```

Measured before the change: 61100.

## Process runs of consecutive bands per work item in v2 forward aligner

Each forward work item now covers a run of up to several consecutive bands in one strip instead of a single band. The wavefront sweeps the run continuously, publishes intermediate band flags as it goes, fetches left-neighbour readiness per band, and records the per-band best at band boundaries. This is meant to cut per-item dequeue, setup and profile-load overhead and reduce the number of flag handoffs, at the cost of less parallelism in the dependency wavefront and more complex synchronisation. A host-side plan checker is added to validate item ordering.

```diff
diff --git a/include/isonclust2_hip.h b/include/isonclust2_hip.h
--- a/include/isonclust2_hip.h
+++ b/include/isonclust2_hip.h
@@ -125,6 +125,8 @@
                    int32_t* score_out);
 int32_t ioc_host_gap_open(double e1_plus_e2);
 double ioc_host_aln_ratio(const char* comp, int32_t comp_len, double e, uint32_t slen, uint32_t k);
+int ioc_host_v2_plan_check(int32_t n_pairs, const uint32_t* n, const uint32_t* m, const float* e, double corridor_frac,
+                           double budget_mb, int32_t run, int32_t want_bands, int64_t* stats);
 
 typedef struct {
     int32_t query;
diff --git a/isonclust2_amd/_lib.py b/isonclust2_amd/_lib.py
--- a/isonclust2_amd/_lib.py
+++ b/isonclust2_amd/_lib.py
@@ -111,7 +111,7 @@
     "ioc_extract_minimizers", "ioc_extracted_download", "ioc_extracted_hpc_download", "ioc_queries_from_extracted",
     "ioc_get_timings", "ioc_count_reference_postings", "ioc_host_gap_limits", "ioc_host_err_cell", "ioc_host_min_total",
     "ioc_cluster_batch", "ioc_cluster_merge", "ioc_cluster_resident", "ioc_host_align", "ioc_host_gap_open",
-    "ioc_host_aln_ratio", "ioc_align_set_pool", "ioc_align_pairs", "ioc_set_aln_verdicts", "ioc_get_ties", "ioc_resident_set_sequences",
+    "ioc_host_aln_ratio", "ioc_host_v2_plan_check", "ioc_align_set_pool", "ioc_align_pairs", "ioc_set_aln_verdicts", "ioc_get_ties", "ioc_resident_set_sequences",
     "ioc_index_update", "ioc_left_export", "ioc_cluster_consensus",
     "ioc_poa_create", "ioc_poa_create_mode", "ioc_poa_destroy", "ioc_poa_bind", "ioc_poa_graph_export", "ioc_poa_last_alignment",
     "ioc_poa_graph_save", "ioc_poa_graph_load", "ioc_poa_graph_load_many", "ioc_gather_records_device", "ioc_queries_generation", "ioc_scored_candidates",
diff --git a/isonclust2_amd/csrc/ioc_align_gpu.hip b/isonclust2_amd/csrc/ioc_align_gpu.hip
--- a/isonclust2_amd/csrc/ioc_align_gpu.hip
+++ b/isonclust2_amd/csrc/ioc_align_gpu.hip
@@ -1193,6 +1193,7 @@
     uint64_t arena_words = 0, prof_total = 0;
     std::vector<std::vector<V2Item>> items;
     std::vector<uint32_t> n_probe;
+    std::vector<uint32_t> run;
     uint32_t max_items = 0, max_flags = 0, max_pairs = 0;
 };
 
@@ -1367,12 +1368,15 @@
     }
 }
 
-void tile_lists(V2Plan& pl)
+void tile_lists(V2Plan& pl, uint32_t run_k, uint32_t few_limit)
 {
     pl.items.resize(pl.slices.size());
     pl.n_probe.assign(pl.slices.size(), 0);
+    pl.run.assign(pl.slices.size(), 1u);
     for (size_t si = 0; si < pl.slices.size(); ++si) {
         const uint32_t k_lo = pl.slices[si].first, k_hi = pl.slices[si].first + pl.slices[si].second;
+        const uint32_t K = (few_limit && pl.slices[si].second <= few_limit) ? 1u : std::max(1u, run_k);
+        pl.run[si] = K;
         uint32_t nf = 0;
         auto& it = pl.items[si];
         uint32_t maxdiag = 0;
@@ -1397,12 +1401,17 @@
             if (!any && dg > 64u) break;
         }
         pl.n_probe[si] = uint32_t(it.size());
-        for (uint32_t dg = 0; dg <= maxdiag; ++dg)
+        uint32_t maxkey = 0;
+        for (uint32_t k2 = k_lo; k2 < k_hi; ++k2) {
+            const V2Couple& cp = pl.cps[k2];
+            maxkey = std::max(maxkey, (cp.nbands - 1u) / K * K + cp.nstrips - 1u);
+        }
+        for (uint32_t key = 0; key <= maxkey; ++key)
             for (uint32_t k2 = k_lo; k2 < k_hi; ++k2) {
                 const V2Couple& cp = pl.cps[k2];
-                if (dg > cp.nbands + cp.nstrips - 2u) continue;
-                const uint32_t b_lo = dg >= cp.nstrips ? dg - cp.nstrips + 1u : 0u, b_hi = std::min(dg, cp.nbands - 1u);
-                for (uint32_t b = b_lo; b <= b_hi; ++b) it.push_back(V2Item{k2, uint16_t(b), uint16_t(dg - b)});
+                const uint32_t nch = (cp.nbands + K - 1u) / K;
+                const uint32_t j_lo = key >= cp.nstrips ? (key - cp.nstrips + K) / K : 0u, j_hi = std::min(key / K, nch - 1u);
+                for (uint32_t j = j_lo; j <= j_hi && j < nch; ++j) it.push_back(V2Item{k2, uint16_t(j * K), uint16_t(key - j * K)});
             }
         pl.max_items = std::max<uint32_t>(pl.max_items, uint32_t(it.size()));
         pl.max_flags = std::max(pl.max_flags, nf);
@@ -1413,6 +1422,7 @@
 struct V2Opts {
     int n_cu, occ, guard;
     uint32_t few_limit;
+    uint32_t run;
     uint32_t deadline;
     unsigned long long deadline_cycles;
     uint32_t help_wgs;
@@ -1509,14 +1519,14 @@
         ACHK(c, hipMemcpyAsync(d_ctl + 1, &one, 4, hipMemcpyHostToDevice, s));
     }
     ACHK(c, hipEventRecord(ev[0], s));
-    auto fwd = [&](decltype(&k_fwd2) kernel, uint32_t n_wg, const V2Item* items, uint32_t n) {
+    auto fwd = [&](decltype(&k_fwd2) kernel, uint32_t n_wg, const V2Item* items, uint32_t n, uint32_t run) {
         hipLaunchKernelGGL(kernel, dim3(n_wg), dim3(64 * V2_WAVES), 0, s, d_pairs, t.cps, items, n, d_ctl, d_ctl + 16, d_ctl + 1, d_pool, P,
                            static_cast<uint32_t*>(c->a_ck.p), t.lrow, t.best, d_ctl + 16 + 2 * pl.max_flags, o.guard, static_cast<const uint4*>(c->a_prof.p),
                            reinterpret_cast<unsigned long long*>(d_ctl + t.ctl_words - 2), few_couples ? d_ctl + 16 + pl.max_flags : static_cast<uint32_t*>(nullptr),
-                           prog_every);
+                           prog_every, run);
     };
     if (n_probe) {
-        fwd(k_fwd2, std::max(1u, std::min(uint32_t(o.occ) * uint32_t(o.n_cu), (n_probe + V2_WAVES - 1) / V2_WAVES)), t.items, n_probe);
+        fwd(k_fwd2, std::max(1u, std::min(uint32_t(o.occ) * uint32_t(o.n_cu), (n_probe + V2_WAVES - 1) / V2_WAVES)), t.items, n_probe, 1u);
         ACHK(c, hipGetLastError());
         hipLaunchKernelGGL(k_fwd2_probe, dim3(n_couples), dim3(64), 0, s, d_pairs, t.cps + k_first, t.pend, static_cast<const uint32_t*>(c->a_ck.p), P);
         ACHK(c, hipGetLastError());
@@ -1524,7 +1534,7 @@
     }
     const uint32_t n_main = n_items - n_probe, per_cu = v2_per_cu(pl, si, o, few_couples);
     const uint32_t n_wg = std::max(1u, std::min(per_cu * uint32_t(o.n_cu), (n_main + V2_WAVES - 1) / V2_WAVES));
-    fwd((per_cu <= 2 && !getenv("IOC_ALIGN_V2_NO_W2")) ? k_fwd2_w2 : k_fwd2, n_wg, t.items + n_probe, n_main);
+    fwd((per_cu <= 2 && !getenv("IOC_ALIGN_V2_NO_W2")) ? k_fwd2_w2 : k_fwd2, n_wg, t.items + n_probe, n_main, pl.run[si]);
     ACHK(c, hipGetLastError());
     const uint32_t n_help = std::min<uint32_t>(n_pairs, o.help_wgs);
     hipLaunchKernelGGL(k_fwd2_ends, dim3(n_pairs), dim3(64), 0, s, d_pairs, t.cps, d_order + first_pair, n_pairs, t.pend, t.lrow, t.best,
@@ -1641,6 +1651,8 @@
     if (const char* e = getenv("IOC_ALIGN_V2_GUARD")) o.guard = std::max(1, std::min(P16_GUARD, atoi(e)));
     o.few_limit = 128;
     if (const char* e = getenv("IOC_ALIGN_V2_FEW")) o.few_limit = uint32_t(std::max(0, atoi(e)));
+    o.run = V2_RUN_DEFAULT;
+    if (const char* e = getenv("IOC_ALIGN_V2_RUN")) o.run = atoi(e) > 0 ? uint32_t(std::min(atoi(e), V2_MAX_BANDS)) : uint32_t(V2_MAX_BANDS);
     if (hipOccupancyMaxActiveBlocksPerMultiprocessor(&o.occ, reinterpret_cast<const void*>(k_fwd2), 64 * V2_WAVES, 0) != hipSuccess) o.occ = 0;
     (void)hipGetLastError();
     if (o.occ < 1) o.occ = 3;
@@ -1660,7 +1672,7 @@
         fprintf(stderr, "[ioc]   aligner v2: %u couples, checkpoint arena %.1f MB (%zu slice(s)) reserved in %.3f ms; corridor: %llu of %llu tiles skipped\n", pl.ncouples,
                 double(pl.arena_words) * 4e-6, pl.slices.size(), std::chrono::duration<double, std::milli>(std::chrono::steady_clock::now() - t_res0).count(),
                 (unsigned long long)pl.tiles_skipped, (unsigned long long)pl.tiles_all);
-    tile_lists(pl);
+    tile_lists(pl, o.run, o.few_limit);
 
     o.deadline = 4;
     if (const char* e = getenv("IOC_TRACE2_DEADLINE")) o.deadline = uint32_t(std::max(0, atoi(e)));
@@ -1689,8 +1701,8 @@
     }
     add_elapsed(c, evs.v, evi);
     if (getenv("IOC_TRACE"))
-        fprintf(stderr, "[ioc]   aligner v2: forward %.3f ms, traceback %.3f ms (device, all slices so far)%s\n", c->tm.ms_align_fwd,
-                c->tm.ms_align_trace, bad ? " — a wait ran out: falling back to version 1" : "");
+        fprintf(stderr, "[ioc]   aligner v2: forward %.3f ms, traceback %.3f ms (device, all slices so far), runs of %u bands%s\n", c->tm.ms_align_fwd,
+                c->tm.ms_align_trace, pl.run.empty() ? 1u : pl.run[0], bad ? " — a wait ran out: falling back to version 1" : "");
     *fell_back = bad;
     return IOC_OK;
 }
@@ -2214,9 +2226,101 @@
     return scatter_results(c, b, pairs, v2, P, hs, hc, out);
 }
 
+int64_t v2_check_order(const V2Plan& pl)
+{
+    int64_t bad = 0;
+    for (uint32_t k2 = 0; k2 < pl.ncouples; ++k2)
+        for (uint32_t b = 1; b < pl.cps[k2].nbands; ++b) bad += (pl.cps[k2].plo[b] < pl.cps[k2].plo[b - 1u] || pl.cps[k2].phi[b] < pl.cps[k2].phi[b - 1u]) ? 1 : 0;
+    for (size_t si = 0; si < pl.slices.size(); ++si) {
+        const uint32_t k_lo = pl.slices[si].first, k_hi = k_lo + pl.slices[si].second, K = pl.run[si];
+        const auto& it = pl.items[si];
+        std::vector<size_t> base(k_hi - k_lo + 1u, 0);
+        for (uint32_t k2 = k_lo; k2 < k_hi; ++k2) base[k2 - k_lo + 1u] = base[k2 - k_lo] + size_t(pl.cps[k2].nbands) * pl.cps[k2].nstrips;
+        const size_t none = ~size_t(0);
+        std::vector<size_t> probe_pos(base.back(), none), item_of(base.back(), none);
+        auto tile = [&](uint32_t k2, uint32_t b, uint32_t s) { return base[k2 - k_lo] + size_t(b) * pl.cps[k2].nstrips + s; };
+        for (size_t x = 0; x < pl.n_probe[si]; ++x) {
+            const V2Item& i = it[x];
+            bad += (i.band > 0 && probe_pos[tile(i.couple, i.band - 1u, i.strip)] == none) ? 1 : 0;
+            bad += (i.strip > 0 && probe_pos[tile(i.couple, i.band, i.strip - 1u)] == none) ? 1 : 0;
+            probe_pos[tile(i.couple, i.band, i.strip)] = x;
+        }
+        for (size_t x = pl.n_probe[si]; x < it.size(); ++x) {
+            const V2Item& i = it[x];
+            const V2Couple& cp = pl.cps[i.couple];
+            bad += (i.couple < k_lo || i.couple >= k_hi || i.band % K != 0u || i.band >= cp.nbands || i.strip >= cp.nstrips) ? 1 : 0;
+            for (uint32_t b = i.band; b < std::min(cp.nbands, uint32_t(i.band) + K); ++b) {
+                size_t& o = item_of[tile(i.couple, b, i.strip)];
+                bad += o != none ? 1 : 0;
+                o = x;
+            }
+        }
+        for (size_t t = 0; t < item_of.size(); ++t) bad += item_of[t] == none ? 1 : 0;
+        for (int wide = 0; wide < 2; ++wide)
+            for (size_t x = pl.n_probe[si]; x < it.size(); ++x) {
+                const V2Item& i = it[x];
+                const V2Couple& cp = pl.cps[i.couple];
+                auto in = [&](uint32_t b, uint32_t s) { return probe_pos[tile(i.couple, b, s)] == none && (wide || (s >= cp.plo[b] && s <= cp.phi[b])); };
+                bool first = true;
+                for (uint32_t b = i.band; b < std::min(cp.nbands, uint32_t(i.band) + K); ++b) {
+                    if (!in(b, i.strip)) {
+                        if (!first) break;
+                        continue;
+                    }
+                    if (first && b > 0 && in(b - 1u, i.strip)) bad += item_of[tile(i.couple, b - 1u, i.strip)] >= x ? 1 : 0;
+                    if (i.strip > 0 && in(b, i.strip - 1u)) bad += item_of[tile(i.couple, b, i.strip - 1u)] >= x ? 1 : 0;
+                    first = false;
+                }
+            }
+    }
+    return bad;
+}
+
 }
 
 extern "C" {
+
+int ioc_host_v2_plan_check(int32_t n_pairs, const uint32_t* n, const uint32_t* m, const float* e, double corridor_frac, double budget_mb, int32_t run,
+                           int32_t want_bands, int64_t* stats)
+{
+    if (n_pairs <= 0 || !n || !m || !e || !stats) return IOC_ERR_ARG;
+    std::vector<AlnPairDev> dp(static_cast<size_t>(n_pairs));
+    std::vector<uint32_t> order(static_cast<size_t>(n_pairs));
+    for (int32_t i = 0; i < n_pairs; ++i) {
+        if (n[i] == 0 || m[i] == 0) return IOC_ERR_ARG;
+        dp[size_t(i)] = AlnPairDev{};
+        dp[size_t(i)].n = n[i];
+        dp[size_t(i)].m = m[i];
+        dp[size_t(i)].e_sum = e[i];
+        dp[size_t(i)].gap_open = ioc_host_gap_open(double(e[i]));
+        order[size_t(i)] = uint32_t(i);
+    }
+    std::sort(order.begin(), order.end(), [&](uint32_t a, uint32_t b) { return uint64_t(dp[a].n) * dp[a].m > uint64_t(dp[b].n) * dp[b].m; });
+    AlnParams P{};
+    P.match = 2;
+    P.mismatch = -2;
+    P.gap_extend = 1;
+    const CorridorModel cm{nullptr, P, std::max(0.0, corridor_frac), true, false};
+    V2Plan pl;
+    pl.cnt = uint32_t(n_pairs);
+    pl.np = uint32_t(n_pairs);
+    pl.ncouples = (pl.cnt + 1u) / 2u;
+    plan_couples(pl, dp, order.data(), cm, want_bands > 0 ? uint32_t(want_bands) : band_target(pl.ncouples, 128u, 3, 256));
+    slice_couples(pl, uint64_t(std::max(0.0, budget_mb) * 1e6));
+    tile_lists(pl, run > 0 ? uint32_t(std::min(run, V2_MAX_BANDS)) : uint32_t(V2_MAX_BANDS), 0u);
+    int64_t items = 0, corr = 0, maxb = 0;
+    for (size_t si = 0; si < pl.slices.size(); ++si) items += int64_t(pl.items[si].size() - pl.n_probe[si]);
+    for (const V2Couple& cp : pl.cps) {
+        corr += cp.corridor ? 1 : 0;
+        maxb = std::max<int64_t>(maxb, cp.nbands);
+    }
+    stats[0] = v2_check_order(pl);
+    stats[1] = items;
+    stats[2] = int64_t(pl.slices.size());
+    stats[3] = corr;
+    stats[4] = maxb;
+    return IOC_OK;
+}
 
 int ioc_align_set_pool(ioc_ctx* c, int32_t n_seqs, const char* seqs, const int64_t* offs)
 {
diff --git a/isonclust2_amd/csrc/ioc_align_v2.inc b/isonclust2_amd/csrc/ioc_align_v2.inc
--- a/isonclust2_amd/csrc/ioc_align_v2.inc
+++ b/isonclust2_amd/csrc/ioc_align_v2.inc
@@ -3,6 +3,7 @@
 constexpr int V2_WAVES = 4;
 constexpr int V2_BLK_C = 8;
 constexpr int V2_MAX_BANDS = 40;
+constexpr int V2_RUN_DEFAULT = 3;
 static_assert(CK2 % TILE == 0 && CK2 == 64 * V2_BLK_C, "block geometry");
 
 struct V2Couple {
@@ -134,7 +135,10 @@
 enum V2Par : uint32_t {
     VP_N0 = 0, VP_N1, VP_M0, VP_M1, VP_GD0, VP_GD1, VP_LROW0, VP_LROW1, VP_BEST0, VP_BEST1, VP_PID0, VP_PID1,
     VP_RDAT_LO, VP_RDAT_HI, VP_RBASE_LO, VP_RBASE_HI, VP_CDAT_LO, VP_CDAT_HI, VP_CBASE_LO, VP_CBASE_HI,
-    VP_MPAD, VP_NQ, VP_FLAG, VP_BAND, VP_STRIP, VP_COLIN_LO, VP_COLIN_HI, VP_RHI0, VP_RHI1, VP_COUNT = 32
+    VP_MPAD, VP_NQ, VP_FLAG, VP_BAND, VP_STRIP, VP_COLIN_LO, VP_COLIN_HI, VP_RHI0, VP_RHI1,
+    VP_NBR, VP_NSTRIPS, VP_LEFTM_LO, VP_LEFTM_HI, VP_LEFTOK, VP_FETK, VP_PUBK,
+    VP_RSTART,
+    VP_COUNT = VP_RSTART + V2_MAX_BANDS + 1
 };
 
 __global__ void __launch_bounds__(128)
@@ -180,7 +184,7 @@
 v2_fwd_body(const AlnPairDev* __restrict__ pairs, const V2Couple* __restrict__ couples, const V2Item* __restrict__ items, uint32_t n_items,
        uint32_t* __restrict__ queue, uint32_t* __restrict__ flags, uint32_t* __restrict__ err, const uint8_t* __restrict__ pool, AlnParams P,
        uint32_t* __restrict__ arena, int2* __restrict__ lrow, int2* __restrict__ bandbest, uint32_t* __restrict__ ovf_out, int guard,
-       const uint4* __restrict__ prof, unsigned long long* __restrict__ cells_done, uint32_t* __restrict__ prog, uint32_t prog_every)
+       const uint4* __restrict__ prof, unsigned long long* __restrict__ cells_done, uint32_t* __restrict__ prog, uint32_t prog_every, uint32_t run)
 {
     __shared__ __attribute__((aligned(16))) uint32_t s_look_all[V2_WAVES][3][128];
     __shared__ __attribute__((aligned(16))) uint32_t s_prof_all[V2_WAVES][2][5][64][4];
@@ -202,7 +206,6 @@
     while (it < n_items) {
         uint32_t band, p, r_lo, nblk[2];
         bool vh[2], last_band[2];
-        bool left_ok = true;
         bool top_none = false;
         bool left_rows = false;
         uint32_t left_idx = 0, nblk_band = 0, left_avail = 0;
@@ -219,16 +222,21 @@
         {
             const V2Item item = items[it];
             const V2Couple cp = couples[item.couple];
+            p = item.strip;
+            uint32_t b_end = min(uint32_t(item.band) + run, cp.nbands);
             band = item.band;
-            p = item.strip;
-            if (p < cp.plo[band] || p > cp.phi[band] ||
-                __builtin_amdgcn_readfirstlane(int(__hip_atomic_load(&flags[cp.flag0 + band * cp.nstrips + p], __ATOMIC_RELAXED, __HIP_MEMORY_SCOPE_AGENT))) != 0) {
+            while (band < b_end && (p < cp.plo[band] || p > cp.phi[band] ||
+                                    __builtin_amdgcn_readfirstlane(int(__hip_atomic_load(&flags[cp.flag0 + band * cp.nstrips + p], __ATOMIC_RELAXED, __HIP_MEMORY_SCOPE_AGENT))) != 0))
+                ++band;
+            uint32_t nbr = 0;
+            while (band + nbr < b_end && p >= cp.plo[band + nbr] && p <= cp.phi[band + nbr]) ++nbr;
+            if (nbr == 0) {
                 it = v2_dequeue(queue);
                 continue;
             }
+            b_end = band + nbr;
             const bool top_in = band > 0 && p >= cp.plo[band - 1u] && p <= cp.phi[band - 1u];
             const bool left_in = p > cp.plo[band];
-            left_ok = p == 0 || left_in;
             top_none = band > 0 && !top_in;
             const bool corner_in = band > 0 && p > 0 && p - 1u >= cp.plo[band - 1u] && p - 1u <= cp.phi[band - 1u];
             if (top_in) (void)v2_wait(&flags[cp.flag0 + (band - 1u) * cp.nstrips + p], err);
@@ -255,7 +263,7 @@
                 m[h] = have ? pr.m : 0u;
                 q[h] = pool + pr.q_off;
                 gd[h] = pr.gap_open - ge;
-                r_hi[h] = min(n[h], uint32_t(cp.bstart[band + 1u]) * uint32_t(CK2));
+                r_hi[h] = min(n[h], uint32_t(cp.bstart[b_end]) * uint32_t(CK2));
                 nblk[h] = r_hi[h] > r_lo ? (r_hi[h] - r_lo + FW_R - 1) / FW_R : 0u;
                 const uint32_t nstr = (m[h] + strip_cols - 1) / strip_cols;
                 vh[h] = have && p < nstr && nblk[h] > 0;
@@ -307,6 +315,18 @@
                 s_par[VP_COLIN_HI] = uint32_t(colin >> 32);
                 s_par[VP_RHI0] = r_hi[0];
                 s_par[VP_RHI1] = r_hi[1];
+                s_par[VP_NBR] = nbr;
+                s_par[VP_NSTRIPS] = cp.nstrips;
+                uint64_t lm = 0;
+                for (uint32_t k = 0; k <= nbr; ++k) {
+                    s_par[VP_RSTART + k] = uint32_t(cp.bstart[band + k]) * uint32_t(CK2) - r_lo;
+                    if (k < nbr && p > cp.plo[band + k]) lm |= 1ull << k;
+                }
+                s_par[VP_LEFTM_LO] = uint32_t(lm);
+                s_par[VP_LEFTM_HI] = uint32_t(lm >> 32);
+                s_par[VP_LEFTOK] = (p == 0 || left_in) ? 1u : 0u;
+                s_par[VP_FETK] = 1;
+                s_par[VP_PUBK] = 0;
             }
             int Ha[2][FW_C], Fa[2][FW_C], dga[2];
 #pragma unroll
@@ -405,7 +425,7 @@
         const uint8_t* profB = reinterpret_cast<const uint8_t*>(&s_prof_all[wv][1][0][lane][0]);
         auto left_edge = [&](int h, uint32_t row) {
             int2 v{ge * int(row + 1) - int(par(VP_GD0 + h)), ALN_NEG};
-            if (!left_ok) v = int2{ALN_NEG, ALN_NEG};
+            if (!par(VP_LEFTOK)) v = int2{ALN_NEG, ALN_NEG};
             else if (vh[h] && p > 0 && row < par(VP_RHI0 + h)) {
                 const uint64_t e = par64(VP_COLIN_LO) + row / 4u;
                 const uint32_t* d = arena + par64(VP_CDAT_LO) + e * 8u;
@@ -485,7 +505,7 @@
                             const int hi_v = v2_half(mx, h) - U16_BIAS, lo_v = v2_half(mn, h) - U16_BIAS;
                             if ((lanef >> h & 1u) && bi >= (top_none ? 1 : 0) && uint32_t(bi) < nblk[h] && (hi_v > guard || lo_v < -guard)) {
 #ifdef IOC_V2_GUARD_DEBUG
-                                if (!(ovf >> h & 1u)) printf("guard: item %u band %u strip %u half %d lane %u step %u hi %d lo %d left_ok %d base %d\n", it, band, p, h, lane, s, hi_v, lo_v, int(left_ok), base[h]);
+                                if (!(ovf >> h & 1u)) printf("guard: item %u band %u strip %u half %d lane %u step %u hi %d lo %d left_ok %d base %d\n", it, band, p, h, lane, s, hi_v, lo_v, int(par(VP_LEFTOK)), base[h]);
 #endif
                                 ovf |= 1u << h;
                             }
@@ -515,12 +535,37 @@
                     asm volatile("s_waitcnt vmcnt(0)" ::: "memory");
                     __hip_atomic_store(&prog[uint32_t(__builtin_amdgcn_readfirstlane(int(par(VP_FLAG))))], s - 63u, __ATOMIC_RELAXED, __HIP_MEMORY_SCOPE_AGENT);
                 }
+                const uint32_t nbr_u = uint32_t(__builtin_amdgcn_readfirstlane(int(par(VP_NBR))));
+                if (nbr_u > 1u) {
+                    const uint32_t k = uint32_t(__builtin_amdgcn_readfirstlane(int(par(VP_PUBK))));
+                    if (k + 1u < nbr_u && s == uint32_t(__builtin_amdgcn_readfirstlane(int(par(VP_RSTART + k + 1u)))) / FW_R + 64u) {
+                        asm volatile("s_waitcnt vmcnt(0)" ::: "memory");
+                        __builtin_amdgcn_fence(__ATOMIC_RELEASE, "agent");
+                        asm volatile("s_waitcnt vmcnt(0)" ::: "memory");
+                        const uint32_t f = uint32_t(__builtin_amdgcn_readfirstlane(int(par(VP_FLAG) + k * par(VP_NSTRIPS))));
+                        __hip_atomic_store(&flags[f], 1u, __ATOMIC_RELAXED, __HIP_MEMORY_SCOPE_AGENT);
+                        v2_lds_store(par_addr + 4u * VP_PUBK, k + 1u);
+                    }
+                }
                 publish(blk);
                 if (left_rows) {
                     const uint32_t need_rows = min(16u * (blk + 2u), nblk_band);
                     if (need_rows > left_avail) {
                         (void)v2_wait_rows(&prog[left_idx], &flags[left_idx], need_rows, err, left_avail);
                         __builtin_amdgcn_fence(__ATOMIC_ACQUIRE, "agent");
+                    }
+                }
+                if (nbr_u > 1u) {
+                    const uint32_t k = uint32_t(__builtin_amdgcn_readfirstlane(int(par(VP_FETK))));
+                    if (k < nbr_u && (blk + 1u) * 64u == uint32_t(__builtin_amdgcn_readfirstlane(int(par(VP_RSTART + k))))) {
+                        const uint32_t lmw = uint32_t(__builtin_amdgcn_readfirstlane(int(par(k < 32u ? VP_LEFTM_LO : VP_LEFTM_HI))));
+                        const bool lin = (lmw >> (k & 31u)) & 1u;
+                        if (lin) {
+                            (void)v2_wait(&flags[uint32_t(__builtin_amdgcn_readfirstlane(int(par(VP_FLAG) + k * par(VP_NSTRIPS) - 1u)))], err);
+                            __builtin_amdgcn_fence(__ATOMIC_ACQUIRE, "agent");
+                        }
+                        v2_lds_store(par_addr + 4u * VP_LEFTOK, (p == 0 || lin) ? 1u : 0u);
+                        v2_lds_store(par_addr + 4u * VP_FETK, k + 1u);
                     }
                 }
                 fetch(blk + 1u);
@@ -595,6 +640,23 @@
                     }
                 }
                 const uint32_t ib = uint32_t(bi);
+                if (strip_has_lastc) {
+                    const uint32_t rel1 = (ib + 1u) * FW_R;
+#pragma unroll
+                    for (int h = 0; h < 2; ++h) {
+                        const uint32_t nh = par(VP_N0 + h);
+                        const bool pair_end = r_lo + rel1 >= nh && r_lo + rel1 - FW_R < nh;
+                        if (act[h] && lastc[h] >= 0 && (pair_end || rel1 % uint32_t(CK2) == 0u)) {
+                            uint32_t k = 0;
+                            while (k + 1u < par(VP_NBR) && par(VP_RSTART + k + 1u) < rel1) ++k;
+                            if (pair_end || rel1 == par(VP_RSTART + k + 1u)) {
+                                bandbest[par(VP_BEST0 + h) + par(VP_BAND) + k] = int2{bc[h], int(bc_i[h])};
+                                bc[h] = ALN_NEG;
+                                bc_i[h] = 0;
+                            }
+                        }
+                    }
+                }
                 if (lanef & 16u) {
                     uint32_t* d = arena + co_off + uint64_t(ib) * 8u;
                     uint4* co = reinterpret_cast<uint4*>(d);
@@ -634,7 +696,6 @@
         }
 #pragma unroll
         for (int h = 0; h < 2; ++h) {
-            if (lastc[h] >= 0) bandbest[par(VP_BEST0 + h) + band] = int2{bc[h], int(bc_i[h])};
             if ((ovf >> h) & 1u) {
                 const uint32_t pidh = par(VP_PID0 + h);
                 if (pidh != 0xFFFFFFFFu) atomicOr(&ovf_out[pidh], 1u);
@@ -647,11 +708,15 @@
                 if (vh[h]) cells += (unsigned long long)(par(VP_RHI0 + h) - r_lo) * (unsigned long long)min(strip_cols, par(VP_M0 + h) - p * strip_cols);
             atomicAdd(cells_done, cells);
         }
-        const uint32_t my_flag = uint32_t(__builtin_amdgcn_readfirstlane(int(par(VP_FLAG))));
         asm volatile("s_waitcnt vmcnt(0)" ::: "memory");
         __builtin_amdgcn_fence(__ATOMIC_RELEASE, "agent");
         asm volatile("s_waitcnt vmcnt(0)" ::: "memory");
-        __hip_atomic_store(&flags[my_flag], 1u, __ATOMIC_RELAXED, __HIP_MEMORY_SCOPE_AGENT);
+        {
+            const uint32_t k_end = uint32_t(__builtin_amdgcn_readfirstlane(int(par(VP_NBR))));
+            const uint32_t f0 = uint32_t(__builtin_amdgcn_readfirstlane(int(par(VP_FLAG)))), fs = uint32_t(__builtin_amdgcn_readfirstlane(int(par(VP_NSTRIPS))));
+            for (uint32_t k = uint32_t(__builtin_amdgcn_readfirstlane(int(par(VP_PUBK)))); k < k_end; ++k)
+                __hip_atomic_store(&flags[f0 + k * fs], 1u, __ATOMIC_RELAXED, __HIP_MEMORY_SCOPE_AGENT);
+        }
         it = v2_dequeue(queue);
     }
 }
@@ -660,14 +725,14 @@
     const AlnPairDev *__restrict__ pairs, const V2Couple *__restrict__ couples, const V2Item *__restrict__ items, uint32_t n_items,        \
         uint32_t *__restrict__ queue, uint32_t *__restrict__ flags, uint32_t *__restrict__ err, const uint8_t *__restrict__ pool, AlnParams P, \
         uint32_t *__restrict__ arena, int2 *__restrict__ lrow, int2 *__restrict__ bandbest, uint32_t *__restrict__ ovf_out, int guard,     \
-        const uint4 *__restrict__ prof, unsigned long long *__restrict__ cells_done, uint32_t *__restrict__ prog, uint32_t prog_every
+        const uint4 *__restrict__ prof, unsigned long long *__restrict__ cells_done, uint32_t *__restrict__ prog, uint32_t prog_every, uint32_t run
 __global__ void __launch_bounds__(64 * V2_WAVES) __attribute__((amdgpu_waves_per_eu(3, 8))) k_fwd2(V2_FWD_ARGS)
 {
-    v2_fwd_body(pairs, couples, items, n_items, queue, flags, err, pool, P, arena, lrow, bandbest, ovf_out, guard, prof, cells_done, prog, prog_every);
+    v2_fwd_body(pairs, couples, items, n_items, queue, flags, err, pool, P, arena, lrow, bandbest, ovf_out, guard, prof, cells_done, prog, prog_every, run);
 }
 __global__ void __launch_bounds__(64 * V2_WAVES) __attribute__((amdgpu_waves_per_eu(2, 2))) k_fwd2_w2(V2_FWD_ARGS)
 {
-    v2_fwd_body(pairs, couples, items, n_items, queue, flags, err, pool, P, arena, lrow, bandbest, ovf_out, guard, prof, cells_done, prog, prog_every);
+    v2_fwd_body(pairs, couples, items, n_items, queue, flags, err, pool, P, arena, lrow, bandbest, ovf_out, guard, prof, cells_done, prog, prog_every, run);
 }
 
 
```

Result: faster. 61830 (median of 6 runs) (+1.2%).
